# aagdev/mlimgsynth

Hardware: AMD Instinct MI355X
Metric: images/sec (20-step Euler-a, cfg 7) SDXL 1024x1024 (higher is better)
Workload: dtype f16; 1 GPU; sdxl-1024x1024-euler_a-20-cfg7-b4-vae; batch_per_gpu=4, global_batch=4, unet_evals_per_image=40, hipgraph=False, parallelism=single GPU, weights=synthetic seed 1234

## Files before the change

### include/mlblock_amd.h

```cpp
#pragma once
#include <stdbool.h>
#include <stddef.h>
#include <stdint.h>

#ifdef __cplusplus
extern "C" {
#endif

typedef struct MLCtx MLCtx;
typedef struct MLTensor MLTensor;

enum { MLT_F32 = 0, MLT_F16 = 1, MLT_Q4_0 = 2, MLT_Q4_1 = 3, MLT_Q5_0 = 6, MLT_Q5_1 = 7, MLT_Q8_0 = 8, MLT_I32 = 26, MLT_I64 = 27, MLT_F64 = 28,
       MLT_BF16 = 30 };

enum MLCtxFlags {
	MLB_F_MULTI_COMPUTE = 1,
	MLB_F_QUIET = 2,
	MLB_F_DUMP = 4,
	MLB_F_HIPGRAPH = 8,
	MLB_F_OPSHAPES = 16,
	MLB_F_SYNTH_PARAMS = 32,
	MLB_F_KEEP = 64,
};

// ... 23 lines not shown
int    mlctx_ln_fused(const MLCtx* C);
void   mlctx_set_autotune(int on);
void   mlctx_set_hoist(int on);
int    mlctx_once_ops(const MLCtx* C);
int    mlctx_plan_tune_misses(const MLCtx* C);
void   mlctx_set_nearest_tile(int on);
int    mlctx_plan_tune_nearest(const MLCtx* C);
int    mlctx_tune_misses(void);
int    mlctx_tune_inplan(MLCtx* C, int reps);
int    mlsd_tune_dump(const char* path);

void      mlctx_block_begin(MLCtx* C);
MLTensor* mlctx_tensor_add(MLCtx* C, const char* name, MLTensor* t);
MLTensor* mlctx_input_new(MLCtx* C, const char* name, int dtype, int n0, int n1, int n2, int n3);
MLTensor* mlctx_result(MLCtx* C);
MLTensor* mlctx_split_add(MLCtx* C, MLTensor* t);
void mlctx_free(MLCtx* C);
int  mlctx_build_alloc(MLCtx* C, MLTensor* result);
int  mlctx_block_graph_dump_path(const MLCtx* C, const char* path);

int mlctx_input_set(MLCtx* C, MLTensor* t, const void* host_data, size_t nbytes);
int mlctx_output_get(MLCtx* C, MLTensor* t, float* host_out, size_t nbytes);
typedef struct LocalTensor {
	float* d;
	int n[4];
	int flags;
} LocalTensor;
enum { LT_F_OWNMEM = 1, LT_F_READY = 2 };
size_t ltensor_nelements(const LocalTensor* S);
size_t ltensor_nbytes(const LocalTensor* S);
void   ltensor_resize(LocalTensor* S, int n0, int n1, int n2, int n3);
void   ltensor_free(LocalTensor* S);
int    ltensor_shape_check(const LocalTensor* S, int n0, int n1, int n2, int n3);
int    ltensor_finite_check(const LocalTensor* S);
int    ltensor_to_backend(MLCtx* C, const LocalTensor* S, MLTensor* input);
int    ltensor_from_backend(MLCtx* C, LocalTensor* S, MLTensor* t);
int mlctx_run_(MLCtx* C, LocalTensor* out, const LocalTensor** inputs);
struct MLTStore;
void mlctx_set_tstore(MLCtx* C, const struct MLTStore* S);
#define mlctx_run(C,O,...) mlctx_run_((C), (O), (const LocalTensor*[]){ __VA_ARGS__, NULL })
void* mlctx_input_device_ptr(MLTensor* t);
int mlctx_input_bind(MLTensor* t, const float* dev_src, int n_src, const float* dev_scale, float scale0, int mode);
uint16_t mlb_f32_to_f16_bits(float f);
float mlb_f16_bits_to_f32(uint16_t h);
const float* mlctx_tensor_device_f32(MLCtx* C, MLTensor* t, int64_t* ld);
void mlctx_tensor_shape(const MLTensor* t, int64_t ne[4]);

int mlctx_param_count(const MLCtx* C);
void mlctx_params_unload(MLCtx* C);
int mlctx_params_loaded(const MLCtx* C);
int mlctx_param_info(const MLCtx* C, int i, const char** key, int* type, int64_t ne[4]);
int mlctx_param_set(MLCtx* C, const char* key, int src_type, const void* host_data, int64_t n_elem);
int mlctx_param_find(const MLCtx* C, const char* key);
int mlctx_param_lora(MLCtx* C, const char* key, const float* up, const float* down, int64_t n0, int64_t n1, int r, float scale);
int mlctx_params_synth(MLCtx* C, uint64_t seed);

typedef struct MLCtxInfo {
	size_t mem_params, mem_compute, mem_total;
	double t_load, t_compute;
	unsigned n_compute, n_conv;
	unsigned n_ops;
	double flops;
} MLCtxInfo;
void mlctx_info(const MLCtx* C, MLCtxInfo* out);
int mlctx_op_info(const MLCtx* C, int i, const char** label, double* flops);
const struct mlsd_gemm_args* mlctx_op_gemm_args(const MLCtx* C, int i);
const struct mlsd_attn_args* mlctx_op_attn_args(const MLCtx* C, int i);
int mlctx_op_attn_is_ctx(const MLCtx* C, int i);
typedef struct mlb_ln_args { const float* x; int64_t ldx; int rows, d; float eps; const float *g, *b; void* y16; float* y32; } mlb_ln_args;
typedef struct mlb_n2h_args { const float* src; int n_src, C, HW; void* dst; int n_dst, Cpad; const float* scale; float scale0; int mode; } mlb_n2h_args;
typedef struct mlb_h2n_args { const float* src; int64_t ld; int n, C, HW; float* dst; float mul, add; } mlb_h2n_args;
typedef struct mlb_temb_args { const float* t; int n, dim; float maxp; void* out; } mlb_temb_args;
typedef struct mlb_act_args { const float* x; void* y; size_t n; int act; } mlb_act_args;
typedef struct mlb_cemb_args { const int32_t* tok; int n, T, d; const void* tw; const float* pw; float* out; } mlb_cemb_args;
typedef struct mlb_smax_args { const float* in; int64_t ld_in; void* out; int64_t ld_out; int rows, cols; float scale; } mlb_smax_args;
typedef struct mlb_copy_args { const void* src; void* dst; size_t nbytes; } mlb_copy_args;
typedef struct mlb_cadd_args { float* dst; int64_t ld_dst; const float* base; int64_t ld_base; const float* ctrl; int64_t ld_ctrl; int n_img, rows, C, n_ctrl; const float* gain; } mlb_cadd_args;
typedef struct mlb_freeu_args { float* dst; int64_t ld_dst; const float* src; int64_t ld_src; int n_img, H, W, C; float* ws; const float* f; } mlb_freeu_args;
typedef struct mlb_xavt_args { const void* v; int64_t ldv; int n_img, Tk, N; void* vt; } mlb_xavt_args;
typedef struct MLOpRecord {
	int kind, fused, once;
	int gn_src[2];
	const char* label;
	const void* args; size_t args_bytes;
} MLOpRecord;
int mlctx_op_record(const MLCtx* C, int i, MLOpRecord* out);
int mlctx_op_kind_info(int kind, const char** name, size_t* args_bytes);
int mlctx_op_kind_can_fuse(int kind);
int mlctx_param_device(const MLCtx* C, int i, const void** dev, size_t* elems, int* elem_bytes);
int mlctx_weight_slab(const MLCtx* C, int k, const void** dev, size_t* nbytes);
typedef struct MLInputRecord { const char* name; const void* stage; size_t stage_bytes; const void* src; int n_src; const void* scale; } MLInputRecord;
int mlctx_input_count(const MLCtx* C);
int mlctx_input_record(const MLCtx* C, int i, MLInputRecord* out);
int mlctx_zeroed_block(const MLCtx* C, int i, const void** dev, size_t* nbytes);
int mlctx_scratch_block(const MLCtx* C, int which, const void** dev, size_t* nbytes);
double mlctx_op_bytes(const MLCtx* C, int i);
int mlctx_profile_ops(MLCtx* C, float* ms_out, int n_out);

MLTensor* mlb_nn_linear(MLCtx* C, MLTensor* x, int n_out, bool bias);
MLTensor* mlb_nn_conv2d(MLCtx* C, MLTensor* x, int ch_out,
	int k0, int k1, int s0, int s1, int p0, int p1, int d0, int d1, bool bias);
MLTensor* mlb_nn_layer_norm(MLCtx* C, MLTensor* x, bool affine, bool bias, float eps);
MLTensor* mlb_nn_groupnorm(MLCtx* C, MLTensor* x, int n_grp, bool affine, float eps);
static inline MLTensor* mlb_nn_groupnorm32(MLCtx* C, MLTensor* x) { return mlb_nn_groupnorm(C, x, 32, true, 1e-6f); }
MLTensor* mlb_downsample(MLCtx* C, MLTensor* x, int ch_out, bool vae);
MLTensor* mlb_upsample(MLCtx* C, MLTensor* x, int ch_out);
// ... 17 lines not shown
```

### include/mlsd_kernels.h

```cpp
#pragma once
#include <stddef.h>
#include <stdint.h>

#ifdef __cplusplus
extern "C" {
#endif

const char* mlsd_last_error(void);
const char* mlsd_peek_runtime_error(void);
void mlsd_runtime_dry(int on);
int mlsd_runtime_is_dry(void);
int mlsd_device_count(void);
int mlsd_device_set(int dev);
int mlsd_device_info(int dev, char* name, int name_len, char* arch, int arch_len, int* n_cu,
                     size_t* mem_total, size_t* mem_free);
int mlsd_malloc(void** out, size_t nbytes);
int mlsd_free(void* p);
int mlsd_host_alloc(void** out, size_t nbytes);
int mlsd_host_free(void* p);
int mlsd_memset(void* dst, int value, size_t nbytes, void* stream);
int mlsd_memcpy(void* dst, const void* src, size_t nbytes, int kind , void* stream);
int mlsd_stream_create(void** out);
int mlsd_stream_create_masked(void** out, const uint32_t* cu_mask, int n_words);
int mlsd_cu_census(unsigned* out_dev, int n_blocks, int spin_cycles, void* stream);
// ... 42 lines not shown
	MLSD_TILE_W4_128x320 = 27,
	MLSD_TILE_PPSK_128x320 = 28,
	MLSD_TILE_SKINNY = 29,
	MLSD_TILE_TT = 30,
	MLSD_TILE_CONV_SMALLN = 31
};
#define MLSD_TILE_ARG(v) ((v) + 1)

typedef struct mlsd_gemm_args {
	const void* A;
	int64_t lda;
	int conv;
	int n_img, H, W, Cin;
	int OH, OW;
	int KH, KW, stride, pad;
	int upsample;
	const void* W_;
	int64_t ldb;
	int M, N, K;
	const float* bias;
	const float* rowbias;
	int rows_per_batch;
	int64_t ldrb;
	const float* resid;
	int64_t ldr;
	int act;
	float* C32;
	int64_t ldc32;
	void* C16;
	int64_t ldc16;
	const float* bias_m;
	int act_after_resid;
	int tile_variant;
	int ksplit;
	void* ws;
	size_t ws_bytes;
	float* colstats;
	int colstats_rows;
	unsigned* sk_flags;
	void* ln_y16; int64_t ldln;
	const float *ln_gamma, *ln_beta;
	float ln_eps;
	float* ln_ws;
	unsigned* ln_cnt;
	int ln_slot;
	void* gn_y16; int64_t gn_ldy;
	const float *gn_gamma, *gn_beta;
	float gn_eps;
	int gn_groups, gn_hw, gn_silu;
	const void* xa_k; int64_t xa_ldk;
	const void* xa_vt;
	void* xa_out; int64_t xa_ldo;
	int xa_Tq, xa_Tk;
	int colstats_shift;
	int wrap;
} mlsd_gemm_args;

int mlsd_gemm(const mlsd_gemm_args* a, void* stream);
int mlsd_gemm_colstats_rows(const mlsd_gemm_args* a);
int mlsd_gemm_ln_fused(const mlsd_gemm_args* a);
int mlsd_gemm_xattn_fused(const mlsd_gemm_args* a);
void mlsd_gemm_set_xattn(int mode);
int mlsd_xattn_pack_vt(const void* v, int64_t ldv, int n_img, int Tk, int N, void* vt, void* stream);
int mlsd_gemm_gn_fused(const mlsd_gemm_args* a);
const char* mlsd_gemm_variant(const mlsd_gemm_args* a);
typedef struct mlsd_gemm_route_info {
	int variant;
	int asked;
	int nsplit;
	int stats_rows;
	int ln;
	int gn;
	int xattn;
	int handoff;
	int stats_rows_if;
	int ln_if;
	size_t ln_ws_bytes_if;
} mlsd_gemm_route_info;
int mlsd_gemm_route(const mlsd_gemm_args* a, mlsd_gemm_route_info* out);
void mlsd_gemm_set_panel(int width);
void mlsd_gemm_set_mode(int mode);
void mlsd_gemm_force_variant(int v);
int mlsd_gemm_num_variants(void);
void mlsd_gemm_set_epilogue(int e);
void mlsd_gemm_set_debug(int d);
void mlsd_gemm_set_splitk_inline(int on);
void mlsd_gemm_set_splitk_parallel(int on);
int mlsd_gemm_splitk_parallel(const mlsd_gemm_args* a);
int mlsd_conv_smalln_eligible(const mlsd_gemm_args* a);
void mlsd_conv_smalln_set(int ring_rows, int strip_rows);
size_t mlsd_gemm_streamk_ws_bytes(void);
void mlsd_gemm_set_cus(int n);
void mlsd_gemm_set_trace(void* buf);
size_t mlsd_gemm_splitk_ws_bytes(int M, int N, int ksplit);

typedef struct mlsd_attn_args {
	const void *q, *k, *v;
	void* out;
	int64_t ldq, ldk, ldv, ldo;
	int64_t bsq, bsk, bsv, bso;
	int n_batch, n_head, d_head, Tq, Tk;
	int causal;
} mlsd_attn_args;

int mlsd_attention(const mlsd_attn_args* a, void* stream);
int mlsd_attention_ctx(const mlsd_attn_args* a, void* stream);
const char* mlsd_attention_variant(const mlsd_attn_args* a, int ctx);
int mlsd_attention_ctx_takes(const mlsd_attn_args* a);
void mlsd_attention_ctx_mode(int mode);
void mlsd_attention_force_old(int on);
void mlsd_attention_x2_min_tq(int tq);
// ... 112 lines not shown
```

### mlimgsynth_amd/csrc/hip/gemm_conv.hip

```cpp
#include <hip/hip_runtime.h>
#include <stdio.h>
#include <string.h>
#include <stddef.h>
#include <type_traits>
#include "common.hpp"
#include "mlsd_kernels.h"
#include "gemm_params.hpp"
#include "gemm_epilogue.hpp"
#include "gemm_pp.hpp"
#include "gemm_skinny.hpp"

namespace {

template <int BM, int BN, int BK, int WAVES_M, int WAVES_N, bool CONV, int NSTAGE, int DBG = 0, bool REG = false, bool PAR = false, bool ST = false, bool WRAP = false>
__global__ __launch_bounds__(WAVES_M* WAVES_N * 64) __attribute__((amdgpu_waves_per_eu((ST && WAVES_M * WAVES_N >= 8) ? 4 : 1, (ST && WAVES_M * WAVES_N >= 8) ? 4 : 10)))
void gemm_kernel(const GemmP p, const GemmP pe)
{
    constexpr int THREADS = WAVES_M * WAVES_N * 64;
    constexpr int WM = BM / WAVES_M, WN = BN / WAVES_N;
    constexpr int TM = WM / 32, TN = WN / 32;
    constexpr int CPR = BK / 8;
    constexpr int RB = BK * 2;
    constexpr int A_IT = BM * CPR / THREADS, B_IT = BN * CPR / THREADS;
    constexpr int LPT = A_IT + B_IT;
// ... 716 lines not shown
}

bool wrap_foldable(const mlsd_gemm_args* a, int wrap)
{
    const int He = a->upsample ? 2 * a->H : a->H, We = a->upsample ? 2 * a->W : a->W;
    if ((wrap & 2) && (a->pad > He || (a->OH - 1) * a->stride - a->pad + a->KH > 2 * He)) return false;
    if ((wrap & 1) && (a->pad > We || (a->OW - 1) * a->stride - a->pad + a->KW > 2 * We)) return false;
    return true;
}

int g_gemm_ncu = 256;
int g_gemm_dbg = 0;
unsigned long long* g_gemm_tbuf = nullptr;
int g_gemm_panel = 8;
int g_gemm_epi = 0;
int g_gemm_sk_inline = 0;
int g_gemm_sk_par = -1;
bool sk_par_on()
{
    if (g_gemm_sk_par < 0) { const char* e = getenv("MLSD_SPLITK_PAR"); g_gemm_sk_par = (e && *e && *e != '0') ? 1 : 0; }
    return g_gemm_sk_par != 0;
}

int device_cus();
bool splitk_par_ok(const mlsd_gemm_args* a, int BM, int nsplit, long tiles)
{
#ifndef MLSD_GEMM_EXPERIMENTS
    return false;
#endif
    if (!sk_par_on() || !a->sk_flags || nsplit < 2 || tiles > 2047 || a->wrap) return false;
    const int cus = device_cus();
    if (cus < g_gemm_ncu || g_gemm_ncu < 256) return false;
    return tiles * nsplit <= (long)cus * (BM == 64 ? 3 : 2);
}

bool wide_epilogue_ok(const mlsd_gemm_args* a)
{
    return (!a->C32 || (!(a->ldc32 & 3) && !((uintptr_t)a->C32 & 15))) && (!a->C16 || (!(a->ldc16 & 3) && !((uintptr_t)a->C16 & 7))) &&
           (!a->resid || (!(a->ldr & 3) && !((uintptr_t)a->resid & 15))) && (!a->bias || !((uintptr_t)a->bias & 15)) &&
           (!a->rowbias || (!(a->ldrb & 3) && !((uintptr_t)a->rowbias & 15)));
}

GemmP gemm_params_from(const mlsd_gemm_args* a, const GemmRoute& r)
{
    GemmP p{};
    p.A = (const _Float16*)a->A; p.B = (const _Float16*)a->W_;
    p.lda = a->lda; p.ldb = a->ldb; p.M = a->M; p.N = a->N; p.K = a->K;
    p.H = a->H; p.W = a->W; p.Cin = a->Cin; p.OH = a->OH; p.OW = a->OW; p.KH = a->KH; p.KW = a->KW;
    p.stride = a->stride; p.pad = a->pad; p.ups = a->upsample; p.wrap = r.wrap;
    p.bias = a->bias; p.biasm = a->bias_m; p.act_post = a->act_after_resid; p.rowbias = a->rowbias; p.rows_per_batch = a->rows_per_batch > 0 ? a->rows_per_batch : 1;
    p.ldrb = a->ldrb; p.resid = a->resid; p.ldr = a->ldr; p.act = a->act;
    p.C32 = a->C32; p.ldc32 = a->ldc32; p.C16 = (_Float16*)a->C16; p.ldc16 = a->ldc16;
    p.cs_shift = a->colstats_shift ? 1 : 0;
    return p;
}

GemmP split_to_workspace(GemmP& p, const mlsd_gemm_args* a)
{
    GemmP pe = p;
    p.bias = p.biasm = p.rowbias = p.resid = nullptr; p.act = 0; p.act_post = 0;
    p.C16 = nullptr; p.C32 = (float*)a->ws; p.ldc32 = a->N; p.ws_stride = (long)a->M * a->N;
    pe.ws_stride = p.ws_stride;
    return pe;
}

template <int BM, int BN, int BK, int WAVES_M, int WAVES_N, int NSTAGE, bool REG = false>
int launch(const mlsd_gemm_args* a, const GemmRoute& r, hipStream_t st)
{
    GemmP p = gemm_params_from(a, r);
    p.nbm = (a->M + BM - 1) / BM; p.nbn = (a->N + BN - 1) / BN;
    p.vec = r.vec;
    p.dbg = g_gemm_dbg;
    p.gw = g_gemm_panel;
    const int nsplit = r.nsplit;
    p.kt_per = r.kt_per;
    if (r.stats_rows > 0 && nsplit == 1) p.colstats = a->colstats;
    GemmP pe = p;
    const bool inl = r.splitk == SPLITK_INLINE;
    if (inl) { p.sk_L = nsplit; p.sk_ws = (float*)a->ws; p.sk_flag = a->sk_flags; }
    else if (nsplit > 1) {
        const size_t need = (size_t)nsplit * a->M * a->N * sizeof(float);
        if (a->ws_bytes < need || ((uintptr_t)a->ws & 15))
            return mlsd_set_error(-1, "mlsd_gemm: split-K workspace too small or misaligned (%zu < %zu)", (size_t)a->ws_bytes, need);
        pe = split_to_workspace(p, a);
        if (r.stats_rows > 0) pe.colstats = a->colstats;
    }
    constexpr int THREADS = WAVES_M * WAVES_N * 64;
    constexpr size_t RING = (size_t)NSTAGE * (BM + BN) * BK * 2;
    constexpr size_t EPI = (size_t)WAVES_M * WAVES_N * 32 * 64 * 4;
    constexpr size_t LDS = RING > EPI ? RING : EPI;
    const dim3 grid(p.nbm * p.nbn, nsplit), block(THREADS);
    auto go = [&](auto kfn, const char* what = "gemm_kernel") -> int {
        if (LDS > 65536) MLSD_HIP_TRY(hipFuncSetAttribute((const void*)kfn, hipFuncAttributeMaxDynamicSharedMemorySize, (int)LDS));
        hipLaunchKernelGGL(kfn, grid, block, LDS, st, p, pe);
        if (r.splitk == SPLITK_TWO_LAUNCH) {
            const long n = (long)a->M * (a->N >> 2);
#ifdef MLSD_GEMM_EXPERIMENTS
            if (r.gn) {
                GemmP pl = pe;
                pl.ln_g = a->gn_gamma; pl.ln_b = a->gn_beta; pl.ln_eps = a->gn_eps; pl.ln_y = (_Float16*)a->gn_y16; pl.ldln = a->gn_ldy;
                pl.gn_G = a->gn_groups; pl.gn_hw = a->gn_hw; pl.gn_silu = a->gn_silu;
                hipLaunchKernelGGL(splitk_reduce_gn, dim3((unsigned)a->gn_groups, (unsigned)(a->M / a->gn_hw)), dim3(256), 0, st, pl, (const float*)a->ws, nsplit);
            } else
#endif
            if (r.ln == 2) {
                GemmP pl = pe;
                pl.ln_g = a->ln_gamma; pl.ln_b = a->ln_beta; pl.ln_eps = a->ln_eps; pl.ln_y = (_Float16*)a->ln_y16; pl.ldln = a->ldln;
                hipLaunchKernelGGL(splitk_reduce_ln, dim3((unsigned)a->M), dim3((unsigned)(((a->N >> 2) + 63) / 64 * 64)), 0, st, pl, (const float*)a->ws, nsplit);
            } else if (pe.colstats)
                hipLaunchKernelGGL(splitk_reduce_stats, dim3((unsigned)(((a->N >> 2) + 63) / 64), (unsigned)((a->M + 31) / 32)), dim3(256), 0, st, pe, (const float*)a->ws, nsplit);
            else
            hipLaunchKernelGGL(splitk_reduce, dim3((unsigned)((n + 255) / 256)), dim3(256), 0, st, pe, (const float*)a->ws, nsplit);
        }
        return mlsd_check_launch(what);
    };
#ifdef MLSD_GEMM_EXPERIMENTS
    if constexpr ((BM == 64 || BM == 128) && BN == 128 && BK == 64 && NSTAGE == 2 && !REG) {
        if (r.splitk == SPLITK_PAR) {
            p.sk_flag = a->sk_flags;
            const char* what = "gemm_kernel(split-K, reduced in the launch)";
            return a->conv ? go(gemm_kernel<BM, BN, BK, WAVES_M, WAVES_N, true, NSTAGE, 0, false, true>, what) : go(gemm_kernel<BM, BN, BK, WAVES_M, WAVES_N, false, NSTAGE, 0, false, true>, what);
        }
    }
#endif
#ifdef MLSD_GEMM_EXPERIMENTS
    if (!a->conv && g_gemm_dbg == 1) return go(gemm_kernel<BM, BN, BK, WAVES_M, WAVES_N, false, NSTAGE, 1, REG>);
    if (!a->conv && g_gemm_dbg == 2) return go(gemm_kernel<BM, BN, BK, WAVES_M, WAVES_N, false, NSTAGE, 2, REG>);
#endif
    if (r.wrap) {
        if constexpr (((BN / WAVES_N) / 32) % 2 == 0) {
            if (p.colstats) return go(gemm_kernel<BM, BN, BK, WAVES_M, WAVES_N, true, NSTAGE, 0, false, false, true, true>);
        }
        return go(gemm_kernel<BM, BN, BK, WAVES_M, WAVES_N, true, NSTAGE, 0, false, false, false, true>);
    }
    if constexpr (((BN / WAVES_N) / 32) % 2 == 0 && !REG) {
        if (p.colstats) return a->conv ? go(gemm_kernel<BM, BN, BK, WAVES_M, WAVES_N, true, NSTAGE, 0, false, false, true>) : go(gemm_kernel<BM, BN, BK, WAVES_M, WAVES_N, false, NSTAGE, 0, false, false, true>);
    }
    return a->conv ? go(gemm_kernel<BM, BN, BK, WAVES_M, WAVES_N, true, NSTAGE, 0, REG>) : go(gemm_kernel<BM, BN, BK, WAVES_M, WAVES_N, false, NSTAGE, 0, REG>);
}

int device_cus()
{
    static thread_local int cached_dev = -1, cached = 0;
    int dev = 0;
    if (mlsd_runtime_is_dry() || hipGetDevice(&dev) != hipSuccess) { (void)hipGetLastError(); return 0; }
    if (dev != cached_dev) {
        hipDeviceProp_t pr;
        cached = hipGetDeviceProperties(&pr, dev) == hipSuccess ? pr.multiProcessorCount : 0;
        cached_dev = dev;
    }
    return cached;
}

int g_gemm_korder = 0;
int pp_epilogue_kind(const mlsd_gemm_args* a, int BN);
bool pp_eligible(const mlsd_gemm_args* a, int BM, int BN)
{
    if ((a->K & 63) || a->K < 192 || (a->M % (BM / 2)) || (a->N % (BN / 4))) return false;
    if (a->conv && ((a->Cin & 63) || a->KH * a->KW > 9)) return false;
    if (a->conv && a->upsample) {
        const int e = pp_epilogue_kind(a, BN);
        if (a->stride != 1 || a->pad > 16 || a->H > 16000 || a->W > 16000 || (e != 2  && e != 5 )) return false;
    }
    if (a->conv && a->wrap) {
        const int e = pp_epilogue_kind(a, BN);
        if (a->pad > 16 || a->H > 16000 || a->W > 16000 || (e != PP_EPI_F32 && e != PP_EPI_F32_STATS && e != PP_EPI_F32_RES && e != PP_EPI_F32_RES_STATS)) return false;
    }
    if (a->rowbias && ((a->rows_per_batch > 0 ? a->rows_per_batch : 1) % BM)) return false;
    if (a->act == MLSD_ACT_GEGLU && BN != 256) return false;
    const int nout = a->act == MLSD_ACT_GEGLU ? a->N / 2 : a->N;
    return !(nout & 3) && wide_epilogue_ok(a) && g_gemm_epi != 1;
}

bool ln_eligible(const mlsd_gemm_args* a)
{
    if (!a->ln_y16 || !a->ln_gamma || !a->ln_beta || !a->ln_ws || !a->ln_cnt || a->conv || a->colstats || a->rowbias || a->bias_m || a->act != MLSD_ACT_NONE) return false;
    if (!a->C32 || a->C16 || (a->M % 128) || (a->N % 320) || (a->ldln & 7) || ((uintptr_t)a->ln_y16 & 15) || ((uintptr_t)a->ln_gamma & 15) || ((uintptr_t)a->ln_beta & 15)) return false;
    const long nbn = a->N / 320, tiles = (long)(a->M / 128) * nbn;
    const bool one_round = tiles <= g_gemm_ncu;
    const bool whole_rounds = g_gemm_ncu == 256 && !(tiles % 256) && (nbn == 1 || nbn == 2 || nbn == 4);
    return (one_round || whole_rounds) && nbn <= 8 && a->ln_slot >= 0 && a->ln_slot < 8191 && pp_eligible(a, 128, 320) && device_cus() >= g_gemm_ncu;
}

int g_xattn_mode = -1;
int xattn_mode()
{
    if (g_xattn_mode < 0) { const char* e = getenv("MLSD_XATTN"); g_xattn_mode = (e && *e >= '0' && *e <= '2') ? *e - '0' : 1; }
    return g_xattn_mode;
}
bool xattn_eligible(const mlsd_gemm_args* a)
{
    if (!a->xa_k || !a->xa_vt || !a->xa_out || !xattn_mode() || a->conv || a->act != MLSD_ACT_NONE || a->C32 || a->resid || a->rowbias || a->bias_m || a->colstats) return false;
    if (a->ln_y16 || a->gn_y16 || (a->M % 128) || (a->N % 320) || (a->K & 63) || a->K < 192) return false;
    if (a->xa_Tq <= 0 || (a->xa_Tq % 128) || (a->M % a->xa_Tq) || a->xa_Tk < 1 || a->xa_Tk > 77) return false;
    if (xattn_mode() != 2 && (long)(a->M / 128) * (a->N / 320) <= g_gemm_ncu / 2) return false;
    if ((a->xa_ldk & 7) || (a->xa_ldo & 7) || ((uintptr_t)a->xa_k & 15) || ((uintptr_t)a->xa_vt & 15) || ((uintptr_t)a->xa_out & 15) || (a->bias && ((uintptr_t)a->bias & 15))) return false;
    return g_gemm_epi != 1 && !(g_gemm_dbg & 2);
}

int pp_epilogue_kind(const mlsd_gemm_args* a, int BN)
{
    if (a->xa_k && BN == 320 && xattn_eligible(a)) return PP_EPI_XATTN;
    if ((g_gemm_dbg & 2) || a->bias_m) return PP_EPI_GENERIC;
    const bool c16_wide = a->C16 && !(a->ldc16 & 7) && !((uintptr_t)a->C16 & 15);
    if (a->act == MLSD_ACT_NONE) {
        if (a->C16 && !a->C32 && !a->resid) return c16_wide ? PP_EPI_F16 : PP_EPI_GENERIC;
        if (a->C32 && !a->C16) {
            if (a->ln_y16 && ln_eligible(a)) return a->resid ? PP_EPI_F32_RES_LN : PP_EPI_F32_LN;
            const bool st = a->colstats != nullptr && !((uintptr_t)a->colstats & 15) && !(a->N & 3);
            return a->resid ? (st ? PP_EPI_F32_RES_STATS : PP_EPI_F32_RES) : (st ? PP_EPI_F32_STATS : PP_EPI_F32);
        }
    } else if (a->act == MLSD_ACT_GEGLU && BN == 256 && c16_wide && !a->C32 && !a->resid && !a->conv) return PP_EPI_GEGLU16;
    return PP_EPI_GENERIC;
}

int sk_share(long ntiles, int nkt, int ncu)
{
    const long even = (ntiles * nkt + ncu - 1) / ncu;
    for (int L = (int)(even < 4 ? 4 : even); L < nkt; ++L) if (nkt % L == 0) return L;
    return nkt;
}

bool sk_eligible(const mlsd_gemm_args* a, int BM, int BN, bool ignore_stats = false)
{
    if (!pp_eligible(a, BM, BN) || !a->ws || !a->sk_flags || ((uintptr_t)a->ws & 15) || device_cus() < g_gemm_ncu || (a->conv && a->upsample)) return false;
    if (a->conv && a->colstats && !ignore_stats) return false;
    if (a->conv && a->wrap && !a->colstats && pp_epilogue_kind(a, BN) != PP_EPI_F32 && pp_epilogue_kind(a, BN) != PP_EPI_F32_RES) return false;
    const long tiles = (long)((a->M + BM - 1) / BM) * ((a->N + BN - 1) / BN), nkt = a->K / 64;
    const long L = sk_share(tiles, (int)nkt, g_gemm_ncu);
    return nkt >= 3 && L >= 4 && L < nkt && a->ws_bytes >= (size_t)g_gemm_ncu * BM * BN * sizeof(float);
}

template <int BM, int BN, int CB0, int CB1, bool RESBATCH, bool SK = false, int NPH = 4, int SCH = 0>
int launch_pp(const mlsd_gemm_args* a, const GemmRoute& r, hipStream_t st)
{
    constexpr int BK = 64;
    GemmP p = gemm_params_from(a, r);
    p.korder = g_gemm_korder;
    p.nbm = (a->M + BM - 1) / BM; p.nbn = (a->N + BN - 1) / BN;
    p.vec = 1;
    p.dbg = g_gemm_dbg; p.gw = g_gemm_panel; p.tbuf = g_gemm_tbuf;
    p.kt_per = (a->K + BK - 1) / BK;
    constexpr size_t LDS = 2 * (size_t)(BM + BN) * BK * 2;
    const int ntiles = p.nbm * p.nbn;
    p.ln_g = a->ln_gamma; p.ln_b = a->ln_beta; p.ln_eps = a->ln_eps; p.ln_y = (_Float16*)a->ln_y16; p.ldln = a->ldln; p.ln_ws = a->ln_ws; p.ln_cnt = a->ln_cnt; p.ln_slot = a->ln_slot;
    if constexpr (SK) {
        p.sk_L = sk_share(ntiles, a->K / BK, g_gemm_ncu);
        p.sk_ws = (float*)a->ws; p.sk_flag = a->sk_flags;
    }
    const dim3 grid(SK ? g_gemm_ncu : (ntiles < g_gemm_ncu ? ntiles : g_gemm_ncu)), block(512);
    auto go = [&](auto kfn) -> int {
        MLSD_HIP_TRY(hipFuncSetAttribute((const void*)kfn, hipFuncAttributeMaxDynamicSharedMemorySize, (int)LDS));
        hipLaunchKernelGGL(kfn, grid, block, LDS, st, p);
        return mlsd_check_launch("gemm_pp_kernel");
    };
    auto go_ln = [&](auto kfn) -> int {
        MLSD_HIP_TRY(hipFuncSetAttribute((const void*)kfn, hipFuncAttributeMaxDynamicSharedMemorySize, (int)(LDS + 4096 + 8192)));
        hipLaunchKernelGGL(kfn, grid, block, LDS + 4096 + 8192, st, p);
        return mlsd_check_launch("gemm_pp_kernel(+LN)");
    };
    auto go_xa = [&](auto kfn) -> int {
        constexpr int XLDS = 57344 + 128 * 640;
        p.xa_k = (const _Float16*)a->xa_k; p.xa_vt = (const _Float16*)a->xa_vt; p.xa_out = (_Float16*)a->xa_out; p.xa_ldk = a->xa_ldk; p.xa_ldo = a->xa_ldo;
        p.xa_Tq = a->xa_Tq; p.xa_Tk = a->xa_Tk; p.xa_sc = 1.4426950408889634f * 0.125f;
        MLSD_HIP_TRY(hipFuncSetAttribute((const void*)kfn, hipFuncAttributeMaxDynamicSharedMemorySize, XLDS));
        hipLaunchKernelGGL(kfn, dim3(ntiles), block, XLDS, st, p);
        return mlsd_check_launch("gemm_pp_kernel(+attention)");
    };
    const int epi = r.epi;
    p.colstats = (epi == PP_EPI_F32_STATS || epi == PP_EPI_F32_RES_STATS) ? a->colstats : nullptr;
    if constexpr (SK) {
        if (r.wrap) {
            if (epi == PP_EPI_F32) return go(gemm_pp_kernel<BM, BN, CB0, CB1, RESBATCH, 5, PP_EPI_F32, true>);
            if (epi == PP_EPI_F32_RES) return go(gemm_pp_kernel<BM, BN, CB0, CB1, RESBATCH, 5, PP_EPI_F32_RES, true>);
            return mlsd_set_error(-1, "mlsd_gemm: stream-K tile: wrap convolution with epilogue %d", epi);
        }
        if (a->conv) {
            switch (epi) {
            case PP_EPI_F32: return go(gemm_pp_kernel<BM, BN, CB0, CB1, RESBATCH, true, PP_EPI_F32, true>);
            case PP_EPI_F32_RES: return go(gemm_pp_kernel<BM, BN, CB0, CB1, RESBATCH, true, PP_EPI_F32_RES, true>);
            case PP_EPI_F32_STATS: return go(gemm_pp_kernel<BM, BN, CB0, CB1, RESBATCH, true, PP_EPI_F32_STATS, true>);
            case PP_EPI_F32_RES_STATS: return go(gemm_pp_kernel<BM, BN, CB0, CB1, RESBATCH, true, PP_EPI_F32_RES_STATS, true>);
            default: return go(gemm_pp_kernel<BM, BN, CB0, CB1, RESBATCH, true, PP_EPI_GENERIC, true>);
            }
        }
        switch (epi) {
        case PP_EPI_F16: return go(gemm_pp_kernel<BM, BN, CB0, CB1, RESBATCH, false, PP_EPI_F16, true>);
        case PP_EPI_F32: return go(gemm_pp_kernel<BM, BN, CB0, CB1, RESBATCH, false, PP_EPI_F32, true>);
        case PP_EPI_F32_RES: return go(gemm_pp_kernel<BM, BN, CB0, CB1, RESBATCH, false, PP_EPI_F32_RES, true>);
        default: return go(gemm_pp_kernel<BM, BN, CB0, CB1, RESBATCH, false, PP_EPI_GENERIC, true>);
        }
    }
    if (r.wrap) {
        if (a->upsample) {
            if (epi == PP_EPI_F32_STATS) return go(gemm_pp_kernel<BM, BN, CB0, CB1, RESBATCH, 6, PP_EPI_F32_STATS, false, NPH, SCH>);
            if (epi == PP_EPI_F32) return go(gemm_pp_kernel<BM, BN, CB0, CB1, RESBATCH, 6, PP_EPI_F32, false, NPH, SCH>);
        } else {
            switch (epi) {
            case PP_EPI_F32: return go(gemm_pp_kernel<BM, BN, CB0, CB1, RESBATCH, 5, PP_EPI_F32, false, NPH, SCH>);
            case PP_EPI_F32_RES: return go(gemm_pp_kernel<BM, BN, CB0, CB1, RESBATCH, 5, PP_EPI_F32_RES, false, NPH, SCH>);
            case PP_EPI_F32_STATS: return go(gemm_pp_kernel<BM, BN, CB0, CB1, RESBATCH, 5, PP_EPI_F32_STATS, false, NPH, SCH>);
            case PP_EPI_F32_RES_STATS: return go(gemm_pp_kernel<BM, BN, CB0, CB1, RESBATCH, 5, PP_EPI_F32_RES_STATS, false, NPH, SCH>);
            default: break;
            }
        }
        return mlsd_set_error(-1, "mlsd_gemm: ping-pong tile: wrap convolution with epilogue %d", epi);
    }
    if (a->conv && a->upsample) {
        if (epi == PP_EPI_F32_STATS) return go(gemm_pp_kernel<BM, BN, CB0, CB1, RESBATCH, 2, PP_EPI_F32_STATS, false, NPH, SCH>);
        if (epi == PP_EPI_F32) return go(gemm_pp_kernel<BM, BN, CB0, CB1, RESBATCH, 2, PP_EPI_F32, false, NPH, SCH>);
        return mlsd_set_error(-1, "mlsd_gemm: ping-pong tile: upsampled convolution with epilogue %d", epi);
    }
    if (a->conv) {
        switch (epi) {
        case PP_EPI_F32: return go(gemm_pp_kernel<BM, BN, CB0, CB1, RESBATCH, true, PP_EPI_F32, false, NPH, SCH>);
        case PP_EPI_F32_RES: return go(gemm_pp_kernel<BM, BN, CB0, CB1, RESBATCH, true, PP_EPI_F32_RES, false, NPH, SCH>);
        case PP_EPI_F32_STATS: return go(gemm_pp_kernel<BM, BN, CB0, CB1, RESBATCH, true, PP_EPI_F32_STATS, false, NPH, SCH>);
        case PP_EPI_F32_RES_STATS: return go(gemm_pp_kernel<BM, BN, CB0, CB1, RESBATCH, true, PP_EPI_F32_RES_STATS, false, NPH, SCH>);
        default: return go(gemm_pp_kernel<BM, BN, CB0, CB1, RESBATCH, true, PP_EPI_GENERIC, false, NPH, SCH>);
        }
    }
    switch (epi) {
    case PP_EPI_F16: return go(gemm_pp_kernel<BM, BN, CB0, CB1, RESBATCH, false, PP_EPI_F16, false, NPH, SCH>);
    case PP_EPI_F32: return go(gemm_pp_kernel<BM, BN, CB0, CB1, RESBATCH, false, PP_EPI_F32, false, NPH, SCH>);
    case PP_EPI_F32_RES: return go(gemm_pp_kernel<BM, BN, CB0, CB1, RESBATCH, false, PP_EPI_F32_RES, false, NPH, SCH>);
    case PP_EPI_F32_STATS: return go(gemm_pp_kernel<BM, BN, CB0, CB1, RESBATCH, false, PP_EPI_F32_STATS, false, NPH, SCH>);
    case PP_EPI_F32_RES_STATS: return go(gemm_pp_kernel<BM, BN, CB0, CB1, RESBATCH, false, PP_EPI_F32_RES_STATS, false, NPH, SCH>);
    case PP_EPI_F32_LN:
        if constexpr (BM == 128 && BN == 320 && NPH == 4 && SCH == 0) return go_ln(gemm_pp_kernel<BM, BN, CB0, CB1, RESBATCH, false, PP_EPI_F32_LN, false, 4, 0>);
        break;
    case PP_EPI_F32_RES_LN:
        if constexpr (BM == 128 && BN == 320 && NPH == 4 && SCH == 0) return go_ln(gemm_pp_kernel<BM, BN, CB0, CB1, RESBATCH, false, PP_EPI_F32_RES_LN, false, 4, 0>);
        break;
    case PP_EPI_GEGLU16:
        if constexpr (BN == 256) return go(gemm_pp_kernel<BM, BN, CB0, CB1, RESBATCH, false, PP_EPI_GEGLU16, false, NPH, SCH>);
        break;
    case PP_EPI_XATTN:
        if constexpr (BM == 128 && BN == 320 && NPH == 4 && SCH == 0) return go_xa(gemm_pp_kernel<BM, BN, CB0, CB1, RESBATCH, false, PP_EPI_XATTN, false, 4, 0>);
        return mlsd_set_error(-1, "mlsd_gemm: cross attention at the end of a projection runs on the four-phase 128x320 tile only");
    default: break;
    }
    return go(gemm_pp_kernel<BM, BN, CB0, CB1, RESBATCH, false, PP_EPI_GENERIC, false, NPH, SCH>);
}

bool skinny_eligible(const mlsd_gemm_args* a)
{
    if (a->M > 128 || a->act == MLSD_ACT_GEGLU || (a->K & 63) || a->K < 128 || (a->N & 3) || !a->ws || ((uintptr_t)a->ws & 15)) return false;
    if (a->conv && (a->upsample || (a->Cin & 63) || a->KH * a->KW > 9)) return false;
    if (a->conv && a->wrap && (a->pad > 16 || a->H > 16000 || a->W > 16000)) return false;
    return wide_epilogue_ok(a);
}

int skinny_slices(const mlsd_gemm_args* a, int* kt_per_out)
{
    const int nkt = a->K / 64;
    int s = a->ksplit < 1 ? 1 : a->ksplit;
    if (s > nkt / 2) s = nkt / 2 > 0 ? nkt / 2 : 1;
    const int maxper = SKINNY_MAXG * 4;
    if ((nkt + s - 1) / s > maxper) s = (nkt + maxper - 1) / maxper;
    const int per = (nkt + s - 1) / s;
    if (kt_per_out) *kt_per_out = per;
    return (nkt + per - 1) / per;
}

int launch_skinny(const mlsd_gemm_args* a, const GemmRoute& r, hipStream_t st)
{
    GemmP p = gemm_params_from(a, r);
    p.vec = 1;
    const int nsplit = r.nsplit;
    const size_t need = (size_t)nsplit * a->M * a->N * sizeof(float);
    if (a->ws_bytes < need) return mlsd_set_error(-1, "mlsd_gemm: skinny-M workspace too small (%zu < %zu)", (size_t)a->ws_bytes, need);
    p.kt_per = r.kt_per;
    const GemmP pe = split_to_workspace(p, a);
    constexpr int PF = 3;
    const dim3 grid((a->N + 63) / 64, nsplit), block(256);
    auto go = [&](auto kfn, int rows, int pf = PF) -> int {
        const size_t lds = (size_t)(pf + 1) * rows * 128;
        static thread_local const void* attr_done[16]; static thread_local int n_done = 0;
        bool seen = false;
        for (int i = 0; i < n_done; ++i) seen |= attr_done[i] == (const void*)kfn;
        if (!seen) {
            MLSD_HIP_TRY(hipFuncSetAttribute((const void*)kfn, hipFuncAttributeMaxDynamicSharedMemorySize, (int)lds));
            if (n_done < 16) attr_done[n_done++] = (const void*)kfn;
        }
        hipLaunchKernelGGL(kfn, grid, block, lds, st, p);
        const long n = (long)a->M * (a->N >> 2);
        hipLaunchKernelGGL(splitk_reduce, dim3((unsigned)((n + 255) / 256)), dim3(256), 0, st, pe, (const float*)a->ws, nsplit);
        return mlsd_check_launch("gemm_skinny_kernel");
    };
#ifdef MLSD_GEMM_EXPERIMENTS
    if (g_gemm_dbg == 16) return a->conv ? go(gemm_skinny_kernel<true, 8, 7, 1>, 128, 7) : go(gemm_skinny_kernel<false, 8, 7, 1>, 128, 7);
    if (g_gemm_dbg == 32) return a->conv ? go(gemm_skinny_kernel<true, 8, 7>, 128, 7) : go(gemm_skinny_kernel<false, 8, 7>, 128, 7);
    if (g_gemm_dbg == 48) return a->conv ? go(gemm_skinny_kernel<true, 8, 3, 1>, 128, 3) : go(gemm_skinny_kernel<false, 8, 3, 1>, 128, 3);
#endif
    if (r.wrap) {
        if (a->M <= 16) return go(gemm_skinny_kernel<true, 1, PF, 0, true>, 32);
        if (a->M <= 64) return go(gemm_skinny_kernel<true, 4, PF, 0, true>, 64);
        return go(gemm_skinny_kernel<true, 8, PF, 0, true>, 128);
    }
    if (a->M <= 16) return a->conv ? go(gemm_skinny_kernel<true, 1, PF>, 32) : go(gemm_skinny_kernel<false, 1, PF>, 32);
// ... 42 lines not shown
    {"256x256x64pp2", 256, 256, 256, 64, 0, 0},
    {"128x320x64ppb", 128, 320, 256, 64, 0, 0},
    {"64x128x64s3", 64, 128, 512, 64, 32, 64},
    {"64x128x64r2", 64, 128, 768, 64, 32, 64, true},
    {"256x128x64pp2", 256, 128, 256, 64, 0, 0},
    {"256x256x64w4", 256, 256, 256, 64, 0, 0},
    {"128x320x64w4", 128, 320, 256, 64, 0, 0},
    {"128x320x64ppsk", 128, 320, 256, 64, 0, 0},
    {"skinny128x64", 128, 64, 512, 64, 0, 0},
    {"128x160x64tt", 128, 160, 512, 64, 0, 0},
    {"conv3x3n16", 64, 16, 512, 64, 0, 0},
};
constexpr int kNumVariants = sizeof(kVariants) / sizeof(kVariants[0]);

int pick_variant(const mlsd_gemm_args* a)
{
    if (g_gemm_variant >= 0 && g_gemm_variant < kNumVariants) return g_gemm_variant;
    if (a->xa_k && xattn_eligible(a) && pp_eligible(a, 128, 320)) return MLSD_TILE_PP_128x320;
    if (mlsd_conv_smalln_eligible(a)) return MLSD_TILE_CONV_SMALLN;
    if (a->tile_variant > 0 && a->tile_variant <= kNumVariants) return a->tile_variant - 1;
    if (a->M <= 64) return MLSD_TILE_64x128;
    auto fill = [&](int bm, int bn, int slots) {
        const long blocks = (long)((a->M + bm - 1) / bm) * ((a->N + bn - 1) / bn);
        const long rounds = (blocks + slots - 1) / slots;
        return (double)blocks / (double)(rounds * slots);
    };
    const double e0 = fill(128, 128, 512), e3 = 1.08 * fill(256, 128, 256);
    if (a->M >= 2048 && a->N >= 1920 && e3 > e0) return MLSD_TILE_256x128;
    return MLSD_TILE_128x128;
}

int general_stats_rows(const mlsd_gemm_args* a, const GemmRoute& r, const Variant& t)
{
    if (!a->colstats || ((uintptr_t)a->colstats & 15) || !a->C32 || a->act == MLSD_ACT_GEGLU || a->ln_y16 || a->gn_y16 || ((t.wave_n / 32) & 1) || (a->N & 3)) return 0;
    if (!r.vec || g_gemm_sk_inline) return 0;
    if (r.nsplit > 1) {
#ifdef MLSD_GEMM_EXPERIMENTS
        if (sk_par_on()) return 0;
#endif
        return 32;
    }
    return t.reg ? 0 : t.wave_m;
}

GemmRoute resolve(const mlsd_gemm_args* a)
{
    GemmRoute r{};
    mlsd_gemm_args aw;
    if (a->wrap) { aw = *a; aw.wrap = conv_wrap(a); a = &aw; }
    r.wrap = a->wrap;
    r.pick = pick_variant(a);
    int v = r.pick;
    GemmFamily fam = FAM_GENERAL;
    switch (v) {
    case MLSD_TILE_W4_256x256: case MLSD_TILE_W4_128x320:
        if (mlsd_gemm_w4_eligible(a, v - MLSD_TILE_W4_256x256)) fam = FAM_W4; else v = v == MLSD_TILE_W4_256x256 ? MLSD_TILE_PP_256x256 : MLSD_TILE_PP_128x320;
        break;
    case MLSD_TILE_PPSK_256x256: if (sk_eligible(a, 256, 256)) fam = FAM_PP_SK; else v = MLSD_TILE_PP_256x256; break;
    case MLSD_TILE_PPSK_128x320: if (sk_eligible(a, 128, 320)) fam = FAM_PP_SK; else v = MLSD_TILE_PP_128x320; break;
    case MLSD_TILE_SKINNY: if (skinny_eligible(a)) fam = FAM_SKINNY; else v = MLSD_TILE_64x128; break;
    case MLSD_TILE_TT: if ((r.epi = mlsd_gemm_tt_eligible(a, tt_ncu()))) fam = FAM_TT; else v = MLSD_TILE_PP_128x320; break;
    case MLSD_TILE_CONV_SMALLN: if (mlsd_conv_smalln_eligible(a)) fam = FAM_SMALLN; else v = MLSD_TILE_128x128; break;
#ifndef MLSD_GEMM_EXPERIMENTS
    case MLSD_TILE_PPB_128x320: v = MLSD_TILE_PP_128x320; break;
    case MLSD_TILE_PP2_256x128: v = MLSD_TILE_256x128; break;
    case 2: case 5: case 6: case 7: case 8: case 10: case 11: case 12: case 13: case 14: case 15: case 23: case 24: v = MLSD_TILE_128x128; break;
#else
    case MLSD_TILE_PPB_128x320: if (r.wrap) v = MLSD_TILE_PP_128x320; break;
    case MLSD_TILE_PP2_256x128: if (r.wrap) v = MLSD_TILE_256x128; break;
    case 2: case 5: case 6: case 7: case 8: case 10: case 11: case 12: case 13: case 14: case 15: case 23: case 24: if (r.wrap) v = MLSD_TILE_128x128; break;
#endif
    default: break;
    }
    if (fam == FAM_GENERAL && !kVariants[v].wave_m) {
        if (pp_eligible(a, kVariants[v].bm, kVariants[v].bn)) fam = FAM_PP;
        else v = kVariants[v].bn == 256 ? MLSD_TILE_256x256 : kVariants[v].bn == 320 ? MLSD_TILE_128x320 : MLSD_TILE_256x128;
    }
    const Variant& t = kVariants[v];
    r.v = v; r.fam = fam; r.bk = t.bk;
    r.nsplit = 1; r.kt_per = (a->K + t.bk - 1) / t.bk;
    switch (fam) {
    case FAM_GENERAL: {
        const int nout = a->act == MLSD_ACT_GEGLU ? a->N / 2 : a->N;
        r.vec = !(nout & 3) && !(a->N & 3) && wide_epilogue_ok(a) && g_gemm_epi != 1;
        int per;
        if (r.vec && (r.nsplit = splitk_slices(a, t.bk, &per)) > 1) {
            r.kt_per = per;
            const long tiles = (long)((a->M + t.bm - 1) / t.bm) * ((a->N + t.bn - 1) / t.bn);
            if (g_gemm_sk_inline && a->sk_flags && tiles <= 4095 && !((uintptr_t)a->ws & 15) &&
                a->ws_bytes >= (size_t)r.nsplit * tiles * t.bm * t.bn * sizeof(float))
                r.splitk = SPLITK_INLINE;
            else if ((v == MLSD_TILE_128x128 || v == MLSD_TILE_64x128) && splitk_par_ok(a, t.bm, r.nsplit, tiles)) r.splitk = SPLITK_PAR;
            else r.splitk = SPLITK_TWO_LAUNCH;
        }
        r.stats_rows = general_stats_rows(a, r, t);
        const bool reduce_norm = (v == MLSD_TILE_128x128 || v == MLSD_TILE_64x128) && r.splitk == SPLITK_TWO_LAUNCH && !g_gemm_sk_inline && a->C32 && !a->C16;
        if (reduce_norm && a->ln_y16 && a->ln_gamma && a->ln_beta && a->N <= 4096 && !(a->ldln & 3) && !((uintptr_t)a->ln_y16 & 7) &&
            !((uintptr_t)a->ln_gamma & 15) && !((uintptr_t)a->ln_beta & 15))
            r.ln = 2;
#ifdef MLSD_GEMM_EXPERIMENTS
        if (reduce_norm && a->gn_y16 && !a->ln_y16 && !a->colstats && a->gn_gamma && a->gn_beta && a->gn_groups > 0 && a->gn_hw > 0 && !(a->N % a->gn_groups) && !(a->M % a->gn_hw)) {
            const int cg = a->N / a->gn_groups;
            r.gn = !(cg & 3) && (long)a->gn_hw * (cg >> 2) <= 256L * GNR_MAXI && !(a->gn_ldy & 3) && !((uintptr_t)a->gn_y16 & 7) && !((uintptr_t)a->gn_gamma & 15) &&
                   !((uintptr_t)a->gn_beta & 15);
        }
#endif
        break;
    }
    case FAM_PP: case FAM_PP_SK:
        r.epi = pp_epilogue_kind(a, t.bn);
        if (r.epi == PP_EPI_F32_STATS || r.epi == PP_EPI_F32_RES_STATS) r.stats_rows = t.bm / 2;
        r.ln = fam == FAM_PP && r.pick == MLSD_TILE_PP_128x320 && (r.epi == PP_EPI_F32_LN || r.epi == PP_EPI_F32_RES_LN);
        r.xattn = fam == FAM_PP && r.pick == MLSD_TILE_PP_128x320 && r.epi == PP_EPI_XATTN && g_gemm_variant < 0;
        break;
    case FAM_SKINNY:
        r.nsplit = skinny_slices(a, &r.kt_per);
        r.splitk = SPLITK_TWO_LAUNCH;
        break;
    case FAM_TT: r.ln = r.epi >= 4 && r.epi <= 7; break;
    case FAM_W4: case FAM_SMALLN: break;
    }
    if (((r.pick == MLSD_TILE_PPSK_256x256 || r.pick == MLSD_TILE_PPSK_128x320) && a->conv && sk_eligible(a, kVariants[r.pick].bm, kVariants[r.pick].bn, true)) || r.pick == MLSD_TILE_TT) r.stats_rows = 0;
    return r;
}

mlsd_gemm_args what_if(const mlsd_gemm_args* a, bool stats, bool ln)
{
    alignas(256) static float ph[64];
    mlsd_gemm_args w = *a;
    if (stats && !w.colstats) w.colstats = ph;
    if (ln && !w.ln_y16) { w.ln_y16 = ph; w.ldln = w.N; w.ln_gamma = w.ln_beta = w.ln_ws = ph; w.ln_cnt = (unsigned*)ph; }
    return w;
}

}

extern "C" {

MLSD_API int mlsd_gemm(const mlsd_gemm_args* a, void* stream)
{
    if (!a || !a->A || !a->W_) return mlsd_set_error(-1, "mlsd_gemm: null operand");
    if (a->M <= 0 || a->N <= 0 || a->K <= 0) return mlsd_set_error(-1, "mlsd_gemm: empty problem M=%d N=%d K=%d", a->M, a->N, a->K);
    if ((a->K & 7) || (a->lda & 7) || (a->ldb & 7)) return mlsd_set_error(-1, "mlsd_gemm: K, lda, ldb must be multiples of 8 (K=%d lda=%ld ldb=%ld)", a->K, (long)a->lda, (long)a->ldb);
    if (((uintptr_t)a->A & 15) || ((uintptr_t)a->W_ & 15)) return mlsd_set_error(-1, "mlsd_gemm: operands must be 16-byte aligned");
    if (a->conv) {
        if (a->K != a->KH * a->KW * a->Cin) return mlsd_set_error(-1, "mlsd_gemm: conv K mismatch");
        if (a->Cin & 7) return mlsd_set_error(-1, "mlsd_gemm: conv Cin must be a multiple of 8");
        if (a->M != a->n_img * a->OH * a->OW) return mlsd_set_error(-1, "mlsd_gemm: conv M mismatch");
        if (a->wrap & ~3) return mlsd_set_error(-1, "mlsd_gemm: wrap %d is not a mode (bit 0: columns, bit 1: rows)", a->wrap);
        if (!wrap_foldable(a, conv_wrap(a)))
            return mlsd_set_error(-1, "mlsd_gemm: wrap: a tap lies more than one image extent outside the %dx%d source (pad %d)", a->H, a->W, a->pad);
    }
    if (a->act == MLSD_ACT_GEGLU && (a->N & 63)) return mlsd_set_error(-1, "mlsd_gemm: GEGLU needs N %% 64 == 0");
    if (!a->C32 && !a->C16 && !a->xa_k) return mlsd_set_error(-1, "mlsd_gemm: no output");
    const GemmRoute r = resolve(a);
    if (a->colstats && a->colstats_rows > 0 && r.stats_rows != a->colstats_rows)
        return mlsd_set_error(-1, "mlsd_gemm: a GroupNorm was planned on this launch's column statistics (blocks of %d rows) but the launch "
                              "would write %d-row blocks / none: tile or epilogue settings changed after planning", a->colstats_rows, r.stats_rows);
    if (a->gn_y16 && !r.gn)
        return mlsd_set_error(-1, "mlsd_gemm: the plan dropped a GroupNorm for this launch's reduce pass but the launch would not run it (tile or K-split settings changed after planning)");
    if (a->xa_k && !r.xattn)
        return mlsd_set_error(-1, "mlsd_gemm: the plan dropped a cross attention for this projection's launch but the launch would not run it (tile settings changed after planning)");
    if (a->ln_y16 && !r.ln)
        return mlsd_set_error(-1, "mlsd_gemm: the plan dropped a LayerNorm for this launch's *_LN epilogue but the launch would not run it (tile or epilogue settings changed after planning)");
    hipStream_t st = (hipStream_t)stream;
    switch (r.fam) {
    case FAM_W4: return mlsd_gemm_w4(a, r.v - MLSD_TILE_W4_256x256, st, g_gemm_ncu);
    case FAM_TT: return mlsd_gemm_tt(a, st, tt_ncu());
    case FAM_SMALLN: return mlsd_conv_smalln(a, st);
    case FAM_SKINNY: return launch_skinny(a, r, st);
    case FAM_PP_SK: return r.v == MLSD_TILE_PPSK_256x256 ? launch_pp<256, 256, 2, 2, false, true>(a, r, st) : launch_pp<128, 320, 3, 2, true, true>(a, r, st);
    case FAM_PP:
        switch (r.v) {
        case MLSD_TILE_PP_256x256: return launch_pp<256, 256, 2, 2, false>(a, r, st);
        case MLSD_TILE_PP2_128x320: return launch_pp<128, 320, 3, 2, true, false, 2>(a, r, st);
        case MLSD_TILE_PP2_256x256: return launch_pp<256, 256, 2, 2, false, false, 2>(a, r, st);
#ifdef MLSD_GEMM_EXPERIMENTS
        case MLSD_TILE_PPB_128x320: return launch_pp<128, 320, 3, 2, true, false, 4, 1>(a, r, st);
        case MLSD_TILE_PP2_256x128: return launch_pp<256, 128, 1, 1, false, false, 2>(a, r, st);
#endif
        default: return launch_pp<128, 320, 3, 2, true>(a, r, st);
        }
    case FAM_GENERAL: break;
    }
    switch (r.v) {
    case MLSD_TILE_64x128: return launch<64, 128, 64, 2, 2, 2>(a, r, st);
    case MLSD_TILE_256x128: return launch<256, 128, 64, 4, 2, 2>(a, r, st);
    case MLSD_TILE_256x128_S3: return launch<256, 128, 32, 4, 2, 3>(a, r, st);
    case MLSD_TILE_256x256: return launch<256, 256, 64, 4, 4, 2>(a, r, st);
    case MLSD_TILE_128x320:
        if (a->act == MLSD_ACT_GEGLU)
            return mlsd_set_error(-1, "%s", r.pick == MLSD_TILE_128x320 ? "mlsd_gemm: tile variant 16 (odd slab count) does not support GEGLU" : "mlsd_gemm: the 128x320 tiles do not support GEGLU");
        return launch<128, 320, 64, 4, 2, 2>(a, r, st);
#ifdef MLSD_GEMM_EXPERIMENTS
    case 2: return launch<128, 128, 32, 2, 2, 4>(a, r, st);
    case 5: return launch<128, 128, 64, 2, 2, 3>(a, r, st);
    case 14: return launch<128, 128, 64, 2, 2, 2, true>(a, r, st);
    case 23: return launch<64, 128, 64, 2, 2, 3>(a, r, st);
    case 24: return launch<64, 128, 64, 2, 2, 2, true>(a, r, st);
    case 6: return launch<256, 256, 32, 2, 4, 3>(a, r, st);
    case 7: return launch<256, 128, 32, 4, 2, 4>(a, r, st);
    case 8: return launch<256, 256, 32, 4, 4, 3>(a, r, st);
    case 10: return launch<256, 256, 32, 4, 4, 4>(a, r, st);
    case 11: return launch<256, 256, 64, 2, 4, 2>(a, r, st);
    case 12: return launch<256, 256, 32, 2, 4, 4>(a, r, st);
    case 13: return launch<256, 256, 64, 4, 4, 2, true>(a, r, st);
    case 15: return launch<256, 128, 64, 4, 2, 2, true>(a, r, st);
#endif
// ... 7 lines not shown
MLSD_API void mlsd_gemm_set_epilogue(int e) { g_gemm_epi = e; }
MLSD_API void mlsd_gemm_set_debug(int d) { g_gemm_dbg = d; }
#ifdef MLSD_GEMM_EXPERIMENTS
MLSD_API void mlsd_gemm_set_korder(int k) { g_gemm_korder = k; }
#else
MLSD_API void mlsd_gemm_set_korder(int k) { (void)k; }
#endif
#ifdef MLSD_GEMM_EXPERIMENTS
MLSD_API void mlsd_gemm_set_splitk_inline(int on) { g_gemm_sk_inline = on != 0; }
#else
MLSD_API void mlsd_gemm_set_splitk_inline(int on) { (void)on; }
#endif
MLSD_API int mlsd_has_experiments(void)
{
#ifdef MLSD_GEMM_EXPERIMENTS
    return 1;
#else
    return 0;
#endif
}
MLSD_API void mlsd_gemm_set_splitk_parallel(int on) { g_gemm_sk_par = on ? 1 : 0; }
MLSD_API int mlsd_gemm_splitk_parallel(const mlsd_gemm_args* a) { return a && a->ksplit >= 2 && a->sk_flags && resolve(a).splitk == SPLITK_PAR; }
MLSD_API void mlsd_gemm_set_cus(int n) { g_gemm_ncu = n > 0 && n <= 256 ? n : 256; }
MLSD_API void mlsd_gemm_set_trace(void* buf) { g_gemm_tbuf = (unsigned long long*)buf; }

MLSD_API int mlsd_gemm_num_variants(void) { return kNumVariants; }

MLSD_API size_t mlsd_gemm_splitk_ws_bytes(int M, int N, int ksplit)
{
    return ksplit > 1 ? (size_t)ksplit * ((M + 127) / 128 * 128) * ((N + 127) / 128 * 128) * sizeof(float) : 0;
}

MLSD_API size_t mlsd_gemm_streamk_ws_bytes(void) { return (size_t)256 * 256 * 256 * sizeof(float); }

MLSD_API int mlsd_gemm_route(const mlsd_gemm_args* a, mlsd_gemm_route_info* out)
{
    if (!a || !out) return -1;
    const mlsd_gemm_args ws = what_if(a, true, false), wl = what_if(a, false, true);
    const GemmRoute r = resolve(a), rs = resolve(&ws), rl = resolve(&wl);
    *out = {r.v, r.v == r.pick, r.nsplit, a->colstats ? r.stats_rows : 0, a->ln_y16 ? r.ln : 0, a->gn_y16 && r.gn, a->xa_k && r.xattn,
            r.fam == FAM_PP_SK || r.ln == 1 || r.splitk == SPLITK_PAR, rs.stats_rows, rl.ln,
            rl.ln == 1 ? (size_t)a->M * (a->N / kVariants[rl.v].bn) * 16 : 0};
    return 0;
}

MLSD_API int mlsd_gemm_colstats_rows(const mlsd_gemm_args* a) { mlsd_gemm_route_info r; return mlsd_gemm_route(a, &r) ? 0 : r.stats_rows; }

MLSD_API int mlsd_gemm_ln_fused(const mlsd_gemm_args* a) { mlsd_gemm_route_info r; return mlsd_gemm_route(a, &r) ? 0 : r.ln; }

MLSD_API int mlsd_gemm_gn_fused(const mlsd_gemm_args* a) { mlsd_gemm_route_info r; return mlsd_gemm_route(a, &r) ? 0 : r.gn; }

MLSD_API void mlsd_gemm_set_xattn(int mode) { g_xattn_mode = (mode >= 0 && mode <= 2) ? mode : -1; }

MLSD_API int mlsd_gemm_xattn_fused(const mlsd_gemm_args* a) { mlsd_gemm_route_info r; return mlsd_gemm_route(a, &r) ? 0 : r.xattn; }

MLSD_API const char* mlsd_gemm_variant(const mlsd_gemm_args* a)
{
    static thread_local char buf[64];
    const GemmRoute r = resolve(a);
    const char *name = kVariants[r.v].name, *op = a->conv ? "conv" : "linear";
    const int ns = r.fam == FAM_GENERAL ? splitk_slices(a, r.bk, nullptr) : 1;
    if (r.fam == FAM_SKINNY) snprintf(buf, sizeof(buf), "gemm<%s,%s,k/%d>", name, op, r.nsplit);
    else if (ns > 1) snprintf(buf, sizeof(buf), "gemm<%s,%s%s,k/%d%s>", name, op, r.ln == 2 ? "+layernorm" : (r.gn ? "+groupnorm" : ""), ns, r.splitk == SPLITK_PAR ? "p" : "");
    else if (r.xattn) snprintf(buf, sizeof(buf), "gemm<%s,linear+attention>", name);
    else if (r.ln) snprintf(buf, sizeof(buf), "gemm<%s,linear+layernorm>", name);
    else snprintf(buf, sizeof(buf), "gemm<%s,%s>", name, op);
    return buf;
}

}
```

### mlimgsynth_amd/csrc/hip/gemm_params.hpp

```cpp
#pragma once
#include <hip/hip_runtime.h>
#include <stddef.h>
#include "common.hpp"
#include "mlsd_kernels.h"

namespace {

struct GemmP {
    const _Float16* A;
    const _Float16* B;
    long lda, ldb;
    int M, N, K;
    int H, W, Cin, OH, OW, KH, KW, stride, pad, ups;
    int korder;
    const float* bias;
    const float* biasm;
    int act_post;
    int wrap;
    const float* rowbias;
    int rows_per_batch;
    long ldrb;
    const float* resid;
    long ldr;
    int act;
    float* C32;
    long ldc32;
    _Float16* C16;
    long ldc16;
    int nbm, nbn;
    int vec;
    int dbg;
    int kt_per;
    long ws_stride;
    int gw;
    unsigned long long* tbuf;
    float* colstats;
    int cs_shift;
    int sk_L;
    float* sk_ws;
    unsigned* sk_flag;
    const float *ln_g, *ln_b;
    float ln_eps;
    _Float16* ln_y;
    long ldln;
    float* ln_ws;
    unsigned* ln_cnt;
    int ln_slot;
    int gn_G, gn_hw, gn_silu;
    const _Float16 *xa_k, *xa_vt;
    _Float16* xa_out;
    long xa_ldk, xa_ldo;
    int xa_Tq, xa_Tk;
    float xa_sc;
};

static_assert(offsetof(GemmP, wrap) + sizeof(int) == offsetof(GemmP, rowbias), "GemmP::wrap must fill act_post's padding");

__device__ __forceinline__ int wrap_fold(int v, int e) { return v < 0 ? v + e : (v >= e ? v - e : v); }

template <int BK>
__device__ __forceinline__ int row_swz(int row) { return BK == 64 ? ((row >> 1) & 7) : ((row >> 2) & 3); }
template <int BK>
__device__ __forceinline__ int lds_off(int row, int chunk) { return row * (BK * 2) + ((chunk ^ row_swz<BK>(row)) << 4); }

__device__ uint4 g_zero_page[4];

template <int N>
__device__ __forceinline__ void wait_vmcnt()
{
    static_assert(N >= 0 && N < 64, "vmcnt immediate range");
    asm volatile("s_waitcnt vmcnt(%0)" ::"n"(N) : "memory");
}

}
```

### mlimgsynth_amd/csrc/hip/gemm_pp.hpp

```cpp
#pragma once
#include "gemm_params.hpp"

namespace {

struct PPTile { int m0, n0; };

template <int BM, int BN>
__device__ __forceinline__ PPTile pp_tile_coords(const GemmP& p, int v)
{
    const int nblk = p.nbm * p.nbn;
    const int q = nblk >> 3, r = nblk & 7, x = v & 7, j = v >> 3;
    int bid = (x < r ? x * (q + 1) : r * (q + 1) + (x - r) * q) + j;
    int bm, bn;
    if (p.gw > 0 && p.nbn > p.gw) {
        const int per_panel = p.gw * p.nbm;
        const int panel = bid / per_panel;
        const int first = panel * p.gw;
        const int w = min(p.gw, p.nbn - first);
        const int rr = bid - panel * per_panel;
        bm = rr / w; bn = first + (rr - bm * w);
    } else {
        bm = bid / p.nbn; bn = bid - bm * p.nbn;
    }
    return PPTile{bm * BM, bn * BN};
}

template <int BM, int BN>
__device__ __forceinline__ PPTile pp_tile_plain(const GemmP& p, int bid)
{
    int bm, bn;
    if (p.gw > 0 && p.nbn > p.gw) {
        const int per_panel = p.gw * p.nbm;
        const int panel = bid / per_panel;
        const int first = panel * p.gw;
        const int w = min(p.gw, p.nbn - first);
        const int rr = bid - panel * per_panel;
        bm = rr / w; bn = first + (rr - bm * w);
    } else {
        bm = bid / p.nbn; bn = bid - bm * p.nbn;
    }
    return PPTile{bm * BM, bn * BN};
}

enum { PP_EPI_GENERIC = 0, PP_EPI_F16 = 1, PP_EPI_F32 = 2, PP_EPI_F32_RES = 3, PP_EPI_GEGLU16 = 4, PP_EPI_F32_STATS = 5, PP_EPI_F32_RES_STATS = 6,
       PP_EPI_F32_LN = 7, PP_EPI_F32_RES_LN = 8, PP_EPI_XATTN = 9 };
template <int BM, int BN, int CB0, int CB1, bool RESBATCH, int CONV, int EPI, bool SK = false, int NPH = 4, int SCH = 0>
__global__ __launch_bounds__(512) void gemm_pp_kernel(const GemmP p)
{
    constexpr int BK = 64, RB = BK * 2;
    constexpr int WM = BM / 2, WN = BN / 4;
    constexpr int RA = WM / 32;
    constexpr int NCB = CB0 + CB1;
    static_assert(NCB * 16 == WN && RA * 32 == WM, "wave tile");
    constexpr int STAGE = (BM + BN) * RB;
    constexpr int BOFF = BM * RB;
    constexpr int NU1 = BM / 128, NU2 = CB0, NU3 = CB1;
    constexpr int W4 = NU3 + 2 * NU1, W1 = 2 * NU1 + NU2, W2 = NU1 + NU2 + NU3;
    extern __shared__ __attribute__((aligned(16))) unsigned char smem[];

    const int tid = threadIdx.x, lane = tid & 63;
    const int wave = __builtin_amdgcn_readfirstlane(tid >> 6);
    const int wr = wave >> 2, wc = wave & 3;
    const int l15 = lane & 15, lg = lane >> 4;
    const int nblk = p.nbm * p.nbn;
    const int G = gridDim.x;
    const int nkt = p.K / BK;
    int ntile = (nblk - (int)blockIdx.x + G - 1) / G;
    int S = ntile * nkt;
    int kt0 = 0, tfirst = 0, skw = 0;
    if constexpr (SK) {
        const int q = G >> 3, r = G & 7, x = (int)blockIdx.x & 7, j = (int)blockIdx.x >> 3;
        skw = (x < r ? x * (q + 1) : r * (q + 1) + (x - r) * q) + j;
        const long W = (long)nblk * nkt, u0 = (long)skw * p.sk_L;
        if (u0 >= W) return;
        const long u1 = min(u0 + p.sk_L, W);
        S = (int)(u1 - u0); tfirst = (int)(u0 / nkt); kt0 = (int)(u0 - (long)tfirst * nkt);
        ntile = (int)((u1 - 1) / nkt) - tfirst + 1;
    }
    auto tile_at = [&](int ti) __attribute__((always_inline)) {
        if constexpr (SK) return pp_tile_plain<BM, BN>(p, min(tfirst + ti, nblk - 1));
        else return pp_tile_coords<BM, BN>(p, (int)blockIdx.x + ti * G);
    };
    int kenter = kt0;

    auto a_row0 = [&](int it, int second) __attribute__((always_inline)) {
        const int g = it * 8 + wave;
        return (g / (WM / 16)) * WM + (g % (WM / 16)) * 8 + second * (WM / 2);
    };
    auto b_row0 = [&](int it, int second) __attribute__((always_inline)) {
        const int per = (second ? CB1 : CB0) * 2;
        const int g = it * 8 + wave;
        return (g / per) * WN + (g % per) * 8 + second * (CB0 * 16);
    };
    auto chunk_of = [&](int row) __attribute__((always_inline)) { return ((lane & 7) ^ ((row >> 1) & 7)) * 8; };

    constexpr bool UPS = (CONV & 3) == 2, WRAP = (CONV & 4) != 0, POS = UPS || WRAP;
    struct SeqA { int kt, par; const _Float16* ptr[NU1]; int mask[CONV ? NU1 : 1]; int pos[POS ? NU1 : 1]; int kh, kw, cin; };
    struct SeqB2 { int kt, par; const _Float16* ptr[NU2]; };
    struct SeqB3 { int kt, par; const _Float16* ptr[NU3]; };
    SeqA sa[2];
    SeqB2 sb2;
    SeqB3 sb3;
    PPTile tnext = tile_at(0);
    PPTile tcur = tnext;
    const _Float16* zsrc = reinterpret_cast<const _Float16*>(g_zero_page);

    auto enter_A = [&](SeqA& s, int second) __attribute__((always_inline)) {
        s.kt = kenter; s.kh = 0; s.kw = 0; s.cin = 0;
        if constexpr (CONV) {
            if (kenter) {
#ifdef MLSD_GEMM_EXPERIMENTS
                if (p.korder) { const int kk = p.KH * p.KW, slab = kenter / kk, tap = kenter - slab * kk; s.cin = slab * BK; s.kh = tap / p.KW; s.kw = tap - s.kh * p.KW; }
                else
#endif
                { const int k0 = kenter * BK, tap = k0 / p.Cin; s.cin = k0 - tap * p.Cin; s.kh = tap / p.KW; s.kw = tap - s.kh * p.KW; }
            }
        }
#pragma unroll
        for (int it = 0; it < NU1; ++it) {
            const int r = a_row0(it, second) + (lane >> 3);
            const int m = min(tnext.m0 + r, p.M - 1);
            if constexpr (CONV) {
                const int ohw = p.OH * p.OW;
                const int img = m / ohw, rem = m - img * ohw;
                const int oh = rem / p.OW, ow = rem - oh * p.OW;
                const int ih0 = oh * p.stride - p.pad, iw0 = ow * p.stride - p.pad;
                const int He = UPS ? 2 * p.H : p.H, We = UPS ? 2 * p.W : p.W;
                int mk = 0;
                if constexpr (WRAP) {
                    const bool wy = p.wrap & 2, wx = p.wrap & 1;
                    for (int kh = 0; kh < p.KH; ++kh)
                        for (int kw = 0; kw < p.KW; ++kw)
                            if ((wy || (unsigned)(ih0 + kh) < (unsigned)He) && (wx || (unsigned)(iw0 + kw) < (unsigned)We)) mk |= 1 << (kh * p.KW + kw);
                } else
                for (int kh = 0; kh < p.KH; ++kh)
                    for (int kw = 0; kw < p.KW; ++kw)
                        if ((unsigned)(ih0 + kh) < (unsigned)He && (unsigned)(iw0 + kw) < (unsigned)We) mk |= 1 << (kh * p.KW + kw);
                s.mask[it] = mk;
                if constexpr (POS) {
                    s.pos[it] = ((ih0 + 16) << 16) | (iw0 + 16);
                    s.ptr[it] = p.A + (long)img * p.H * p.W * p.lda + chunk_of(r);
                } else
                s.ptr[it] = p.A + ((long)img * p.H * p.W + (long)ih0 * p.W + iw0) * p.lda + chunk_of(r);
            } else {
                s.ptr[it] = p.A + (long)m * p.lda + chunk_of(r) + kenter * BK;
            }
        }
    };
    auto enter_B2 = [&](SeqB2& s) __attribute__((always_inline)) {
        s.kt = kenter;
#pragma unroll
        for (int it = 0; it < NU2; ++it) {
            const int r = b_row0(it, 0) + (lane >> 3);
            s.ptr[it] = p.B + (long)min(tnext.n0 + r, p.N - 1) * p.ldb + chunk_of(r) + kenter * BK;
        }
    };
    auto enter_B3 = [&](SeqB3& s) __attribute__((always_inline)) {
        s.kt = kenter;
#pragma unroll
        for (int it = 0; it < NU3; ++it) {
            const int r = b_row0(it, 1) + (lane >> 3);
            s.ptr[it] = p.B + (long)min(tnext.n0 + r, p.N - 1) * p.ldb + chunk_of(r) + kenter * BK;
        }
    };
    auto issue_A = [&](SeqA& s, int second) __attribute__((always_inline)) {
        unsigned char* stage = smem + s.par * STAGE;
        const long toff = CONV ? ((long)s.kh * p.W + s.kw) * p.lda + s.cin : 0;
        const int tbit = CONV ? 1 << (s.kh * p.KW + s.kw) : 0;
#pragma unroll
        for (int it = 0; it < NU1; ++it) {
            unsigned char* dst = stage + a_row0(it, second) * RB;
            const _Float16* src = s.ptr[it];
            if constexpr (WRAP) {
                const int He = UPS ? 2 * p.H : p.H, We = UPS ? 2 * p.W : p.W;
                int ih = wrap_fold((s.pos[it] >> 16) - 16 + s.kh, He), iw = wrap_fold((s.pos[it] & 0xffff) - 16 + s.kw, We);
                if constexpr (UPS) { ih >>= 1; iw >>= 1; }
                src = (s.mask[it] & tbit) ? s.ptr[it] + ((long)ih * p.W + iw) * p.lda + s.cin : zsrc;
            } else
            if constexpr (UPS) {
// ... 86 lines not shown
        } else {
#pragma unroll
            for (int e = 0; e < 4; ++e) v[e] = fmaxf(v[e], act_lo);
        }
        return v;
    };
    f32x4 cb[NCB];
    f32x4 rpre[RESBATCH ? 2 * RA * NCB : 1];
    auto epi_rows = [&](auto QA, auto I, int wrow0, int wcol0) __attribute__((always_inline)) {
        constexpr int qa = decltype(QA)::value, i = decltype(I)::value;
        const int m = wrow0 + qa * (WM / 2) + i * 16 + l15;
        const float bm = p.biasm ? p.biasm[m] : 0.f;
        if (!geglu) {
            const long col = wcol0 + 4 * lg;
            const float* rrow = p.resid ? p.resid + (long)m * p.ldr + col : nullptr;
            float* c32 = p.C32 ? p.C32 + (long)m * p.ldc32 + col : nullptr;
            _Float16* c16 = p.C16 ? p.C16 + (long)m * p.ldc16 + col : nullptr;
#pragma unroll
            for (int c = 0; c < NCB; ++c) {
                f32x4 v = acc[qa][i][c] + cb[c];
                v += bm;
                f32x4 rs = {0.f, 0.f, 0.f, 0.f};
                if constexpr (RESBATCH) { if (p.resid) rs = rpre[(qa * RA + i) * NCB + c]; }
                else { if (rrow) rs = *reinterpret_cast<const f32x4*>(rrow + c * 16); }
                if (p.act_post) v += rs;
                v = act4(v);
                if (!p.act_post) v += rs;
                if (c32) *reinterpret_cast<f32x4*>(c32 + c * 16) = v;
                if (c16) {
                    f16x4 h = {(_Float16)v[0], (_Float16)v[1], (_Float16)v[2], (_Float16)v[3]};
                    *reinterpret_cast<f16x4*>(c16 + c * 16) = h;
                }
            }
        } else if constexpr (CB0 == 2 && CB1 == 2) {
            const long col = (wcol0 >> 6) * 32 + 4 * lg;
            const float* rrow = p.resid ? p.resid + (long)m * p.ldr + col : nullptr;
            float* c32 = p.C32 ? p.C32 + (long)m * p.ldc32 + col : nullptr;
            _Float16* c16 = p.C16 ? p.C16 + (long)m * p.ldc16 + col : nullptr;
#pragma unroll
            for (int j = 0; j < 2; ++j) {
                const f32x4 a4 = acc[qa][i][j] + cb[j], g4 = acc[qa][i][2 + j] + cb[2 + j];
                f32x4 v;
                v[0] = a4[0] * gelu_tanh_f(g4[0]); v[1] = a4[1] * gelu_tanh_f(g4[1]);
                v[2] = a4[2] * gelu_tanh_f(g4[2]); v[3] = a4[3] * gelu_tanh_f(g4[3]);
                if (rrow) v += *reinterpret_cast<const f32x4*>(rrow + j * 16);
                if (c32) *reinterpret_cast<f32x4*>(c32 + j * 16) = v;
                if (c16) {
                    f16x4 h = {(_Float16)v[0], (_Float16)v[1], (_Float16)v[2], (_Float16)v[3]};
                    *reinterpret_cast<f16x4*>(c16 + j * 16) = h;
                }
            }
        }
    };
    auto epi_fast = [&](auto S32_, auto S16_, auto RES_, auto ST_, int wrow0, int wcol0) __attribute__((always_inline)) {
        constexpr bool S32 = decltype(S32_)::value, S16 = decltype(S16_)::value, RES = decltype(RES_)::value, ST = decltype(ST_)::value;
        constexpr int NR = 2 * RA;
        constexpr int PF = !ST ? (BM == 128 ? NR : 2) : (BM == 128 ? NR : 1);
        f32x4 cs[ST ? NCB : 1], cq[ST ? NCB : 1], ck[ST ? NCB : 1];
        if constexpr (ST) {
#pragma unroll
            for (int c = 0; c < NCB; ++c) { cs[c] = f32x4{0.f, 0.f, 0.f, 0.f}; cq[c] = f32x4{0.f, 0.f, 0.f, 0.f}; }
        }
        f32x4 rr[RES ? NR : 1][RES ? NCB : 1];
        const float* rbase = RES ? p.resid + (long)(wrow0 + l15) * p.ldr + wcol0 + 4 * lg : nullptr;
        auto row_of = [&](int r) __attribute__((always_inline)) { return (r / RA) * (WM / 2) + (r % RA) * 16; };
        auto fetch = [&](int r) __attribute__((always_inline)) {
            if constexpr (RES) {
                const float* rp = rbase + (long)row_of(r) * p.ldr;
#pragma unroll
                for (int c = 0; c < NCB; ++c) rr[r][c] = *reinterpret_cast<const f32x4*>(rp + c * 16);
            }
        };
#pragma unroll
        for (int r = 0; r < PF && r < NR; ++r) fetch(r);
        float* c32b = S32 ? p.C32 + (long)(wrow0 + l15) * p.ldc32 + wcol0 + 4 * lg : nullptr;
        _Float16* c16b = S16 ? p.C16 + (long)(wrow0 + l15) * p.ldc16 + wcol0 + 4 * lg : nullptr;
#pragma unroll
        for (int r = 0; r < NR; ++r) {
            if (r + PF < NR) fetch(r + PF);
            const int qa = r / RA, i = r % RA;
            if constexpr (S16 && !S32 && !RES && !ST) {
                _Float16* rowp = p.C16 + (long)(wrow0 + l15 + row_of(r)) * p.ldc16 + wcol0 + 8 * (lg >> 1) + 16 * (lg & 1);
#pragma unroll
                for (int c = 0; c + 1 < NCB; c += 2) {
                    const f32x4 v0 = acc[qa][i][c] + cb[c], v1 = acc[qa][i][c + 1] + cb[c + 1];
                    const f16x4 h0 = {(_Float16)v0[0], (_Float16)v0[1], (_Float16)v0[2], (_Float16)v0[3]};
                    const f16x4 h1 = {(_Float16)v1[0], (_Float16)v1[1], (_Float16)v1[2], (_Float16)v1[3]};
                    u32x2 a = __builtin_bit_cast(u32x2, h0), b = __builtin_bit_cast(u32x2, h1);
                    const auto r0 = __builtin_amdgcn_permlane16_swap(a[0], b[0], false, false);
                    const auto r1 = __builtin_amdgcn_permlane16_swap(a[1], b[1], false, false);
                    *reinterpret_cast<u32x4*>(rowp + c * 16) = u32x4{r0[0], r1[0], r0[1], r1[1]};
                }
                if constexpr (NCB & 1) {
                    const f32x4 v = acc[qa][i][NCB - 1] + cb[NCB - 1];
                    f16x4 h = {(_Float16)v[0], (_Float16)v[1], (_Float16)v[2], (_Float16)v[3]};
                    *reinterpret_cast<f16x4*>(c16b + (long)row_of(r) * p.ldc16 + (NCB - 1) * 16) = h;
                }
            } else {
#pragma unroll
            for (int c = 0; c < NCB; ++c) {
                f32x4 v = acc[qa][i][c] + cb[c];
                if constexpr (RES) v += rr[r][c];
                if constexpr (ST) {
                    if (r == 0) {
#pragma unroll
                        for (int e = 0; e < 4; ++e) { const float k = __shfl(v[e], lane & 48, 64); ck[c][e] = p.cs_shift ? k : 0.f; }
                    }
                    const f32x4 d = v - ck[c];
                    cs[c] += d; cq[c] += d * d;
                }
                if constexpr (S32) *reinterpret_cast<f32x4*>(c32b + (long)row_of(r) * p.ldc32 + c * 16) = v;
                if constexpr (S16) {
                    f16x4 h = {(_Float16)v[0], (_Float16)v[1], (_Float16)v[2], (_Float16)v[3]};
                    *reinterpret_cast<f16x4*>(c16b + (long)row_of(r) * p.ldc16 + c * 16) = h;
                }
            }
            }
        }
        if constexpr (ST) {
            auto row16_sum = [&](float v) __attribute__((always_inline)) {
                v += __builtin_bit_cast(float, __builtin_amdgcn_update_dpp(0, __builtin_bit_cast(int, v), 0xB1, 0xF, 0xF, false));
                v += __builtin_bit_cast(float, __builtin_amdgcn_update_dpp(0, __builtin_bit_cast(int, v), 0x4E, 0xF, 0xF, false));
                v += __builtin_bit_cast(float, __builtin_amdgcn_update_dpp(0, __builtin_bit_cast(int, v), 0x141, 0xF, 0xF, false));
                v += __builtin_bit_cast(float, __builtin_amdgcn_update_dpp(0, __builtin_bit_cast(int, v), 0x140, 0xF, 0xF, false));
                return v;
            };
            const long rb = (long)(tcur.m0 / BM) * 2 + wr;
            float* st = p.colstats + rb * 2 * p.N + wcol0 + 4 * lg;
#pragma unroll
            for (int c = 0; c < NCB; ++c) {
#pragma unroll
                for (int e = 0; e < 4; ++e) { cs[c][e] = row16_sum(cs[c][e]); cq[c][e] = row16_sum(cq[c][e]); }
                if (l15 == 0) {
// ... 333 lines not shown
            wait_vmcnt<0>();
            __builtin_amdgcn_s_barrier();
            xstamp(6);
            _Float16* orow = p.xa_out + (long)(tcur.m0 + wave * 16 + l15) * p.xa_ldo + tcur.n0 + 8 * (lg >> 1) + 16 * (lg & 1);
#pragma unroll
            for (int h = 0; h < 5; ++h) {
                union VF { f16x4 h4[2]; f16x8 f; };
                VF vf[4][3];
#pragma unroll
                for (int dt = 0; dt < 4; ++dt) {
                    const unsigned char* vr = smem + QOFF + (h * 64 + dt * 16 + l15) * VP + lg * 8;
#pragma unroll
                    for (int ks = 0; ks < 3; ++ks) {
                        vf[dt][ks].h4[0] = *reinterpret_cast<const f16x4*>(vr + ks * 64);
                        vf[dt][ks].h4[1] = *reinterpret_cast<const f16x4*>(vr + ks * 64 + 32);
                    }
                }
                f32x4 oa[4];
#pragma unroll
                for (int dt = 0; dt < 4; ++dt) oa[dt] = f32x4{0.f, 0.f, 0.f, 0.f};
#pragma unroll
                for (int ks = 0; ks < 3; ++ks)
#pragma unroll
                    for (int dt = 0; dt < 4; ++dt) oa[dt] = __builtin_amdgcn_mfma_f32_16x16x32_f16(vf[dt][ks].f, pf[h][ks], oa[dt], 0, 0, 0);
#pragma unroll
                for (int dt = 0; dt < 4; dt += 2) {
                    const f32x4 o0 = oa[dt] * linv[h], o1 = oa[dt + 1] * linv[h];
                    const f16x4 h0 = {(_Float16)o0[0], (_Float16)o0[1], (_Float16)o0[2], (_Float16)o0[3]};
                    const f16x4 h1 = {(_Float16)o1[0], (_Float16)o1[1], (_Float16)o1[2], (_Float16)o1[3]};
                    const u32x2 a = __builtin_bit_cast(u32x2, h0), b = __builtin_bit_cast(u32x2, h1);
                    const auto r0 = __builtin_amdgcn_permlane16_swap(a[0], b[0], false, false);
                    const auto r1 = __builtin_amdgcn_permlane16_swap(a[1], b[1], false, false);
                    *reinterpret_cast<u32x4*>(orow + h * 64 + dt * 16) = u32x4{r0[0], r1[0], r0[1], r1[1]};
                }
            }
            xstamp(7);
        }
    };
    auto epilogue = [&]() __attribute__((always_inline)) {
        const int wrow0 = tcur.m0 + wr * WM, wcol0 = tcur.n0 + wc * WN;
        if (wrow0 >= p.M || wcol0 >= p.N) return;
        const float* rbias = p.rowbias ? p.rowbias + (long)(tcur.m0 / p.rows_per_batch) * p.ldrb : nullptr;
#pragma unroll
        for (int c = 0; c < NCB; ++c) {
            const int n = wcol0 + c * 16 + 4 * lg;
            f32x4 v = {0.f, 0.f, 0.f, 0.f};
            if (p.bias) v = *reinterpret_cast<const f32x4*>(p.bias + n);
            if (rbias) v += *reinterpret_cast<const f32x4*>(rbias + n);
            cb[c] = v;
        }
        using std::integral_constant;
        using T = std::true_type;
        using F = std::false_type;
        if constexpr (EPI == PP_EPI_F16) { epi_fast(F{}, T{}, F{}, F{}, wrow0, wcol0); return; }
        if constexpr (EPI == PP_EPI_F32) { epi_fast(T{}, F{}, F{}, F{}, wrow0, wcol0); return; }
        if constexpr (EPI == PP_EPI_F32_RES) { epi_fast(T{}, F{}, T{}, F{}, wrow0, wcol0); return; }
        if constexpr (EPI == PP_EPI_F32_STATS) { epi_fast(T{}, F{}, F{}, T{}, wrow0, wcol0); return; }
        if constexpr (EPI == PP_EPI_F32_RES_STATS) { epi_fast(T{}, F{}, T{}, T{}, wrow0, wcol0); return; }
        if constexpr (EPI == PP_EPI_GEGLU16) { epi_fast_geglu(wrow0, wcol0); return; }
        if constexpr (EPI == PP_EPI_F32_LN) { epi_ln(F{}, wrow0, wcol0); return; }
        if constexpr (EPI == PP_EPI_F32_RES_LN) { epi_ln(T{}, wrow0, wcol0); return; }
        if constexpr (EPI == PP_EPI_XATTN) { epi_xattn(wrow0, wcol0); return; }
        if constexpr (EPI == PP_EPI_GENERIC) {
        if constexpr (RESBATCH) {
            if (p.resid) {
#pragma unroll
                for (int qa = 0; qa < 2; ++qa)
#pragma unroll
                    for (int i = 0; i < RA; ++i)
#pragma unroll
                        for (int c = 0; c < NCB; ++c)
                            rpre[(qa * RA + i) * NCB + c] = *reinterpret_cast<const f32x4*>(
                                p.resid + (long)(wrow0 + qa * (WM / 2) + i * 16 + l15) * p.ldr + wcol0 + c * 16 + 4 * lg);
            }
        }
        epi_rows(integral_constant<int, 0>{}, integral_constant<int, 0>{}, wrow0, wcol0);
        epi_rows(integral_constant<int, 0>{}, integral_constant<int, 1>{}, wrow0, wcol0);
        if constexpr (RA > 2) {
            epi_rows(integral_constant<int, 0>{}, integral_constant<int, 2>{}, wrow0, wcol0);
            epi_rows(integral_constant<int, 0>{}, integral_constant<int, 3>{}, wrow0, wcol0);
        }
        epi_rows(integral_constant<int, 1>{}, integral_constant<int, 0>{}, wrow0, wcol0);
        epi_rows(integral_constant<int, 1>{}, integral_constant<int, 1>{}, wrow0, wcol0);
        if constexpr (RA > 2) {
            epi_rows(integral_constant<int, 1>{}, integral_constant<int, 2>{}, wrow0, wcol0);
            epi_rows(integral_constant<int, 1>{}, integral_constant<int, 3>{}, wrow0, wcol0);
        }
        }
    };

    auto stamp = [&](int slot) __attribute__((always_inline)) {
        if (p.tbuf && tid == 0) p.tbuf[(long)blockIdx.x * 8 + slot] = __builtin_readcyclecounter();
    };
    stamp(0);
    sa[0].par = sa[1].par = sb2.par = sb3.par = 0;
    enter_A(sa[0], 0); enter_A(sa[1], 1); enter_B2(sb2); enter_B3(sb3);
    kenter = 0;
    tcur = tnext;
    tnext = tile_at(ntile > 1 ? 1 : 0);
    if constexpr (NPH == 4 && SCH == 1) {
        issue_A(sa[0], 0); issue_B2(); issue_A(sa[1], 1); issue_B3(); issue_A(sa[0], 0); issue_B2();
        wait_vmcnt<NU1 + NU2 + NU3 + NU1>();
    } else {
        issue_A(sa[0], 0); issue_B2(); issue_B3(); issue_A(sa[1], 1);
        if constexpr (NPH == 4) { issue_A(sa[0], 0); wait_vmcnt<W4>(); }
        else wait_vmcnt<NU1>();
    }
    __builtin_amdgcn_s_barrier();
    stamp(1);
    if (wr == 1) __builtin_amdgcn_s_barrier();

// ... 185 lines not shown
```

### mlimgsynth_amd/csrc/host/mlblock.c

```c
#include "mlblock_int.h"
#include <math.h>
#include <stdarg.h>
#include <time.h>

#define CHUNK_BYTES   ((size_t)64 << 20)
#define BIG_BYTES     ((size_t)8 << 20)
#define ALIGN_UP(x,a) (((x) + (a) - 1) / (a) * (a))

#define SK_FLAG_WORDS 4096
#define LN_CNT_WORDS 8192

static mlsd_gemm_route_info route_of(const mlsd_gemm_args* g) { mlsd_gemm_route_info r; mlsd_gemm_route(g, &r); return r; }

#define VEC_PUSH(C, arr, n, cap, T) \
	(((n) == (cap) ? ((cap) = (cap) ? (cap)*2 : 64, (arr) = (T*)realloc((arr), sizeof(T)*(cap))) : 0), &(arr)[(n)++])

static double now_s(void)
{
	struct timespec ts; clock_gettime(CLOCK_MONOTONIC, &ts);
	return ts.tv_sec + ts.tv_nsec*1e-9;
}

int mlctx_fail(MLCtx* C, const char* fmt, ...)
{
	char buf[400];
	va_list ap; va_start(ap, fmt); vsnprintf(buf, sizeof(buf), fmt, ap); va_end(ap);
	if (C && !C->err) C->err = -1;
	return mlsd_set_error(-1, "%s%s%s", C ? C->name : "", C ? ": " : "", buf);
}

MLB_API MLCtx* mlctx_new(void* stream)
{
	MLCtx *C = (MLCtx*)calloc(1, sizeof(MLCtx));
	C->stream = stream;
	C->wtype = MLT_F16;
	C->dry = mlsd_runtime_is_dry();
	return C;
}

static void ctx_reset_(MLCtx* C);
static void wstream_free(MLCtx* C);
static void ctx_reset(MLCtx* C)
{
	const int was = mlsd_runtime_is_dry();
	if (C->dry != was) mlsd_runtime_dry(C->dry);
	ctx_reset_(C);
	if (C->dry != was) mlsd_runtime_dry(was);
	C->dry = was;
}

static void ctx_reset_(MLCtx* C)
{
	if (C->graph_exec) { mlsd_graph_destroy(C->graph_exec); C->graph_exec = NULL; }
	for (int i=0;i<C->n_tensors;++i) free(C->tensors[i]);
	C->n_tensors = 0; C->n_inputs = 0; C->result = NULL;
	for (int i=0;i<C->n_names;++i) free(C->names[i].name);
	C->n_names = 0;
	for (int i=0;i<C->n_params;++i) free(C->params[i].key);
	C->n_params = 0;
	C->n_ops = 0;
	for (int i=0;i<C->n_chunks;++i) mlsd_free(C->chunks[i]);
	if (C->splitk_ws) { mlsd_free(C->splitk_ws); C->splitk_ws = NULL; C->splitk_ws_bytes = 0; }
	if (C->sk_flags) { mlsd_free(C->sk_flags); C->sk_flags = NULL; }
	if (C->ln_cnt) { mlsd_free(C->ln_cnt); C->ln_cnt = NULL; }
	if (C->ln_ws) { mlsd_free(C->ln_ws); C->ln_ws = NULL; C->ln_ws_bytes = 0; }
	if (C->lora_buf) { mlsd_free(C->lora_buf); C->lora_buf = NULL; C->lora_buf_bytes = 0; }
	wstream_free(C);
	C->n_chunks = 0; C->cur = NULL; C->cur_left = 0; C->n_free = 0; C->n_zeroed = 0;
	C->mem_compute = C->mem_params = C->mem_live = C->mem_peak_live = 0;
	C->err = 0; C->prepared = 0; C->tuned = 0; C->n_tune_miss = 0; C->n_tune_near = 0; C->static_valid = 0; C->n_once = 0;
	C->n_ln_fused = 0; C->n_ln_alias = 0; C->n_gn_fused = 0;
	memset(&C->kvb, 0, sizeof(C->kvb));
	memset(&C->epb, 0, sizeof(C->epb));
	memset(&C->info, 0, sizeof(C->info));
}

MLB_API void mlctx_destroy(MLCtx* C)
{
	if (!C) return;
	mlsd_stream_sync(C->stream);
	ctx_reset(C);
	free(C->ops); free(C->tensors); free(C->inputs); free(C->names); free(C->params); free(C->chunks); free(C->freel); free(C->zeroed);
	free(C);
}

MLB_API void mlctx_free(MLCtx* C) { mlctx_destroy(C); }
MLB_API MLTensor* mlctx_split_add(MLCtx* C, MLTensor* t) { (void)C; return t; }

MLB_API void mlctx_begin(MLCtx* C, const char* name)
{
	mlsd_stream_sync(C->stream);
	ctx_reset(C);
	snprintf(C->name, sizeof(C->name), "%s", name ? name : "");
}

MLB_API void mlctx_end(MLCtx* C) { mlsd_stream_sync(C->stream); ctx_reset(C); }
MLB_API void mlctx_set_tprefix(MLCtx* C, const char* p) { snprintf(C->tprefix, sizeof(C->tprefix), "%s", p ? p : ""); }
MLB_API void mlctx_set_flags(MLCtx* C, int f) { C->flags = f; }
MLB_API void mlctx_set_wtype(MLCtx* C, int t) { C->wtype = t; }
MLB_API void mlctx_set_conv_wrap(MLCtx* C, int mode) { C->conv_wrap = mode & 3; }
MLB_API MLTensor* mlctx_result(MLCtx* C) { return C->result; }
MLB_API int mlctx_sync(MLCtx* C) { return mlsd_stream_sync(C->stream) ? -1 : 1; }

MLB_API int mlctx_ln_fused(const MLCtx* C) { return C ? C->n_ln_fused : 0; }
MLB_API int mlctx_ln_alias_refused(const MLCtx* C) { return C ? C->n_ln_alias : 0; }
MLB_API void mlctx_set_cus(MLCtx* C, int n) { if (C) C->cu_budget = n; }

MLB_API int mlctx_handoff_check(MLCtx* C)
{
	if (!C) return 0;
	unsigned w = 0, w2 = 0;
	if (C->sk_flags && (mlsd_memcpy(&w, C->sk_flags + 4095, 4, 1, C->stream) || mlsd_stream_sync(C->stream))) return -1;
	if (C->ln_cnt && (mlsd_memcpy(&w2, C->ln_cnt + 8191, 4, 1, C->stream) || mlsd_stream_sync(C->stream))) return -1;
	if (!w && !w2) return 0;
	mlsd_stream_sync(C->stream);
	if (C->sk_flags) mlsd_memset(C->sk_flags, 0, SK_FLAG_WORDS * 4, C->stream);
	if (C->ln_cnt) mlsd_memset(C->ln_cnt, 0, LN_CNT_WORDS * 4, C->stream);
	if (C->ln_ws) mlsd_memset(C->ln_ws, 0, C->ln_ws_bytes, C->stream);
	mlsd_stream_sync(C->stream);
	return mlsd_set_error(-8, "an in-launch hand-off (%s) timed out (block not resident: is the GPU shared with another process?); results of this plan are invalid",
	                      w ? "stream-K" : "LayerNorm statistics");
}

MLB_API int mlctx_handoff_ops(const MLCtx* C)
{
	int n = 0;
	if (!C || !C->prepared) return 0;
	for (int i=0;i<C->n_ops;++i) {
		const MLOp *o = &C->ops[i];
		if (o->kind == OP_GEMM && route_of(&o->u.gemm).handoff) ++n;
	}
	return n;
}

static int g_handoff_retries = 0;
// ... 75 lines not shown
void* mlctx_dalloc(MLCtx* C, size_t nbytes, int is_param) { return dalloc_ex(C, nbytes, is_param, 0x7fffffff); }

static int is_virtual(const MLCtx* C, const void* p) { return C->pstream && (const char*)p >= MLW_VBASE && (const char*)p < MLW_VBASE + C->pv_size; }

void* mlctx_walloc(MLCtx* C, size_t nbytes)
{
	if (!C->pstream) return dalloc_ex(C, nbytes, 1, 0x7fffffff);
	nbytes = ALIGN_UP(nbytes ? nbytes : 256, 256);
	MLWAlloc *a = VEC_PUSH(C, C->pv_allocs, C->n_pv, C->cap_pv, MLWAlloc);
	a->voff = C->pv_size; a->bytes = nbytes; a->moff = a->voff;
	C->pv_size += nbytes;
	return MLW_VBASE + a->voff;
}

void mlctx_drelease(MLCtx* C, void* p, size_t nbytes)
{
	if (!p || !nbytes) return;
	nbytes = ALIGN_UP(nbytes, 256);
	if (C->flags & MLB_F_KEEP) return;
	MLFreeBlk *b = VEC_PUSH(C, C->freel, C->n_free, C->cap_free, MLFreeBlk);
	b->ptr = p; b->size = nbytes; b->rel_op = C->n_ops;
	C->mem_live -= nbytes;
}

MLTensor* mlt_new(MLCtx* C, int n, int h, int w, int c)
{
	MLTensor *t = (MLTensor*)calloc(1, sizeof(MLTensor));
	t->n = n; t->h = h; t->w = w; t->c = c; t->prod = -1; t->def_op = C->n_ops;
	if (h > 1 || 0) { t->ne[0]=w; t->ne[1]=h; t->ne[2]=c; t->ne[3]=n; }
	else { t->ne[0]=c; t->ne[1]=w; t->ne[2]=n; t->ne[3]=1; }
	*VEC_PUSH(C, C->tensors, C->n_tensors, C->cap_tensors, MLTensor*) = t;
	return t;
}

MLB_API void mlctx_tensor_shape(const MLTensor* t, int64_t ne[4]) { memcpy(ne, t->ne, sizeof(t->ne)); }

MLOp* mlctx_op_new(MLCtx* C, MLOpKind kind, const char* label)
{
	MLOp *op = VEC_PUSH(C, C->ops, C->n_ops, C->cap_ops, MLOp);
	memset(op, 0, sizeof(*op));
	op->kind = kind;
	snprintf(op->label, sizeof(op->label), "%s", label ? label : "");
	return op;
}

float* mlt_need32(MLCtx* C, MLTensor* t)
{
	if (!t) return NULL;
	if (t->d32) return t->d32;
	if (t->released) { mlctx_fail(C, "use of released tensor %s", t->name); return NULL; }
	const int64_t rows = (int64_t)t->n * t->h * t->w;
	if (t->prod >= 0) {
		MLOp *op = &C->ops[t->prod];
		t->sz32 = (size_t)rows * t->c * sizeof(float);
		t->d32 = (float*)dalloc_ex(C, t->sz32, 0, t->prod); t->ld32 = t->c;
		op->u.gemm.C32 = t->d32; op->u.gemm.ldc32 = t->c;
		return t->d32;
	}
	mlctx_fail(C, "tensor %s has no fp32 form", t->name);
	return NULL;
}

void* mlt_need16(MLCtx* C, MLTensor* t)
{
	if (!t) return NULL;
	if (t->d16) return t->d16;
	if (t->released) { mlctx_fail(C, "use of released tensor %s", t->name); return NULL; }
	const int64_t rows = (int64_t)t->n * t->h * t->w;
	if (t->prod >= 0) {
		MLOp *op = &C->ops[t->prod];
		if (t->c % 8) {
			const int cpad = (t->c + 7) / 8 * 8;
			const size_t sz = (size_t)rows * cpad * 2;
			t->d16 = dalloc_ex(C, sz, 2, 0); t->ld16 = cpad;
			if (t->d16) mlsd_memset(t->d16, 0, sz, C->stream);
			if (t->d16) { MLFreeBlk *z = VEC_PUSH(C, C->zeroed, C->n_zeroed, C->cap_zeroed, MLFreeBlk); z->ptr = t->d16; z->size = sz; z->rel_op = t->prod; }
		} else {
			t->sz16 = (size_t)rows * t->c * 2;
			t->d16 = dalloc_ex(C, t->sz16, 0, t->prod); t->ld16 = t->c;
		}
		op = &C->ops[t->prod];
		op->u.gemm.C16 = t->d16; op->u.gemm.ldc16 = t->ld16;
		return t->d16;
	}
	if (t->is_input && t->in_type == MLT_F32 && t->h > 1) {
		const int cpad = (t->c + 7) / 8 * 8;
		t->sz16 = (size_t)rows * cpad * 2;
		t->d16 = mlctx_dalloc(C, t->sz16, 0); t->ld16 = cpad;
		MLOp *op = mlctx_op_new(C, OP_NCHW2NHWC, "nchw_to_nhwc_f16");
		op->u.n2h.src = t->in_src ? t->in_src : (const float*)t->in_stage;
		op->u.n2h.n_src = t->in_src ? t->in_src_n : t->n; op->u.n2h.C = t->c; op->u.n2h.HW = t->h*t->w;
		op->u.n2h.dst = t->d16; op->u.n2h.n_dst = t->n; op->u.n2h.Cpad = cpad;
		op->u.n2h.scale = t->in_scale; op->u.n2h.scale0 = t->in_scale0; op->u.n2h.mode = t->in_mode;
		return t->d16;
	}
	if (t->d32 && t->ld32 == t->c) {
		t->sz16 = (size_t)rows * t->c * 2;
		t->d16 = mlctx_dalloc(C, t->sz16, 0); t->ld16 = t->c;
		MLOp *op = mlctx_op_new(C, OP_ACT, "f32_to_f16");
		op->u.act.x = t->d32; op->u.act.y = t->d16; op->u.act.n = (size_t)rows * t->c; op->u.act.act = MLSD_ACT_NONE;
		return t->d16;
	}
	mlctx_fail(C, "tensor %s has no fp16 form", t->name);
	return NULL;
}

MLB_API void mlb_release(MLCtx* C, MLTensor* t)
{
	if (!t || t->released || t->is_input) return;
	t->released = 1;
	if (t->sz32) mlctx_drelease(C, t->d32, t->sz32);
	if (t->sz16) mlctx_drelease(C, t->d16, t->sz16);
	if (t->sz_silu) mlctx_drelease(C, t->silu16, t->sz_silu);
	t->d32 = NULL; t->d16 = NULL; t->silu16 = NULL; t->sz32 = t->sz16 = t->sz_silu = 0;
}

MLB_API void mlctx_block_begin(MLCtx* C)
{
	MLNameRec *r = VEC_PUSH(C, C->names, C->n_names, C->cap_names, MLNameRec);
	memset(r, 0, sizeof(*r)); r->param = -1;
}
// ... 936 lines not shown
		for (int g=0; g<ns; ++g) {
			float a = 0, b = 0, c = 0, d = 0;
			mlsd_event_elapsed_ms(TC[par][0], T0[par][g], &a); mlsd_event_elapsed_ms(TC[par][0], T1[par][g], &b);
			mlsd_event_elapsed_ms(TC[par][0], TC[par][g], &c); mlsd_event_elapsed_ms(TC[par][0], C->ev_done[g], &d);
			fprintf(stderr, "[wstream] %2d (%4zu MiB, ops %d..%d): %7.2f .. %7.2f | %7.2f .. %7.2f\n", g, C->segs[g].bytes >> 20, C->segs[g].op0, C->segs[g].op1, a, b, c, d);
		}
	}
	return 1;
}

static void wire_gn_fold(MLCtx* C)
{
	const char *e = getenv("MLSD_NO_GN_FOLD");
	if (e && *e && *e != '0') return;
	const char *eh = getenv("MLSD_GN_FOLD_MAX_HW");
	const int max_hw = eh && *eh ? atoi(eh) : 1024;
	for (int i=1;i<C->n_ops;++i) {
		MLOp *l = &C->ops[i];
		if (l->kind != OP_GN || l->fused) continue;
		mlsd_gn_args *n = &l->u.gn;
		if (n->C2 || n->raw16 || n->cs1 || !n->y16 || l->gn_src[0] != i - 1) continue;
		MLOp *o = &C->ops[i-1];
		mlsd_gemm_args *g = &o->u.gemm;
		if (o->kind != OP_GEMM || o->once || g->C32 != n->x1 || g->ldc32 != n->ld1 || g->N != n->C1 || g->M != n->n_img * n->HW || g->ln_y16 || g->gn_y16 || g->colstats || g->ksplit < 2) continue;
		if (!mlsd_groupnorm_single_pass(n->n_img, n->HW, n->C1, n->n_grp)) continue;
		if (n->HW > max_hw) continue;
		{
			const char *y0 = (const char*)n->y16, *y1 = y0 + (size_t)g->M * g->N * 2;
			const struct { const void* p; size_t nb; } rd[4] = {
				{ g->resid, g->resid ? (size_t)g->M * (size_t)g->ldr * 4 : 0 }, { g->bias, g->bias ? (size_t)g->N * 4 : 0 },
				{ g->rowbias, g->rowbias ? (size_t)(g->M / (g->rows_per_batch > 0 ? g->rows_per_batch : 1)) * (size_t)g->ldrb * 4 : 0 }, { g->ws, g->ws_bytes } };
			int clash = 0;
			for (int q=0;q<4;++q) if (rd[q].p && rd[q].nb && (const char*)rd[q].p < y1 && y0 < (const char*)rd[q].p + rd[q].nb) clash = 1;
			if (clash) continue;
		}
		g->gn_y16 = n->y16; g->gn_ldy = n->C1; g->gn_gamma = n->gamma; g->gn_beta = n->beta; g->gn_eps = n->eps; g->gn_groups = n->n_grp; g->gn_hw = n->HW; g->gn_silu = n->silu;
		if (mlsd_gemm_gn_fused(g) == 1) { l->fused = 1; C->n_gn_fused++; }
		else { g->gn_y16 = NULL; g->gn_gamma = g->gn_beta = NULL; g->gn_groups = g->gn_hw = g->gn_silu = 0; }
	}
}
MLB_API int mlctx_gn_fused(const MLCtx* C) { return C ? C->n_gn_fused : 0; }

MLB_API int mlctx_prep(MLCtx* C)
{
	if (C->err) return C->err;
	if (!C->n_names || !C->result) return mlctx_fail(C, "mlctx_prep: empty graph");
	if (!mlt_need32(C, C->result)) return -1;
	if (resolve_names(C) < 0) return -1;
	double fl = 0; unsigned nconv = 0;
	for (int i=0;i<C->n_ops;++i) {
		MLOp *op = &C->ops[i];
		if (op->kind == OP_GEMM) {
			if (!op->u.gemm.C32 && !op->u.gemm.C16 && !op->u.gemm.xa_k) return mlctx_fail(C, "op %d (%s): output never consumed", i, op->label);
			if (op->u.gemm.conv) nconv++;
			if (!autotune_on()) { int r = select_gemm(C, op); if (r < 0) return -1; if (r != 1) { C->n_tune_miss++; g_tune_miss++; } }
		}
		fl += op->flops;
	}
	if (C->flags & MLB_F_DUMP) {
		char path[96]; snprintf(path, sizeof(path), "dump-graph-%s.txt", C->name[0] ? C->name : "ctx");
		if (mlctx_block_graph_dump_path(C, path) < 0) return -1;
	}
	if (!autotune_on()) { wire_gn_stats(C); wire_ln_fold(C); wire_gn_fold(C); }
	C->info.flops = fl; C->info.n_conv = nconv; C->info.n_ops = C->n_ops;
	C->info.mem_params = C->mem_params; C->info.mem_compute = C->mem_compute; C->info.mem_total = C->mem_params + C->mem_compute;
	if (C->err) return C->err;
	if (wstream_setup(C) < 0) return -1;
	C->info.mem_params = C->mem_params; C->info.mem_total = C->mem_params + C->mem_compute;
	C->prepared = 1;
	return 1;
}

static int g_hoist = -1;
static int hoist_on(void)
{
	if (g_hoist < 0) { const char *e = getenv("MLSD_NO_HOIST"); g_hoist = (e && *e && *e != '0') ? 0 : 1; }
	return g_hoist;
}
MLB_API void mlctx_set_hoist(int on) { g_hoist = on ? 1 : 0; }
MLB_API int mlctx_once_ops(const MLCtx* C) { return C->n_once; }

MLB_API int mlctx_compute(MLCtx* C)
{
	if (!C->prepared) return mlctx_fail(C, "mlctx_compute before mlctx_prep");
	for (int i=0;i<C->n_params;++i) if (!C->params[i].loaded)
		return mlctx_fail(C, "parameter '%s' was never loaded", C->params[i].key);
	double t0 = now_s();
	if (!C->tuned && autotune_on() && !mlsd_runtime_is_dry()) {
		if (C->pstream && C->n_segs) return mlctx_fail(C, "tile timing mode (MLSD_AUTOTUNE / mlctx_set_autotune) on a weight-streaming context: tune the resident plan, the shapes are the same");
		for (int i=0;i<C->n_ops;++i) {
			if (C->ops[i].kind == OP_GEMM && !C->ops[i].u.gemm.tile_variant && tune_gemm(C, &C->ops[i]) < 0) return -1;
			if (run_op(C, &C->ops[i])) {
				char why[300]; snprintf(why, sizeof(why), "%s", mlsd_last_error());
				mlsd_set_error(-1, "%s: op %d (%s) failed: %s", C->name, i, C->ops[i].label, why);
				return -1;
			}
		}
		C->tuned = 1;
		C->info.n_compute++;
		return 1;
	}
	if (C->pstream && C->n_segs) {
		if (compute_streamed(C) < 0) return -1;
		C->static_valid = 1;
		C->info.t_compute = now_s() - t0;
		C->info.n_compute++;
		return 1;
	}
	int hoist = C->n_once > 0 && hoist_on();
	if (C->flags & MLB_F_HIPGRAPH) {
// ... 16 lines not shown
			int rc = run_op(C, &C->ops[i]);
			if (rc) {
				char why[300]; snprintf(why, sizeof(why), "%s", mlsd_last_error());
				mlsd_set_error(-1, "%s: op %d (%s) failed: %s", C->name, i, C->ops[i].label, why);
				return -1;
			}
		}
	}
	C->static_valid = 1;
	C->info.t_compute = now_s() - t0;
	C->info.n_compute++;
	return 1;
}

MLB_API void mlctx_info(const MLCtx* C, MLCtxInfo* out)
{
	*out = C->info;
	out->mem_params = C->mem_params; out->mem_compute = C->mem_compute; out->mem_total = C->mem_params + C->mem_compute;
}

MLB_API const mlsd_gemm_args* mlctx_op_gemm_args(const MLCtx* C, int i)
{
	if (!C || i < 0 || i >= C->n_ops || C->ops[i].kind != OP_GEMM) return NULL;
	return &C->ops[i].u.gemm;
}

MLB_API const mlsd_attn_args* mlctx_op_attn_args(const MLCtx* C, int i)
{
	if (!C || i < 0 || i >= C->n_ops || (C->ops[i].kind != OP_ATTN && C->ops[i].kind != OP_ATTN_CTX)) return NULL;
	return &C->ops[i].u.attn;
}

MLB_API int mlctx_op_record(const MLCtx* C, int i, MLOpRecord* out)
{
	if (!C || !out || i < 0 || i >= C->n_ops) return -1;
	const MLOp *o = &C->ops[i];
	out->kind = (int)o->kind; out->fused = o->fused; out->once = o->once;
	out->gn_src[0] = o->gn_src[0]; out->gn_src[1] = o->gn_src[1];
	out->label = o->label; out->args = &o->u; out->args_bytes = k_op_class[o->kind].args_bytes;
	return 1;
}

MLB_API int mlctx_param_device(const MLCtx* C, int i, const void** dev, size_t* elems, int* elem_bytes)
{
	if (!C || i < 0 || i >= C->n_params) return -1;
	if (dev) *dev = C->params[i].dev;
	if (elems) *elems = C->params[i].dev_elems;
	if (elem_bytes) *elem_bytes = C->params[i].type == MLT_F16 ? 2 : 4;
	return 1;
}

MLB_API int mlctx_weight_slab(const MLCtx* C, int k, const void** dev, size_t* nbytes)
{
	if (!C || !C->pstream || k < 0 || k >= C->n_slab || !C->slab[k]) return 0;
	if (dev) *dev = C->slab[k];
	if (nbytes) *nbytes = C->slab_bytes;
	return 1;
}

MLB_API int mlctx_input_count(const MLCtx* C) { return C ? C->n_inputs : 0; }
MLB_API int mlctx_input_record(const MLCtx* C, int i, MLInputRecord* out)
{
	if (!C || !out || i < 0 || i >= C->n_inputs) return -1;
	const MLTensor *t = C->inputs[i];
	out->name = t->name; out->stage = t->in_stage; out->stage_bytes = t->in_bytes;
	out->src = t->in_src; out->n_src = t->in_src_n; out->scale = t->in_scale;
	return 1;
}

MLB_API int mlctx_zeroed_block(const MLCtx* C, int i, const void** dev, size_t* nbytes)
{
	if (!C || i < 0 || i >= C->n_zeroed) return 0;
	if (dev) *dev = C->zeroed[i].ptr;
	if (nbytes) *nbytes = C->zeroed[i].size;
	return 1;
}

MLB_API int mlctx_scratch_block(const MLCtx* C, int which, const void** dev, size_t* nbytes)
{
	const void *p = NULL; size_t n = 0;
	if (!C) return 0;
	switch (which) {
	case 0: p = C->splitk_ws; n = C->splitk_ws_bytes; break;
	case 1: p = C->sk_flags; n = (size_t)SK_FLAG_WORDS * 4; break;
	case 2: p = C->ln_cnt; n = (size_t)LN_CNT_WORDS * 4; break;
	case 3: p = C->ln_ws; n = C->ln_ws_bytes; break;
	}
	if (!p) return 0;
	if (dev) *dev = p;
	if (nbytes) *nbytes = n;
	return 1;
}

MLB_API int mlctx_op_attn_is_ctx(const MLCtx* C, int i) { return C && i >= 0 && i < C->n_ops && C->ops[i].kind == OP_ATTN_CTX; }

MLB_API int mlctx_op_info(const MLCtx* C, int i, const char** label, double* flops)
{
	if (i < 0 || i >= C->n_ops) return -1;
	if (label) {
		const MLOp *op = &C->ops[i];
		const MLOpClass *k = &k_op_class[op->kind];
		static _Thread_local char buf[96];
		*label = (!op->label[0] && k->unnamed) ? k->unnamed(op) : op->label;
		if (k->shape && (C->flags & MLB_F_OPSHAPES)) {
			snprintf(buf, sizeof(buf), "%s ", *label);
			const size_t l = strlen(buf);
// ... 100 lines not shown
	}
	case 2: {
		const int64_t k = i % p->lp[0], row = i / p->lp[0], d = p->lp[1];
		const int64_t j = row < d ? row : row - d;
		return ((j >> 5) * 64 + (row < d ? 0 : 32) + (j & 31)) * p->lp[0] + k;
	}
	case 3: {
		const int64_t d = p->lp[1], j = i < d ? i : i - d;
		return (j >> 5) * 64 + (i < d ? 0 : 32) + (j & 31);
	}
	default: return i;
	}
}

MLB_API int mlctx_param_set(MLCtx* C, const char* key, int src_type, const void* host, int64_t n_elem)
{
	if (!C->prepared) return mlctx_fail(C, "mlctx_param_set before mlctx_prep (names are resolved at prep)");
	MLParam *p = NULL;
	for (int i=0;i<C->n_params;++i) if (C->params[i].key && !strcmp(C->params[i].key, key)) { p = &C->params[i]; break; }
	if (!p) return mlctx_fail(C, "unknown parameter '%s'", key);
	const int64_t n = p->ne[0]*p->ne[1]*p->ne[2]*p->ne[3];
	if (n != n_elem) return mlctx_fail(C, "parameter '%s': %lld elements given, %lld expected", key, (long long)n_elem, (long long)n);
	const size_t esz = p->type == MLT_F16 ? 2 : 4;
	void *buf = calloc(p->dev_elems, esz);
	if (src_type != MLT_F32 && src_type != MLT_F16 && src_type != MLT_BF16 && src_type != MLT_F64) {
		free(buf);
		return mlctx_fail(C, "parameter '%s': unsupported source type %d", key, src_type);
	}
	for (int64_t i=0;i<n;++i) {
		float v;
		switch (src_type) {
		case MLT_F16: v = f16_to_f32(((const uint16_t*)host)[i]); break;
		case MLT_BF16: { uint32_t u = (uint32_t)((const uint16_t*)host)[i] << 16; memcpy(&v, &u, 4); } break;
		case MLT_F64: { double d; memcpy(&d, (const char*)host + i*8, 8); v = (float)d; } break;
		default: memcpy(&v, (const char*)host + i*4, 4); break;
		}
		const int64_t o = param_dst_index(p, i);
		if (p->type == MLT_F16) ((uint16_t*)buf)[o] = f32_to_f16_rne(v); else ((float*)buf)[o] = v;
	}
	int rc = 0;
	char *pm = param_master(C, p);
	if (pm) {
		if (C->copy_stream) { mlsd_stream_sync(C->stream); mlsd_stream_sync(C->copy_stream); }
		C->pf_valid = 0;
		memcpy(pm, buf, p->dev_elems * esz);
	} else {
		rc = mlsd_memcpy(p->dev, buf, p->dev_elems * esz, 0, C->stream);
		if (!rc) rc = mlsd_stream_sync(C->stream);
	}
	free(buf);
	if (rc) return -1;
	p->loaded = 1;
	C->static_valid = 0;
	return 1;
}

MLB_API int mlctx_param_find(const MLCtx* C, const char* key)
{
	for (int i=0; C && key && i<C->n_params; ++i) if (C->params[i].key && !strcmp(C->params[i].key, key)) return i;
	return -1;
}

static int scratch_need(MLCtx* C, void** buf, size_t* have, size_t nbytes)
{
	if (*have >= nbytes) return 0;
	if (mlsd_stream_sync(C->stream)) return -1;
	if (*buf) mlsd_free(*buf);
	*buf = NULL; *have = 0;
	if (mlsd_malloc(buf, ALIGN_UP(nbytes, (size_t)1 << 20))) return -1;
	*have = ALIGN_UP(nbytes, (size_t)1 << 20);
	return 0;
}

MLB_API int mlctx_param_lora(MLCtx* C, const char* key, const float* up, const float* down, int64_t n0, int64_t n1, int r, float scale)
{
	if (!C) return -1;
	if (!C->prepared) return mlctx_fail(C, "mlctx_param_lora before mlctx_prep (names are resolved at prep)");
	const int ip = mlctx_param_find(C, key);
	if (ip < 0) return 0;
	MLParam *p = &C->params[ip];
	const int64_t n = p->ne[0]*p->ne[1]*p->ne[2]*p->ne[3];
	if (!up || !down || r < 1 || n0 < 1 || n1 < 1 || n0 > n || n % n0 || n / n0 != n1)
		return mlctx_fail(C, "parameter '%s': LoRA of %lld x %lld, rank %d, for %lld elements", key, (long long)n1, (long long)n0, r, (long long)n);
	if (!p->loaded) return mlctx_fail(C, "parameter '%s': LoRA before the weight is loaded", key);
	if (p->type != MLT_F16 && p->type != MLT_F32) return mlctx_fail(C, "parameter '%s': unsupported type %d", key, p->type);
	const size_t nu = (size_t)n1 * (size_t)r, nd = (size_t)r * (size_t)n0, pbytes = p->dev_elems * (p->type == MLT_F16 ? 2 : 4);
	if (scratch_need(C, &C->lora_buf, &C->lora_buf_bytes, 256 + (nu + nd) * 4)) return -1;
	int *d_flag = (int*)C->lora_buf;
	float *d_up = (float*)((char*)C->lora_buf + 256), *d_down = d_up + nu;
	void *W = p->dev;
	char *pm = param_master(C, p);
	if (pm) {
		if (C->copy_stream) { mlsd_stream_sync(C->stream); mlsd_stream_sync(C->copy_stream); }
		C->pf_valid = 0;
		if (scratch_need(C, &C->pscratch, &C->pscratch_bytes, pbytes)) return -1;
		W = C->pscratch;
		if (mlsd_memcpy(W, pm, pbytes, 0, C->stream)) return -1;
	}
	int bad = 0;
	if (mlsd_memset(d_flag, 0, 4, C->stream) || mlsd_memcpy(d_up, up, nu * 4, 0, C->stream) || mlsd_memcpy(d_down, down, nd * 4, 0, C->stream)) return -1;
	if (mlsd_lora_apply(W, p->type == MLT_F16 ? 1 : 0, n0, n1, d_up, d_down, r, scale, p->layout, p->lp[0], p->lp[1], p->lp[2], p->lp[3], p->lp[4], d_flag, C->stream)) return -1;
	if (mlsd_memcpy(&bad, d_flag, 4, 1, C->stream) || mlsd_stream_sync(C->stream)) return -1;
	C->static_valid = 0;
	if (bad) return mlsd_set_error(-1, "NaN in LoRA result");
	if (pm && (mlsd_memcpy(pm, W, pbytes, 1, C->stream) || mlsd_stream_sync(C->stream))) return -1;
	return 1;
}

static uint64_t mix64(uint64_t z)
{
	z ^= z >> 30; z *= 0xBF58476D1CE4E5B9ULL;
	z ^= z >> 27; z *= 0x94D049BB133111EBULL;
	z ^= z >> 31; return z;
}

MLB_API int mlctx_params_synth(MLCtx* C, uint64_t seed)
{
	if (!C->prepared) return mlctx_fail(C, "mlctx_params_synth before mlctx_prep");
	double t0 = now_s();
	for (int i=0;i<C->n_params;++i) {
		MLParam *p = &C->params[i];
		int nd = 4; while (nd > 1 && p->ne[nd-1] == 1) nd--;
		float offset = 0, scale;
		const size_t lk = strlen(p->key);
		if (nd == 1) {
			if (lk >= 5 && !strcmp(p->key + lk - 5, ".bias")) { offset = 0; scale = 0.05f; }
			else { offset = 1; scale = 0.1f; }
		} else {
			const double fan_in = nd >= 3 ? (double)p->ne[0]*p->ne[1]*p->ne[2] : (double)p->ne[0];
			scale = (float)(1.0 / sqrt(fan_in));
		}
		uint64_t h = 0xCBF29CE484222325ULL;
		for (const char *s = p->key; *s; ++s) { h ^= (unsigned char)*s; h *= 0x100000001B3ULL; }
		const uint64_t key = mix64(h ^ (seed * 0x9E3779B97F4A7C15ULL));
		const float kf = (float)((double)scale * 1.7320508075688772 / 65536.0);
		const int64_t n = p->ne[0]*p->ne[1]*p->ne[2]*p->ne[3];
		void *dst = p->dev;
		char *pm = param_master(C, p);
		const size_t pbytes = p->dev_elems * (p->type == MLT_F16 ? 2 : 4);
		if (pm) {
			if (C->pf_valid) { if (C->copy_stream) mlsd_stream_sync(C->copy_stream); C->pf_valid = 0; }
			if (C->pscratch_bytes < pbytes) {
				if (mlsd_stream_sync(C->stream)) return -1;
				if (C->pscratch) mlsd_free(C->pscratch);
				C->pscratch = NULL; C->pscratch_bytes = 0;
				if (mlsd_malloc(&C->pscratch, ALIGN_UP(pbytes, (size_t)1 << 20))) return -1;
				C->pscratch_bytes = ALIGN_UP(pbytes, (size_t)1 << 20);
			}
			dst = C->pscratch;
			if (p->layout == 1 && p->lp[4] != p->lp[2] && mlsd_memset(dst, 0, pbytes, C->stream)) return -1;
		}
		if (mlsd_synth_fill(dst, p->type == MLT_F16 ? 1 : 0, n, key, offset, kf, p->layout,
				p->lp[0], p->lp[1], p->lp[2], p->lp[3], p->lp[4], C->stream)) return -1;
		if (pm && mlsd_memcpy(pm, dst, pbytes, 1, C->stream)) return -1;
		p->loaded = 1;
	}
	if (mlsd_stream_sync(C->stream)) return -1;
	C->info.t_load = now_s() - t0;
	return 1;
}
```

### mlimgsynth_amd/csrc/host/mlblock_int.h

```cpp
#pragma once
#include "mlblock_amd.h"
#include "mlsd_kernels.h"
#include <stdio.h>
#include <stdlib.h>
#include <string.h>

#define MLB_API __attribute__((visibility("default")))

int mlsd_set_error(int code, const char* fmt, ...);

typedef enum {
	OP_GEMM, OP_ATTN, OP_GN, OP_LN, OP_NCHW2NHWC, OP_NHWC2NCHW, OP_TEMB, OP_ACT, OP_CLIP_EMBED, OP_SOFTMAX,
	OP_COPY_F32, OP_XA_VT, OP_ATTN_CTX, OP_CTRL_ADD, OP_FREEU_BACKBONE, OP_FREEU_SKIP,
	OP_KIND_COUNT
} MLOpKind;

typedef struct MLOp {
	MLOpKind kind;
	double flops;
	char label[56];
	int gn_src[2];
	int fused;
	int folded_from;
	int once;
	union {
		mlsd_gemm_args gemm;
		mlsd_attn_args attn;
		mlsd_gn_args gn;
		mlb_ln_args ln;
		mlb_n2h_args n2h;
		mlb_h2n_args h2n;
		mlb_temb_args temb;
		mlb_act_args act;
		mlb_cemb_args cemb;
		mlb_smax_args smax;
		mlb_copy_args copy;
		mlb_cadd_args cadd;
		mlb_freeu_args freeu;
		mlb_xavt_args xavt;
	} u;
} MLOp;

#define MLOP_MAX_OUTPUTS 5
#define MLOP_MAX_PARAMS  7
typedef struct MLOpClass {
	const char* name;
	size_t args_bytes;
	int (*run)(const MLOp* op, void* stream);
	struct { int n; size_t off[MLOP_MAX_OUTPUTS]; } out;
	int (*outputs)(const MLOp* op, const void* out[MLOP_MAX_OUTPUTS]);
	struct { int n; size_t off[MLOP_MAX_PARAMS]; } params;
	double (*bytes)(const MLOp* op);
	void (*shape)(const MLOp* op, char* buf, size_t n);
	const char* (*unnamed)(const MLOp* op);
	int fused_is_no_launch;
} MLOpClass;
extern const MLOpClass k_op_class[OP_KIND_COUNT];
int mlop_outputs(const MLOp* op, const void* out[MLOP_MAX_OUTPUTS]);

struct MLTensor {
	int64_t ne[4];
	int n, h, w, c;
	float* d32;  int64_t ld32;
	void*  d16;  int64_t ld16;
	size_t sz32, sz16;
	int prod;
	int def_op;
	MLTensor *cat_a, *cat_b;
	void* silu16;
	size_t sz_silu;
	int is_input, in_type;
	void* in_stage;
	size_t in_bytes;
	const float* in_src; int in_src_n; const float* in_scale; float in_scale0; int in_mode;
	int released;
	int* dirty;
// ... 9 lines not shown
	void* dev;
	size_t dev_elems;
	int loaded;
} MLParam;

typedef struct { int kind; char* name; int param; int64_t ne[4]; } MLNameRec;

typedef struct { void* ptr; size_t size; int rel_op; } MLFreeBlk;

#define MLW_NSLAB_MAX 5
struct MLCtx {
	void* stream;
	char name[64];
	char tprefix[32];
	int flags, wtype;
	int conv_wrap;
	int err;
	MLOp* ops; int n_ops, cap_ops;
	MLTensor** tensors; int n_tensors, cap_tensors;
	MLTensor** inputs; int n_inputs, cap_inputs;
	MLTensor* result;
	MLNameRec* names; int n_names, cap_names;
	MLParam* params; int n_params, cap_params;
	void** chunks; int n_chunks, cap_chunks;
	char* cur; size_t cur_left;
	MLFreeBlk* freel; int n_free, cap_free;
	MLFreeBlk* zeroed; int n_zeroed, cap_zeroed;
	size_t mem_compute, mem_params, mem_peak_live, mem_live;
	void* gn_ws; size_t gn_ws_bytes;
	void* graph_exec;
	struct { MLTensor* ctx; char* wbase; char* out16; int n_in, n_total, n_used; } kvb;
	struct { MLTensor* emb; char* wbase; float* bbase; float* out32; int n_in, n_total, n_used; } epb;
	const struct MLTStore* tstore;
	int prepared, tuned, n_tune_miss, n_tune_near;
	int static_valid;
	int n_once, graph_hoisted;
	int dry;
	void* splitk_ws; size_t splitk_ws_bytes;
	unsigned* sk_flags;
	unsigned* ln_cnt; float* ln_ws; size_t ln_ws_bytes; int n_ln_fused;
	int n_gn_fused;
	int n_ln_alias, cu_budget;
	int pstream;
	size_t pv_size;
	struct MLWAlloc* pv_allocs; int n_pv, cap_pv;
	char* pmaster;
	size_t slab_bytes; char* slab[MLW_NSLAB_MAX]; int n_slab;
	int pf_valid;
	struct MLWSeg* segs; int n_segs;
	void* copy_stream; void **ev_up, **ev_done;
	void* pscratch; size_t pscratch_bytes;
	void* lora_buf; size_t lora_buf_bytes;
	size_t stream_bytes_per_eval; int stream_copies_per_eval;
	MLCtxInfo info;
};

#define MLW_VBASE ((char*)0xFFFF600000000000ULL)
typedef struct MLWAlloc { size_t voff, bytes, moff; } MLWAlloc;
typedef struct MLWSeg { int op0, op1; int n; struct { size_t voff, bytes, soff, moff; } *r; size_t bytes; } MLWSeg;
void* mlctx_walloc(MLCtx* C, size_t nbytes);

MLTensor* mlt_new(MLCtx* C, int n, int h, int w, int c);
void*     mlctx_dalloc(MLCtx* C, size_t nbytes, int is_param);
void      mlctx_drelease(MLCtx* C, void* p, size_t nbytes);
MLOp*     mlctx_op_new(MLCtx* C, MLOpKind kind, const char* label);
int       mlctx_fail(MLCtx* C, const char* fmt, ...);
MLParam*  mlctx_param_new(MLCtx* C, const char* name, int type, int64_t n0, int64_t n1, int64_t n2, int64_t n3,
	int layout, int64_t lp0, int64_t lp1);
MLParam*  mlctx_param_new_at(MLCtx* C, const char* name, int type, int64_t n0, int64_t n1, int64_t n2, int64_t n3,
	int layout, void* dev);
void      mlctx_named_op(MLCtx* C, const char* name);
float*    mlt_need32(MLCtx* C, MLTensor* t);
void*     mlt_need16(MLCtx* C, MLTensor* t);

MLTensor* mlctx_input_new_seq(MLCtx* C, const char* name, int dtype, int d, int T, int N);
MLTensor* mlctx_input_new_img(MLCtx* C, const char* name, int w, int h, int c, int n);

typedef struct {
	int act;
	MLTensor* resid;
	MLTensor* rowbias;
	int act_post;
} MLEpilogue;
MLTensor* mlb_linear_ex(MLCtx* C, MLTensor* x, int n_out, bool bias, const MLEpilogue* ep, int geglu);
MLTensor* mlb_conv2d_ex(MLCtx* C, MLTensor* x, int ch_out, int k, int s, int p, int upsample, bool bias, const MLEpilogue* ep);
MLTensor* mlb_conv2d_ex2(MLCtx* C, MLTensor* x, int ch_out, int k, int s, int p, int p_end, int upsample, bool bias, const MLEpilogue* ep);
MLTensor* mlb_groupnorm_ex(MLCtx* C, MLTensor* x, int n_grp, float eps, int silu, int want_raw16, MLTensor** raw_out);
MLTensor* mlb_layer_norm_ex(MLCtx* C, MLTensor* x, float eps, int out32);
MLTensor* mlb_attn_mhead_ex(MLCtx* C, MLTensor* q, MLTensor* k, MLTensor* v, int d_out, int d_embed, int n_head,
	bool mask, bool bias, bool bias_out, MLTensor* resid);
MLTensor* mlb_resnet_ex(MLCtx* C, MLTensor* x, MLTensor* emb, int ch_out);
int mlb_cross_kv_batch(MLCtx* C, MLTensor* ctx, int n_total);
int mlb_emb_proj_batch(MLCtx* C, MLTensor* emb, int n_total);
```

### mlimgsynth_amd/csrc/host/mlblock_nn.c

```c
#include "mlblock_int.h"
#include <math.h>

#define T true
#define MLN(NAME,X)  mlctx_tensor_add(C, (NAME), (X))

static int64_t rows_of(const MLTensor* t) { return (int64_t)t->n * t->h * t->w; }

MLTensor* mlb_linear_ex(MLCtx* C, MLTensor* x, int n_out, bool bias, const MLEpilogue* ep, int geglu)
{
	if (!x || C->err) return NULL;
	mlctx_block_begin(C);
	const int n_in = x->c;
	if (C->wtype != MLT_F16 && C->wtype != MLT_F32 && C->wtype != MLT_BF16) { mlctx_fail(C, "unsupported linear weight type %d", C->wtype); return NULL; }
	if (n_in % 8) { mlctx_fail(C, "linear: n_in=%d must be a multiple of 8", n_in); return NULL; }
	const void *xd = mlt_need16(C, x);
	if (!xd) return NULL;
	MLParam *w = mlctx_param_new(C, "weight", MLT_F16, n_in, n_out, 1, 1, geglu ? 2 : 0, 0, 0);
	const void *wd = w->dev;
	const float *bd = NULL;
	if (bias) { MLParam *b = mlctx_param_new(C, "bias", MLT_F32, n_out, 1, 1, 1, geglu ? 3 : 0, 0, 0); bd = (const float*)b->dev; }
	const int n_res = geglu ? n_out/2 : n_out;
	MLTensor *y = mlt_new(C, x->n, x->h, x->w, n_res);
	const float *rd = NULL; int64_t ldr = 0;
	if (ep && ep->resid) {
// ... 92 lines not shown
	void *ws = mlctx_dalloc(C, mlsd_groupnorm_ws_bytes(x->n, HW, n_grp), 0);
	MLOp *op = mlctx_op_new(C, OP_GN, silu ? "groupnorm_silu" : "groupnorm");
	mlsd_gn_args *g = &op->u.gn;
	g->x1 = x1; g->ld1 = a->ld32; g->C1 = a->c;
	g->x2 = x2; g->ld2 = bb ? bb->ld32 : 0; g->C2 = bb ? bb->c : 0;
	g->n_img = x->n; g->HW = HW; g->n_grp = n_grp; g->eps = eps; g->gamma = wd; g->beta = bd; g->silu = silu;
	g->y16 = y->d16; g->raw16 = raw ? raw->d16 : NULL; g->ws = ws;
	op->gn_src[0] = a->prod; op->gn_src[1] = bb ? bb->prod : -1;
	return y;
}

MLB_API MLTensor* mlb_nn_groupnorm(MLCtx* C, MLTensor* x, int n_grp, bool affine, float eps)
{
	if (!affine) { mlctx_fail(C, "groupnorm without affine is not implemented"); return NULL; }
	return mlb_groupnorm_ex(C, x, n_grp, eps, 0, 0, NULL);
}

MLTensor* mlb_layer_norm_ex(MLCtx* C, MLTensor* x, float eps, int out32)
{
	if (!x || C->err) return NULL;
	mlctx_block_begin(C);
	if (!(eps > 0)) eps = 1e-5f;
	const int d = x->c;
	MLParam *w = mlctx_param_new(C, "weight", MLT_F32, d, 1, 1, 1, 0, 0, 0);
	const float *wd = (const float*)w->dev;
	MLParam *b = mlctx_param_new(C, "bias", MLT_F32, d, 1, 1, 1, 0, 0, 0);
	const float *bd = (const float*)b->dev;
	const float *xd = mlt_need32(C, x);
	if (!xd) return NULL;
	MLTensor *y = mlt_new(C, x->n, x->h, x->w, d);
	const int64_t rows = rows_of(x);
	y->sz16 = (size_t)rows * d * 2; y->d16 = mlctx_dalloc(C, y->sz16, 0); y->ld16 = d;
	if (out32) { y->sz32 = (size_t)rows * d * 4; y->d32 = (float*)mlctx_dalloc(C, y->sz32, 0); y->ld32 = d; }
	MLOp *op = mlctx_op_new(C, OP_LN, "layernorm");
	op->u.ln.x = xd; op->u.ln.ldx = x->ld32; op->u.ln.rows = (int)rows; op->u.ln.d = d; op->u.ln.eps = eps;
	op->u.ln.g = wd; op->u.ln.b = bd; op->u.ln.y16 = y->d16; op->u.ln.y32 = y->d32;
	op->gn_src[0] = x->prod; op->gn_src[1] = -1;
	return y;
}

MLB_API MLTensor* mlb_nn_layer_norm(MLCtx* C, MLTensor* x, bool affine, bool bias, float eps)
{
	if (!affine || !bias) { mlctx_fail(C, "layer_norm without affine+bias is not implemented"); return NULL; }
	return mlb_layer_norm_ex(C, x, eps, 1);
}

MLB_API MLTensor* mlb_downsample(MLCtx* C, MLTensor* x, int ch_out, bool vae)
{
	mlctx_block_begin(C);
	if (vae) return MLN("conv", mlb_conv2d_ex2(C, x, ch_out, 3, 2, 0, 1, 0, T, NULL));
	return MLN("conv", mlb_conv2d_ex(C, x, ch_out, 3, 2, 1, 0, T, NULL));
}

MLB_API MLTensor* mlb_upsample(MLCtx* C, MLTensor* x, int ch_out)
{
	mlctx_block_begin(C);
	return MLN("conv", mlb_conv2d_ex(C, x, ch_out, 3, 1, 1, 1, T, NULL));
}

static void* silu16_of(MLCtx* C, MLTensor* emb)
{
	if (emb->silu16) return emb->silu16;
	const float *e = mlt_need32(C, emb);
	if (!e) return NULL;
	const size_t n = (size_t)rows_of(emb) * emb->c;
	emb->sz_silu = n * 2;
	emb->silu16 = mlctx_dalloc(C, emb->sz_silu, 0);
	MLOp *op = mlctx_op_new(C, OP_ACT, "silu_f16");
	op->u.act.x = e; op->u.act.y = emb->silu16; op->u.act.n = n; op->u.act.act = MLSD_ACT_SILU;
	return emb->silu16;
}

int mlb_emb_proj_batch(MLCtx* C, MLTensor* emb, int n_total)
{
	if (!emb || n_total <= 0 || C->err) return -1;
	void *e16 = silu16_of(C, emb);
	if (!e16) return -1;
	const int n_in = emb->c;
	const int64_t rows = rows_of(emb);
	C->epb.emb = emb; C->epb.n_in = n_in; C->epb.n_total = n_total; C->epb.n_used = 0;
	C->epb.wbase = (char*)mlctx_walloc(C, (size_t)n_total * n_in * 2);
	C->epb.bbase = (float*)mlctx_walloc(C, (size_t)n_total * 4);
	C->epb.out32 = (float*)mlctx_dalloc(C, (size_t)rows * n_total * 4, 0);
	MLOp *op = mlctx_op_new(C, OP_GEMM, "");
	mlsd_gemm_args *g = &op->u.gemm;
	g->A = e16; g->lda = n_in; g->W_ = C->epb.wbase; g->ldb = n_in; g->M = (int)rows; g->N = n_total; g->K = n_in;
	g->bias = C->epb.bbase; g->C32 = C->epb.out32; g->ldc32 = n_total;
	op->flops = 2.0 * rows * (double)n_total * n_in;
	return 1;
}

MLTensor* mlb_resnet_ex(MLCtx* C, MLTensor* x, MLTensor* emb, int ch_out)
{
	if (!x || C->err) return NULL;
	MLTensor *x0 = x;
	const int ch_in = x->c;
	mlctx_block_begin(C);
	const int need_skip = ch_in != ch_out;
	MLTensor *raw = NULL;
	MLTensor *h = MLN("norm1", mlb_groupnorm_ex(C, x, 32, 1e-6f, 1, need_skip && x->cat_a != NULL, &raw));
	MLEpilogue ep1 = {0};
	MLTensor *ep_t = NULL;
	if (emb) {
		if (C->epb.emb == emb && emb->c == C->epb.n_in && C->epb.n_used + ch_out <= C->epb.n_total) {
			const int off = C->epb.n_used;
			mlctx_block_begin(C);
			mlctx_param_new_at(C, "weight", MLT_F16, emb->c, ch_out, 1, 1, 0, C->epb.wbase + (size_t)off * emb->c * 2);
			mlctx_param_new_at(C, "bias", MLT_F32, ch_out, 1, 1, 1, 0, C->epb.bbase + off);
			mlctx_named_op(C, "emb_proj");
// ... 269 lines not shown
```

### mlimgsynth_amd/csrc/host/tune_table.inc

```
	{ 0, 616, 166400, 2048, 0, 0, 0, 0, 2, 0, 0, 0, 10, 1 },
	{ 0, 8, 1280, 320, 1, 0, 0, 0, 2, 0, 0, 0, 30, 2 },
	{ 0, 8, 1280, 1280, 0, 0, 0, 0, 1, 0, 0, 0, 30, 10 },
	{ 0, 8, 1280, 2816, 1, 0, 0, 0, 2, 0, 0, 0, 30, 13 },
	{ 0, 8, 1280, 1280, 0, 0, 0, 0, 5, 0, 0, 0, 30, 10 },
	{ 1, 131072, 320, 72, 0, 128, 1, 0, 1, 8, 3, 0, 5, 1 },
	{ 0, 8, 320, 1280, 0, 0, 0, 0, 1, 0, 0, 0, 2, 10 },
	{ 1, 131072, 320, 2880, 0, 128, 1, 0, 1, 320, 3, 1, 21, 1 },
	{ 1, 131072, 320, 2880, 0, 128, 1, 0, 5, 320, 3, 0, 19, 1 },
	{ 1, 131072, 320, 2880, 0, 128, 1, 0, 7, 320, 3, 0, 19, 1 },
	{ 1, 32768, 320, 2880, 0, 64, 2, 0, 3, 320, 3, 0, 19, 1 },
	{ 0, 8, 640, 1280, 0, 0, 0, 0, 1, 0, 0, 0, 2, 10 },
	{ 1, 32768, 640, 2880, 0, 64, 1, 0, 1, 320, 3, 1, 21, 1 },
	{ 1, 32768, 640, 320, 0, 64, 1, 0, 1, 320, 1, 0, 19, 1 },
	{ 1, 32768, 640, 5760, 0, 64, 1, 0, 5, 640, 3, 0, 21, 1 },
	{ 1, 32768, 640, 640, 0, 64, 1, 0, 1, 640, 1, 0, 31, 1 },
	{ 0, 32768, 1920, 640, 0, 0, 0, 0, 2, 0, 0, 0, 18, 1 },
	{ 0, 32768, 640, 640, 0, 0, 0, 0, 5, 0, 0, 0, 19, 1 },
	{ 0, 32768, 640, 640, 0, 0, 0, 0, 2, 0, 0, 0, 31, 1 },
	{ 0, 32768, 5120, 640, 5, 0, 0, 0, 2, 0, 0, 0, 18, 1 },
	{ 0, 32768, 640, 2560, 0, 0, 0, 0, 5, 0, 0, 0, 19, 1 },
	{ 0, 32768, 640, 2560, 0, 0, 0, 0, 7, 0, 0, 0, 19, 1 },
	{ 1, 32768, 640, 640, 0, 64, 1, 0, 5, 640, 1, 0, 19, 1 },
	{ 1, 32768, 640, 5760, 0, 64, 1, 0, 1, 640, 3, 1, 21, 1 },
	{ 1, 32768, 640, 640, 0, 64, 1, 0, 7, 640, 1, 0, 19, 1 },
// ... 853 lines not shown
	{ 1, 4608, 640, 17280, 0, 48, 1, 0, 1, 1920, 3, 1, 29, 1 },
	{ 1, 4608, 640, 1920, 0, 48, 1, 0, 1, 1920, 1, 0, 31, 1 },
	{ 1, 18432, 640, 5760, 0, 96, 1, 1, 1, 640, 3, 0, 22, 1 },
	{ 1, 18432, 320, 960, 0, 96, 1, 0, 1, 960, 1, 0, 31, 1 },
	{ 1, 18432, 320, 640, 0, 96, 1, 0, 1, 640, 1, 0, 31, 1 },
	{ 1, 18432, 4, 2880, 0, 96, 1, 0, 1, 320, 3, 0, 1, 2 },
	{ 1, 6144, 640, 5760, 0, 48, 1, 0, 5, 640, 3, 0, 20, 1 },
	{ 1, 6144, 640, 5760, 0, 48, 1, 0, 1, 640, 3, 1, 20, 1 },
	{ 1, 1536, 1280, 11520, 0, 24, 1, 0, 5, 1280, 3, 0, 1, 4 },
	{ 0, 1536, 3840, 1280, 0, 0, 0, 0, 2, 0, 0, 0, 31, 1 },
	{ 0, 1536, 1280, 5120, 0, 0, 0, 0, 7, 0, 0, 0, 1, 4 },
	{ 1, 1536, 1280, 11520, 0, 24, 1, 0, 1, 1280, 3, 1, 1, 4 },
	{ 1, 1536, 1280, 2560, 0, 24, 1, 0, 1, 2560, 1, 0, 1, 4 },
	{ 1, 1536, 1280, 17280, 0, 24, 1, 0, 1, 1920, 3, 1, 1, 4 },
	{ 1, 1536, 1280, 1920, 0, 24, 1, 0, 1, 1920, 1, 0, 1, 4 },
	{ 1, 6144, 1280, 11520, 0, 48, 1, 1, 1, 1280, 3, 0, 1, 1 },
	{ 1, 6144, 640, 17280, 0, 48, 1, 0, 1, 1920, 3, 1, 20, 1 },
	{ 1, 6144, 640, 11520, 0, 48, 1, 0, 1, 1280, 3, 1, 20, 1 },
	{ 1, 24576, 640, 5760, 0, 96, 1, 1, 1, 640, 3, 0, 5, 1 },
	{ 1, 73728, 320, 2880, 0, 96, 1, 0, 7, 320, 3, 0, 21, 1 },
	{ 1, 18432, 640, 320, 0, 48, 1, 0, 1, 320, 1, 0, 31, 1 },
	{ 1, 18432, 640, 640, 0, 48, 1, 0, 1, 640, 1, 0, 10, 1 },
	{ 0, 18432, 640, 640, 0, 0, 0, 0, 5, 0, 0, 0, 18, 1 },
	{ 0, 18432, 640, 640, 0, 0, 0, 0, 2, 0, 0, 0, 18, 1 },
	{ 0, 18432, 640, 2560, 0, 0, 0, 0, 5, 0, 0, 0, 20, 1 },
	{ 0, 18432, 640, 2560, 0, 0, 0, 0, 7, 0, 0, 0, 20, 1 },
	{ 1, 18432, 640, 640, 0, 48, 1, 0, 7, 640, 1, 0, 10, 1 },
	{ 1, 4608, 1280, 5760, 0, 24, 1, 0, 1, 640, 3, 1, 2, 1 },
	{ 0, 4608, 3840, 1280, 0, 0, 0, 0, 2, 0, 0, 0, 31, 1 },
	{ 1, 4608, 1280, 11520, 0, 24, 1, 0, 1, 1280, 3, 1, 2, 1 },
	{ 1, 4608, 1280, 23040, 0, 24, 1, 0, 1, 2560, 3, 1, 2, 1 },
	{ 1, 4608, 1280, 2560, 0, 24, 1, 0, 1, 2560, 1, 0, 31, 1 },
	{ 1, 4608, 1280, 17280, 0, 24, 1, 0, 1, 1920, 3, 1, 2, 1 },
	{ 1, 18432, 1280, 11520, 0, 48, 1, 1, 1, 1280, 3, 0, 22, 1 },
	{ 1, 18432, 640, 1920, 0, 48, 1, 0, 1, 1920, 1, 0, 18, 1 },
	{ 1, 18432, 640, 1280, 0, 48, 1, 0, 1, 1280, 1, 0, 10, 1 },
	{ 1, 18432, 640, 960, 0, 48, 1, 0, 1, 960, 1, 0, 31, 1 },
	{ 1, 73728, 640, 5760, 0, 96, 1, 1, 1, 640, 3, 0, 5, 1 },
	{ 1, 73728, 4, 2880, 0, 96, 1, 0, 1, 320, 3, 0, 5, 1 },
	{ 0, 4608, 640, 2560, 0, 0, 0, 0, 7, 0, 0, 0, 2, 1 },
	{ 1, 6144, 640, 320, 0, 48, 1, 0, 1, 320, 1, 0, 31, 1 },
	{ 0, 6144, 640, 640, 0, 0, 0, 0, 2, 0, 0, 0, 31, 1 },
	{ 1, 1536, 1280, 640, 0, 24, 1, 0, 1, 640, 1, 0, 31, 1 },
	{ 1, 1536, 1280, 1280, 0, 24, 1, 0, 1, 1280, 1, 0, 31, 1 },
	{ 1, 1536, 1280, 23040, 0, 24, 1, 0, 1, 2560, 3, 1, 29, 1 },
	{ 1, 6144, 640, 1920, 0, 48, 1, 0, 1, 1920, 1, 0, 31, 1 },
	{ 1, 6144, 640, 1280, 0, 48, 1, 0, 1, 1280, 1, 0, 31, 1 },
	{ 1, 6144, 640, 960, 0, 48, 1, 0, 1, 960, 1, 0, 31, 1 },
	{ 1, 24576, 320, 960, 0, 96, 1, 0, 1, 960, 1, 0, 31, 1 },
	{ 1, 24576, 320, 640, 0, 96, 1, 0, 1, 640, 1, 0, 31, 1 },
	{ 0, 18432, 1920, 640, 0, 0, 0, 0, 2, 0, 0, 0, 31, 1 },
	{ 0, 4608, 1280, 5120, 0, 0, 0, 0, 5, 0, 0, 0, 31, 1 },
	{ 1, 73728, 320, 640, 0, 96, 1, 0, 1, 640, 1, 0, 31, 1 },
```

### mlimgsynth_amd/kernels.py

```python
import ctypes

from . import _lib
from ._lib import check, lib, vp

c_i64, c_int, c_f = ctypes.c_int64, ctypes.c_int, ctypes.c_float

ACT_NONE, ACT_SILU, ACT_GELU, ACT_GELU_QUICK, ACT_RELU, ACT_GEGLU = range(6)
RESAMPLE_NEAREST, RESAMPLE_BILINEAR, RESAMPLE_BICUBIC = range(3)

TILE_128x128, TILE_64x128, TILE_256x128, TILE_256x128_S3, TILE_256x256, TILE_128x320 = 0, 1, 3, 4, 9, 16
TILE_PP_256x256, TILE_PP_128x320, TILE_PPSK_256x256, TILE_PP2_128x320, TILE_PP2_256x256, TILE_PPB_128x320 = 17, 18, 19, 20, 21, 22
TILE_PP2_256x128, TILE_W4_256x256, TILE_W4_128x320, TILE_PPSK_128x320, TILE_SKINNY, TILE_TT, TILE_CONV_SMALLN = 25, 26, 27, 28, 29, 30, 31
TILE_LABELS = {TILE_128x128: "128x128x64s2", TILE_64x128: "64x128x64s2", TILE_256x128: "256x128x64s2", TILE_256x128_S3: "256x128x32s3",
               TILE_256x256: "256x256x64s2w16", TILE_128x320: "128x320x64s2", TILE_PP_256x256: "256x256x64pp", TILE_PP_128x320: "128x320x64pp",
               TILE_PPSK_256x256: "256x256x64ppsk", TILE_PP2_128x320: "128x320x64pp2", TILE_PP2_256x256: "256x256x64pp2",
               TILE_PPB_128x320: "128x320x64ppb", TILE_PP2_256x128: "256x128x64pp2", TILE_W4_256x256: "256x256x64w4",
               TILE_W4_128x320: "128x320x64w4", TILE_PPSK_128x320: "128x320x64ppsk", TILE_SKINNY: "skinny128x64", TILE_TT: "128x160x64tt",
               TILE_CONV_SMALLN: "conv3x3n16"}


def tile_arg(v):
    return v + 1


class GemmArgs(ctypes.Structure):
    _fields_ = [("A", vp), ("lda", c_i64), ("conv", c_int), ("n_img", c_int), ("H", c_int), ("W", c_int),
                ("Cin", c_int), ("OH", c_int), ("OW", c_int), ("KH", c_int), ("KW", c_int), ("stride", c_int),
                ("pad", c_int), ("upsample", c_int), ("W_", vp), ("ldb", c_i64), ("M", c_int), ("N", c_int),
                ("K", c_int), ("bias", vp), ("rowbias", vp), ("rows_per_batch", c_int), ("ldrb", c_i64),
                ("resid", vp), ("ldr", c_i64), ("act", c_int), ("C32", vp), ("ldc32", c_i64), ("C16", vp),
                ("ldc16", c_i64), ("bias_m", vp), ("act_after_resid", c_int), ("tile_variant", c_int),
                ("ksplit", c_int), ("ws", vp), ("ws_bytes", ctypes.c_size_t), ("colstats", vp), ("colstats_rows", c_int), ("sk_flags", vp),
                ("ln_y16", vp), ("ldln", ctypes.c_int64), ("ln_gamma", vp), ("ln_beta", vp), ("ln_eps", ctypes.c_float), ("ln_ws", vp), ("ln_cnt", vp), ("ln_slot", c_int),
                ("gn_y16", vp), ("gn_ldy", ctypes.c_int64), ("gn_gamma", vp), ("gn_beta", vp), ("gn_eps", ctypes.c_float), ("gn_groups", c_int), ("gn_hw", c_int),
                ("gn_silu", c_int),
                ("xa_k", vp), ("xa_ldk", c_i64), ("xa_vt", vp), ("xa_out", vp), ("xa_ldo", c_i64), ("xa_Tq", c_int), ("xa_Tk", c_int),
                ("colstats_shift", c_int), ("wrap", c_int)]


class GemmRouteInfo(ctypes.Structure):
    _fields_ = [("variant", c_int), ("asked", c_int), ("nsplit", c_int), ("stats_rows", c_int), ("ln", c_int), ("gn", c_int), ("xattn", c_int),
                ("handoff", c_int), ("stats_rows_if", c_int), ("ln_if", c_int), ("ln_ws_bytes_if", ctypes.c_size_t)]


class AttnArgs(ctypes.Structure):
    _fields_ = [("q", vp), ("k", vp), ("v", vp), ("out", vp), ("ldq", c_i64), ("ldk", c_i64), ("ldv", c_i64),
                ("ldo", c_i64), ("bsq", c_i64), ("bsk", c_i64), ("bsv", c_i64), ("bso", c_i64), ("n_batch", c_int),
                ("n_head", c_int), ("d_head", c_int), ("Tq", c_int), ("Tk", c_int), ("causal", c_int)]


class GnArgs(ctypes.Structure):
    _fields_ = [("x1", vp), ("x2", vp), ("ld1", c_i64), ("ld2", c_i64), ("C1", c_int), ("C2", c_int),
                ("n_img", c_int), ("HW", c_int), ("n_grp", c_int), ("eps", c_f), ("gamma", vp), ("beta", vp),
                ("silu", c_int), ("y16", vp), ("raw16", vp), ("ws", vp), ("cs1", vp), ("cs2", vp), ("rb_rows1", c_int), ("rb_rows2", c_int),
                ("cs_shifted", c_int)]


class LnArgs(ctypes.Structure):
    _fields_ = [("x", vp), ("ldx", c_i64), ("rows", c_int), ("d", c_int), ("eps", c_f), ("g", vp), ("b", vp), ("y16", vp), ("y32", vp)]


class N2hArgs(ctypes.Structure):
    _fields_ = [("src", vp), ("n_src", c_int), ("C", c_int), ("HW", c_int), ("dst", vp), ("n_dst", c_int), ("Cpad", c_int), ("scale", vp),
                ("scale0", c_f), ("mode", c_int)]


class H2nArgs(ctypes.Structure):
    _fields_ = [("src", vp), ("ld", c_i64), ("n", c_int), ("C", c_int), ("HW", c_int), ("dst", vp), ("mul", c_f), ("add", c_f)]


class TembArgs(ctypes.Structure):
    _fields_ = [("t", vp), ("n", c_int), ("dim", c_int), ("maxp", c_f), ("out", vp)]


class ActArgs(ctypes.Structure):
    _fields_ = [("x", vp), ("y", vp), ("n", ctypes.c_size_t), ("act", c_int)]


class CembArgs(ctypes.Structure):
    _fields_ = [("tok", vp), ("n", c_int), ("T", c_int), ("d", c_int), ("tw", vp), ("pw", vp), ("out", vp)]


class SmaxArgs(ctypes.Structure):
    _fields_ = [("in_", vp), ("ld_in", c_i64), ("out", vp), ("ld_out", c_i64), ("rows", c_int), ("cols", c_int), ("scale", c_f)]


class CopyArgs(ctypes.Structure):
    _fields_ = [("src", vp), ("dst", vp), ("nbytes", ctypes.c_size_t)]

# ... 160 lines not shown
```

Baseline: 3.007 images/s.

## Decompose nearest-upsample 3x3 conv into four 2x2 phase convolutions

Replaces the nearest-neighbour upsample followed by a 3x3 convolution with four sub-pixel phase GEMMs. Each phase runs a 2x2 kernel on the low-resolution input using pre-summed derived weights, and a new epilogue scatters results into the interleaved full-resolution output. This cuts the upsample convolution FLOPs from 9 taps to 4 per output and avoids reading the upsampled input. In exchange it adds derived weight buffers, four launches per upsample, and extra weight-derivation steps whenever weights are loaded or LoRA is applied. It only activates for large launches without conv wrap.

```diff
diff --git a/include/mlblock_amd.h b/include/mlblock_amd.h
--- a/include/mlblock_amd.h
+++ b/include/mlblock_amd.h
@@ -99,6 +99,7 @@
 int mlctx_param_info(const MLCtx* C, int i, const char** key, int* type, int64_t ne[4]);
 int mlctx_param_set(MLCtx* C, const char* key, int src_type, const void* host_data, int64_t n_elem);
 int mlctx_param_find(const MLCtx* C, const char* key);
+int mlctx_ups_weights(const MLCtx* C, int i, int* param, const void** dev, int* cout, int* cin);
 int mlctx_param_lora(MLCtx* C, const char* key, const float* up, const float* down, int64_t n0, int64_t n1, int r, float scale);
 int mlctx_params_synth(MLCtx* C, uint64_t seed);
 
diff --git a/include/mlsd_kernels.h b/include/mlsd_kernels.h
--- a/include/mlsd_kernels.h
+++ b/include/mlsd_kernels.h
@@ -118,11 +118,20 @@
 	const void* xa_vt;
 	void* xa_out; int64_t xa_ldo;
 	int xa_Tq, xa_Tk;
+	int tap_oy, tap_ox;
+	int out_phase;
 	int colstats_shift;
 	int wrap;
 } mlsd_gemm_args;
 
 int mlsd_gemm(const mlsd_gemm_args* a, void* stream);
+int mlsd_ups_phase_weights(const void* src, void* dst, int cout, int cin, void* stream);
+int mlsd_ups_phase_weights_host(const void* src, void* dst, int cout, int cin);
+long mlsd_conv_tap_source(const mlsd_gemm_args* a, int m, int kh, int kw);
+long mlsd_conv_out_pixel(const mlsd_gemm_args* a, int m);
+int mlsd_gemm_phase_form(const mlsd_gemm_args* a);
+void mlsd_gemm_set_ups_phases(int mode);
+int mlsd_gemm_ups_phases(void);
 int mlsd_gemm_colstats_rows(const mlsd_gemm_args* a);
 int mlsd_gemm_ln_fused(const mlsd_gemm_args* a);
 int mlsd_gemm_xattn_fused(const mlsd_gemm_args* a);
diff --git a/mlimgsynth_amd/csrc/hip/gemm_conv.hip b/mlimgsynth_amd/csrc/hip/gemm_conv.hip
--- a/mlimgsynth_amd/csrc/hip/gemm_conv.hip
+++ b/mlimgsynth_amd/csrc/hip/gemm_conv.hip
@@ -792,6 +792,7 @@
     p.ldrb = a->ldrb; p.resid = a->resid; p.ldr = a->ldr; p.act = a->act;
     p.C32 = a->C32; p.ldc32 = a->ldc32; p.C16 = (_Float16*)a->C16; p.ldc16 = a->ldc16;
     p.cs_shift = a->colstats_shift ? 1 : 0;
+    p.tap_oy = a->tap_oy; p.tap_ox = a->tap_ox; p.opix = a->out_phase;
     return p;
 }
 
@@ -894,9 +895,17 @@
 
 int g_gemm_korder = 0;
 int pp_epilogue_kind(const mlsd_gemm_args* a, int BN);
+bool phase_fields(const mlsd_gemm_args* a) { return a->tap_oy || a->tap_ox || a->out_phase; }
+bool phase_ok(const mlsd_gemm_args* a, int BN)
+{
+    if (!a->conv || a->upsample || a->stride != 1 || a->tap_oy < 0 || a->tap_oy > 1 || a->tap_ox < 0 || a->tap_ox > 1 || a->out_phase < 0 || a->out_phase > 4) return false;
+    if (!a->out_phase) return true;
+    return !(a->OW & 15) && a->OH > 0 && a->M == a->n_img * a->OH * a->OW && pp_epilogue_kind(a, BN) == PP_EPI_F32_PIX;
+}
 bool pp_eligible(const mlsd_gemm_args* a, int BM, int BN)
 {
-    if ((a->K & 63) || a->K < 192 || (a->M % (BM / 2)) || (a->N % (BN / 4))) return false;
+    if (phase_fields(a) && !phase_ok(a, BN)) return false;
+    if ((a->K & 63) || a->K < 192 || (a->out_phase ? (a->M & 15) : (a->M % (BM / 2))) || (a->N % (BN / 4))) return false;
     if (a->conv && ((a->Cin & 63) || a->KH * a->KW > 9)) return false;
     if (a->conv && a->upsample) {
         const int e = pp_epilogue_kind(a, BN);
@@ -904,7 +913,7 @@
     }
     if (a->conv && a->wrap) {
         const int e = pp_epilogue_kind(a, BN);
-        if (a->pad > 16 || a->H > 16000 || a->W > 16000 || (e != PP_EPI_F32 && e != PP_EPI_F32_STATS && e != PP_EPI_F32_RES && e != PP_EPI_F32_RES_STATS)) return false;
+        if (a->pad > 16 || a->H > 16000 || a->W > 16000 || (e != PP_EPI_F32 && e != PP_EPI_F32_STATS && e != PP_EPI_F32_RES && e != PP_EPI_F32_RES_STATS && e != PP_EPI_F32_PIX)) return false;
     }
     if (a->rowbias && ((a->rows_per_batch > 0 ? a->rows_per_batch : 1) % BM)) return false;
     if (a->act == MLSD_ACT_GEGLU && BN != 256) return false;
@@ -942,6 +951,8 @@
 {
     if (a->xa_k && BN == 320 && xattn_eligible(a)) return PP_EPI_XATTN;
     if ((g_gemm_dbg & 2) || a->bias_m) return PP_EPI_GENERIC;
+    if (a->out_phase)
+        return (a->act == MLSD_ACT_NONE && a->C32 && !a->C16 && !a->resid && !a->rowbias && !a->colstats && !a->ln_y16 && !a->gn_y16 && !a->xa_k) ? PP_EPI_F32_PIX : PP_EPI_GENERIC;
     const bool c16_wide = a->C16 && !(a->ldc16 & 7) && !((uintptr_t)a->C16 & 15);
     if (a->act == MLSD_ACT_NONE) {
         if (a->C16 && !a->C32 && !a->resid) return c16_wide ? PP_EPI_F16 : PP_EPI_GENERIC;
@@ -963,7 +974,7 @@
 
 bool sk_eligible(const mlsd_gemm_args* a, int BM, int BN, bool ignore_stats = false)
 {
-    if (!pp_eligible(a, BM, BN) || !a->ws || !a->sk_flags || ((uintptr_t)a->ws & 15) || device_cus() < g_gemm_ncu || (a->conv && a->upsample)) return false;
+    if (!pp_eligible(a, BM, BN) || !a->ws || !a->sk_flags || ((uintptr_t)a->ws & 15) || device_cus() < g_gemm_ncu || (a->conv && a->upsample) || phase_fields(a)) return false;
     if (a->conv && a->colstats && !ignore_stats) return false;
     if (a->conv && a->wrap && !a->colstats && pp_epilogue_kind(a, BN) != PP_EPI_F32 && pp_epilogue_kind(a, BN) != PP_EPI_F32_RES) return false;
     const long tiles = (long)((a->M + BM - 1) / BM) * ((a->N + BN - 1) / BN), nkt = a->K / 64;
@@ -1031,6 +1042,8 @@
         default: return go(gemm_pp_kernel<BM, BN, CB0, CB1, RESBATCH, false, PP_EPI_GENERIC, true>);
         }
     }
+    if (epi == PP_EPI_F32_PIX)
+        return r.wrap ? go(gemm_pp_kernel<BM, BN, CB0, CB1, RESBATCH, 5, PP_EPI_F32_PIX, false, NPH, SCH>) : go(gemm_pp_kernel<BM, BN, CB0, CB1, RESBATCH, true, PP_EPI_F32_PIX, false, NPH, SCH>);
     if (r.wrap) {
         if (a->upsample) {
             if (epi == PP_EPI_F32_STATS) return go(gemm_pp_kernel<BM, BN, CB0, CB1, RESBATCH, 6, PP_EPI_F32_STATS, false, NPH, SCH>);
@@ -1085,7 +1098,7 @@
 
 bool skinny_eligible(const mlsd_gemm_args* a)
 {
-    if (a->M > 128 || a->act == MLSD_ACT_GEGLU || (a->K & 63) || a->K < 128 || (a->N & 3) || !a->ws || ((uintptr_t)a->ws & 15)) return false;
+    if (a->M > 128 || a->act == MLSD_ACT_GEGLU || (a->K & 63) || a->K < 128 || (a->N & 3) || !a->ws || ((uintptr_t)a->ws & 15) || phase_fields(a)) return false;
     if (a->conv && (a->upsample || (a->Cin & 63) || a->KH * a->KW > 9)) return false;
     if (a->conv && a->wrap && (a->pad > 16 || a->H > 16000 || a->W > 16000)) return false;
     return wide_epilogue_ok(a);
@@ -1234,6 +1247,10 @@
     r.pick = pick_variant(a);
     int v = r.pick;
     GemmFamily fam = FAM_GENERAL;
+    if (phase_fields(a)) {
+        const bool is_pp = v == MLSD_TILE_PP_256x256 || v == MLSD_TILE_PP_128x320 || v == MLSD_TILE_PP2_256x256 || v == MLSD_TILE_PP2_128x320;
+        if (!is_pp || !pp_eligible(a, kVariants[v].bm, kVariants[v].bn)) v = pp_eligible(a, 256, 256) ? MLSD_TILE_PP_256x256 : MLSD_TILE_PP_128x320;
+    }
     switch (v) {
     case MLSD_TILE_W4_256x256: case MLSD_TILE_W4_128x320:
         if (mlsd_gemm_w4_eligible(a, v - MLSD_TILE_W4_256x256)) fam = FAM_W4; else v = v == MLSD_TILE_W4_256x256 ? MLSD_TILE_PP_256x256 : MLSD_TILE_PP_128x320;
@@ -1336,6 +1353,10 @@
     if (a->act == MLSD_ACT_GEGLU && (a->N & 63)) return mlsd_set_error(-1, "mlsd_gemm: GEGLU needs N %% 64 == 0");
     if (!a->C32 && !a->C16 && !a->xa_k) return mlsd_set_error(-1, "mlsd_gemm: no output");
     const GemmRoute r = resolve(a);
+    if (phase_fields(a) && r.fam != FAM_PP)
+        return mlsd_set_error(-1, "mlsd_gemm: tap_oy / tap_ox / out_phase = %d / %d / %d: only the ping-pong convolution tiles take the phase form of an upsampling convolution "
+                              "(conv, no upsample, stride 1, K %% 64 == 0 and >= 192, Cin %% 64 == 0, N in whole wave columns; out_phase: OW %% 16 == 0, fp32 output, bias only)",
+                              a->tap_oy, a->tap_ox, a->out_phase);
     if (a->colstats && a->colstats_rows > 0 && r.stats_rows != a->colstats_rows)
         return mlsd_set_error(-1, "mlsd_gemm: a GroupNorm was planned on this launch's column statistics (blocks of %d rows) but the launch "
                               "would write %d-row blocks / none: tile or epilogue settings changed after planning", a->colstats_rows, r.stats_rows);
@@ -1449,6 +1470,16 @@
 
 MLSD_API void mlsd_gemm_set_xattn(int mode) { g_xattn_mode = (mode >= 0 && mode <= 2) ? mode : -1; }
 
+MLSD_API int mlsd_gemm_phase_form(const mlsd_gemm_args* a) { return a && phase_fields(a) && resolve(a).fam == FAM_PP; }
+
+static int g_ups_phases = -2;
+MLSD_API void mlsd_gemm_set_ups_phases(int mode) { g_ups_phases = (mode == 0 || mode == 2) ? mode : -1; }
+MLSD_API int mlsd_gemm_ups_phases(void)
+{
+    if (g_ups_phases == -2) { const char* e = getenv("MLSD_UPS_PHASES"); g_ups_phases = (e && (*e == '0' || *e == '2') && !e[1]) ? *e - '0' : -1; }
+    return g_ups_phases;
+}
+
 MLSD_API int mlsd_gemm_xattn_fused(const mlsd_gemm_args* a) { mlsd_gemm_route_info r; return mlsd_gemm_route(a, &r) ? 0 : r.xattn; }
 
 MLSD_API const char* mlsd_gemm_variant(const mlsd_gemm_args* a)
diff --git a/mlimgsynth_amd/csrc/hip/gemm_params.hpp b/mlimgsynth_amd/csrc/hip/gemm_params.hpp
--- a/mlimgsynth_amd/csrc/hip/gemm_params.hpp
+++ b/mlimgsynth_amd/csrc/hip/gemm_params.hpp
@@ -52,11 +52,20 @@
     long xa_ldk, xa_ldo;
     int xa_Tq, xa_Tk;
     float xa_sc;
+    int tap_oy, tap_ox, opix;
 };
 
 static_assert(offsetof(GemmP, wrap) + sizeof(int) == offsetof(GemmP, rowbias), "GemmP::wrap must fill act_post's padding");
 
-__device__ __forceinline__ int wrap_fold(int v, int e) { return v < 0 ? v + e : (v >= e ? v - e : v); }
+__host__ __device__ __forceinline__ int wrap_fold(int v, int e) { return v < 0 ? v + e : (v >= e ? v - e : v); }
+
+__host__ __device__ __forceinline__ long ups_out_pixel(int m, int OH, int OW, int opix)
+{
+    const int hw = OH * OW, ph = opix - 1;
+    const int img = m / hw, rem = m - img * hw;
+    const int y = rem / OW, x = rem - y * OW;
+    return (long)img * 4 * hw + (long)(2 * y + (ph >> 1)) * (2 * OW) + 2 * x + (ph & 1);
+}
 
 template <int BK>
 __device__ __forceinline__ int row_swz(int row) { return BK == 64 ? ((row >> 1) & 7) : ((row >> 2) & 3); }
diff --git a/mlimgsynth_amd/csrc/hip/gemm_pp.hpp b/mlimgsynth_amd/csrc/hip/gemm_pp.hpp
--- a/mlimgsynth_amd/csrc/hip/gemm_pp.hpp
+++ b/mlimgsynth_amd/csrc/hip/gemm_pp.hpp
@@ -43,7 +43,7 @@
 }
 
 enum { PP_EPI_GENERIC = 0, PP_EPI_F16 = 1, PP_EPI_F32 = 2, PP_EPI_F32_RES = 3, PP_EPI_GEGLU16 = 4, PP_EPI_F32_STATS = 5, PP_EPI_F32_RES_STATS = 6,
-       PP_EPI_F32_LN = 7, PP_EPI_F32_RES_LN = 8, PP_EPI_XATTN = 9 };
+       PP_EPI_F32_LN = 7, PP_EPI_F32_RES_LN = 8, PP_EPI_XATTN = 9, PP_EPI_F32_PIX = 10 };
 template <int BM, int BN, int CB0, int CB1, bool RESBATCH, int CONV, int EPI, bool SK = false, int NPH = 4, int SCH = 0>
 __global__ __launch_bounds__(512) void gemm_pp_kernel(const GemmP p)
 {
@@ -124,7 +124,7 @@
                 const int ohw = p.OH * p.OW;
                 const int img = m / ohw, rem = m - img * ohw;
                 const int oh = rem / p.OW, ow = rem - oh * p.OW;
-                const int ih0 = oh * p.stride - p.pad, iw0 = ow * p.stride - p.pad;
+                const int ih0 = oh * p.stride - p.pad + p.tap_oy, iw0 = ow * p.stride - p.pad + p.tap_ox;
                 const int He = UPS ? 2 * p.H : p.H, We = UPS ? 2 * p.W : p.W;
                 int mk = 0;
                 if constexpr (WRAP) {
@@ -317,8 +317,9 @@
             }
         }
     };
-    auto epi_fast = [&](auto S32_, auto S16_, auto RES_, auto ST_, int wrow0, int wcol0) __attribute__((always_inline)) {
-        constexpr bool S32 = decltype(S32_)::value, S16 = decltype(S16_)::value, RES = decltype(RES_)::value, ST = decltype(ST_)::value;
+    auto epi_fast = [&](auto S32_, auto S16_, auto RES_, auto ST_, auto PIX_, int wrow0, int wcol0) __attribute__((always_inline)) {
+        constexpr bool S32 = decltype(S32_)::value, S16 = decltype(S16_)::value, RES = decltype(RES_)::value, ST = decltype(ST_)::value, PIX = decltype(PIX_)::value;
+        static_assert(!PIX || (S32 && !S16 && !RES && !ST), "the pixel map is built for the plain fp32 epilogue");
         constexpr int NR = 2 * RA;
         constexpr int PF = !ST ? (BM == 128 ? NR : 2) : (BM == 128 ? NR : 1);
         f32x4 cs[ST ? NCB : 1], cq[ST ? NCB : 1], ck[ST ? NCB : 1];
@@ -338,12 +339,21 @@
         };
 #pragma unroll
         for (int r = 0; r < PF && r < NR; ++r) fetch(r);
-        float* c32b = S32 ? p.C32 + (long)(wrow0 + l15) * p.ldc32 + wcol0 + 4 * lg : nullptr;
+        float* c32b = S32 && !PIX ? p.C32 + (long)(wrow0 + l15) * p.ldc32 + wcol0 + 4 * lg : nullptr;
         _Float16* c16b = S16 ? p.C16 + (long)(wrow0 + l15) * p.ldc16 + wcol0 + 4 * lg : nullptr;
 #pragma unroll
         for (int r = 0; r < NR; ++r) {
             if (r + PF < NR) fetch(r + PF);
             const int qa = r / RA, i = r % RA;
+            if constexpr (PIX) {
+                const int mb = wrow0 + row_of(r);
+                if (mb < p.M) {
+                    const long opx = ups_out_pixel(mb, p.OH, p.OW, p.opix) + 2 * l15;
+                    float* orow = p.C32 + opx * p.ldc32 + wcol0 + 4 * lg;
+#pragma unroll
+                    for (int c = 0; c < NCB; ++c) *reinterpret_cast<f32x4*>(orow + c * 16) = acc[qa][i][c] + cb[c];
+                }
+            } else
             if constexpr (S16 && !S32 && !RES && !ST) {
                 _Float16* rowp = p.C16 + (long)(wrow0 + l15 + row_of(r)) * p.ldc16 + wcol0 + 8 * (lg >> 1) + 16 * (lg & 1);
 #pragma unroll
@@ -783,11 +793,12 @@
         using std::integral_constant;
         using T = std::true_type;
         using F = std::false_type;
-        if constexpr (EPI == PP_EPI_F16) { epi_fast(F{}, T{}, F{}, F{}, wrow0, wcol0); return; }
-        if constexpr (EPI == PP_EPI_F32) { epi_fast(T{}, F{}, F{}, F{}, wrow0, wcol0); return; }
-        if constexpr (EPI == PP_EPI_F32_RES) { epi_fast(T{}, F{}, T{}, F{}, wrow0, wcol0); return; }
-        if constexpr (EPI == PP_EPI_F32_STATS) { epi_fast(T{}, F{}, F{}, T{}, wrow0, wcol0); return; }
-        if constexpr (EPI == PP_EPI_F32_RES_STATS) { epi_fast(T{}, F{}, T{}, T{}, wrow0, wcol0); return; }
+        if constexpr (EPI == PP_EPI_F16) { epi_fast(F{}, T{}, F{}, F{}, F{}, wrow0, wcol0); return; }
+        if constexpr (EPI == PP_EPI_F32) { epi_fast(T{}, F{}, F{}, F{}, F{}, wrow0, wcol0); return; }
+        if constexpr (EPI == PP_EPI_F32_RES) { epi_fast(T{}, F{}, T{}, F{}, F{}, wrow0, wcol0); return; }
+        if constexpr (EPI == PP_EPI_F32_STATS) { epi_fast(T{}, F{}, F{}, T{}, F{}, wrow0, wcol0); return; }
+        if constexpr (EPI == PP_EPI_F32_RES_STATS) { epi_fast(T{}, F{}, T{}, T{}, F{}, wrow0, wcol0); return; }
+        if constexpr (EPI == PP_EPI_F32_PIX) { epi_fast(T{}, F{}, F{}, F{}, T{}, wrow0, wcol0); return; }
         if constexpr (EPI == PP_EPI_GEGLU16) { epi_fast_geglu(wrow0, wcol0); return; }
         if constexpr (EPI == PP_EPI_F32_LN) { epi_ln(F{}, wrow0, wcol0); return; }
         if constexpr (EPI == PP_EPI_F32_RES_LN) { epi_ln(T{}, wrow0, wcol0); return; }
diff --git a/mlimgsynth_amd/csrc/hip/ups_phase.hip b/mlimgsynth_amd/csrc/hip/ups_phase.hip
--- /dev/null
+++ b/mlimgsynth_amd/csrc/hip/ups_phase.hip
@@ -0,0 +1,75 @@
+#include <hip/hip_runtime.h>
+#include "common.hpp"
+#include "gemm_params.hpp"
+
+namespace {
+
+__host__ __device__ __forceinline__ void ups_tap_set(int par, int a, int& k0, int& k1)
+{
+    if (par == 0) { k0 = a ? 1 : 0; k1 = a ? 2 : 0; }
+    else { k0 = a ? 2 : 0; k1 = a ? 2 : 1; }
+}
+
+__host__ __device__ __forceinline__ _Float16 ups_phase_weight(const _Float16* src, long e, int cout, int cin)
+{
+    const int c = (int)(e % cin); long t = e / cin;
+    const int b = (int)(t & 1), a = (int)((t >> 1) & 1); t >>= 2;
+    const int o = (int)(t % cout), phase = (int)(t / cout);
+    int kh0, kh1, kw0, kw1;
+    ups_tap_set(phase >> 1, a, kh0, kh1);
+    ups_tap_set(phase & 1, b, kw0, kw1);
+    float s = 0.f;
+    bool first = true;
+    for (int kh = kh0; kh <= kh1; ++kh)
+        for (int kw = kw0; kw <= kw1; ++kw) {
+            const float w = (float)src[((long)(o * 3 + kh) * 3 + kw) * cin + c];
+            s = first ? w : s + w;
+            first = false;
+        }
+    return (_Float16)s;
+}
+
+__global__ void ups_phase_weights_kernel(const _Float16* __restrict__ src, _Float16* __restrict__ dst, int cout, int cin, long n)
+{
+    GRID_LOOP(e, n) dst[e] = ups_phase_weight(src, e, cout, cin);
+}
+
+}
+
+extern "C" {
+
+MLSD_API int mlsd_ups_phase_weights(const void* src, void* dst, int cout, int cin, void* stream)
+{
+    if (!src || !dst || cout < 1 || cin < 1) return mlsd_set_error(-1, "mlsd_ups_phase_weights: null pointer or empty weight (%d x %d)", cout, cin);
+    const long n = 16L * cout * cin;
+    if (mlsd_runtime_is_dry()) return mlsd_ups_phase_weights_host(src, dst, cout, cin);
+    hipLaunchKernelGGL(ups_phase_weights_kernel, dim3(nblk(n)), dim3(256), 0, (hipStream_t)stream, (const _Float16*)src, (_Float16*)dst, cout, cin, n);
+    return mlsd_check_launch("ups_phase_weights");
+}
+
+MLSD_API int mlsd_ups_phase_weights_host(const void* src, void* dst, int cout, int cin)
+{
+    if (!src || !dst || cout < 1 || cin < 1) return mlsd_set_error(-1, "mlsd_ups_phase_weights_host: null pointer or empty weight (%d x %d)", cout, cin);
+    const long n = 16L * cout * cin;
+    for (long e = 0; e < n; ++e) ((_Float16*)dst)[e] = ups_phase_weight((const _Float16*)src, e, cout, cin);
+    return 0;
+}
+
+MLSD_API long mlsd_conv_tap_source(const mlsd_gemm_args* a, int m, int kh, int kw)
+{
+    if (!a || !a->conv || a->upsample || m < 0 || m >= a->M) return -2;
+    const int ohw = a->OH * a->OW, img = m / ohw, rem = m - img * ohw, oh = rem / a->OW, ow = rem - oh * a->OW;
+    int ih = oh * a->stride - a->pad + a->tap_oy + kh, iw = ow * a->stride - a->pad + a->tap_ox + kw;
+    if (a->wrap & 2) ih = wrap_fold(ih, a->H);
+    if (a->wrap & 1) iw = wrap_fold(iw, a->W);
+    if ((unsigned)ih >= (unsigned)a->H || (unsigned)iw >= (unsigned)a->W) return -1;
+    return ((long)img * a->H + ih) * a->W + iw;
+}
+
+MLSD_API long mlsd_conv_out_pixel(const mlsd_gemm_args* a, int m)
+{
+    if (!a || m < 0 || m >= a->M) return -2;
+    return a->out_phase ? ups_out_pixel(m, a->OH, a->OW, a->out_phase) : m;
+}
+
+}
diff --git a/mlimgsynth_amd/csrc/host/mlblock.c b/mlimgsynth_amd/csrc/host/mlblock.c
--- a/mlimgsynth_amd/csrc/host/mlblock.c
+++ b/mlimgsynth_amd/csrc/host/mlblock.c
@@ -69,7 +69,7 @@
 	C->n_chunks = 0; C->cur = NULL; C->cur_left = 0; C->n_free = 0; C->n_zeroed = 0;
 	C->mem_compute = C->mem_params = C->mem_live = C->mem_peak_live = 0;
 	C->err = 0; C->prepared = 0; C->tuned = 0; C->n_tune_miss = 0; C->n_tune_near = 0; C->static_valid = 0; C->n_once = 0;
-	C->n_ln_fused = 0; C->n_ln_alias = 0; C->n_gn_fused = 0;
+	C->n_ln_fused = 0; C->n_ln_alias = 0; C->n_gn_fused = 0; C->n_ups = 0;
 	memset(&C->kvb, 0, sizeof(C->kvb));
 	memset(&C->epb, 0, sizeof(C->epb));
 	memset(&C->info, 0, sizeof(C->info));
@@ -80,7 +80,7 @@
 	if (!C) return;
 	mlsd_stream_sync(C->stream);
 	ctx_reset(C);
-	free(C->ops); free(C->tensors); free(C->inputs); free(C->names); free(C->params); free(C->chunks); free(C->freel); free(C->zeroed);
+	free(C->ops); free(C->tensors); free(C->inputs); free(C->names); free(C->params); free(C->chunks); free(C->freel); free(C->zeroed); free(C->ups);
 	free(C);
 }
 
@@ -262,9 +262,10 @@
 	const int64_t rows = (int64_t)t->n * t->h * t->w;
 	if (t->prod >= 0) {
 		MLOp *op = &C->ops[t->prod];
+		const int nph = op->phases > 0 ? op->phases : 1;
 		t->sz32 = (size_t)rows * t->c * sizeof(float);
-		t->d32 = (float*)dalloc_ex(C, t->sz32, 0, t->prod); t->ld32 = t->c;
-		op->u.gemm.C32 = t->d32; op->u.gemm.ldc32 = t->c;
+		t->d32 = (float*)dalloc_ex(C, t->sz32, 0, t->prod - (nph - 1)); t->ld32 = t->c;
+		for (int k=0;k<nph;++k) { op[-k].u.gemm.C32 = t->d32; op[-k].u.gemm.ldc32 = t->c; }
 		return t->d32;
 	}
 	mlctx_fail(C, "tensor %s has no fp32 form", t->name);
@@ -277,6 +278,9 @@
 	if (t->d16) return t->d16;
 	if (t->released) { mlctx_fail(C, "use of released tensor %s", t->name); return NULL; }
 	const int64_t rows = (int64_t)t->n * t->h * t->w;
+	if (t->prod >= 0 && C->ops[t->prod].phases > 0) {
+		if (!mlt_need32(C, t)) return NULL;
+	} else
 	if (t->prod >= 0) {
 		MLOp *op = &C->ops[t->prod];
 		if (t->c % 8) {
@@ -1319,10 +1323,10 @@
 		MLOp *op = &C->ops[i];
 		if (op->kind == OP_GEMM) {
 			if (!op->u.gemm.C32 && !op->u.gemm.C16 && !op->u.gemm.xa_k) return mlctx_fail(C, "op %d (%s): output never consumed", i, op->label);
-			if (op->u.gemm.conv) nconv++;
+			if (op->u.gemm.conv && (!op->u.gemm.out_phase || op->phases)) nconv++;
 			if (!autotune_on()) { int r = select_gemm(C, op); if (r < 0) return -1; if (r != 1) { C->n_tune_miss++; g_tune_miss++; } }
 		}
-		fl += op->flops;
+		fl += op->flops + op->flops_saved;
 	}
 	if (C->flags & MLB_F_DUMP) {
 		char path[96]; snprintf(path, sizeof(path), "dump-graph-%s.txt", C->name[0] ? C->name : "ctx");
@@ -1445,6 +1449,11 @@
 
 MLB_API int mlctx_weight_slab(const MLCtx* C, int k, const void** dev, size_t* nbytes)
 {
+	if (C && !C->pstream && k >= 0 && k < C->n_ups) {
+		if (dev) *dev = C->ups[k].dev;
+		if (nbytes) *nbytes = (size_t)16 * C->ups[k].cout * C->ups[k].cin * 2;
+		return 1;
+	}
 	if (!C || !C->pstream || k < 0 || k >= C->n_slab || !C->slab[k]) return 0;
 	if (dev) *dev = C->slab[k];
 	if (nbytes) *nbytes = C->slab_bytes;
@@ -1651,7 +1660,48 @@
 	if (rc) return -1;
 	p->loaded = 1;
 	C->static_valid = 0;
-	return 1;
+	if (mlctx_ups_derive(C, (int)(p - C->params)) < 0) return -1;
+	return 1;
+}
+
+void* mlctx_ups_weights_new(MLCtx* C, int param, int cout, int cin)
+{
+	void *dev = mlctx_walloc(C, (size_t)16 * cout * cin * 2);
+	if (!dev) return NULL;
+	struct MLUpsW *u = VEC_PUSH(C, C->ups, C->n_ups, C->cap_ups, struct MLUpsW);
+	u->param = param; u->dev = dev; u->cout = cout; u->cin = cin;
+	return dev;
+}
+
+int mlctx_ups_derive(MLCtx* C, int param)
+{
+	int n = 0;
+	for (int i=0;i<C->n_ups;++i) {
+		const struct MLUpsW *u = &C->ups[i];
+		if (param >= 0 && u->param != param) continue;
+		if (is_virtual(C, u->dev)) {
+			if (mlsd_stream_sync(C->stream) || (C->copy_stream && mlsd_stream_sync(C->copy_stream))) return -1;
+			C->pf_valid = 0;
+			const size_t vo = (size_t)((const char*)u->dev - MLW_VBASE);
+			const MLWAlloc *a = &C->pv_allocs[pv_find(C, vo)];
+			if (mlsd_ups_phase_weights_host(param_master(C, &C->params[u->param]), C->pmaster + a->moff + (vo - a->voff), u->cout, u->cin)) return -1;
+		} else
+		if (mlsd_ups_phase_weights(C->params[u->param].dev, u->dev, u->cout, u->cin, C->stream)) return -1;
+		++n;
+	}
+	return n;
+}
+
+MLB_API int mlctx_ups_weights(const MLCtx* C, int i, int* param, const void** dev, int* cout, int* cin)
+{
+	if (!C) return 0;
+	if (i >= 0 && i < C->n_ups) {
+		if (param) *param = C->ups[i].param;
+		if (dev) *dev = C->ups[i].dev;
+		if (cout) *cout = C->ups[i].cout;
+		if (cin) *cin = C->ups[i].cin;
+	}
+	return C->n_ups;
 }
 
 MLB_API int mlctx_param_find(const MLCtx* C, const char* key)
@@ -1703,6 +1753,7 @@
 	C->static_valid = 0;
 	if (bad) return mlsd_set_error(-1, "NaN in LoRA result");
 	if (pm && (mlsd_memcpy(pm, W, pbytes, 1, C->stream) || mlsd_stream_sync(C->stream))) return -1;
+	if (mlctx_ups_derive(C, ip) < 0) return -1;
 	return 1;
 }
 
@@ -1754,6 +1805,7 @@
 		if (pm && mlsd_memcpy(pm, dst, pbytes, 1, C->stream)) return -1;
 		p->loaded = 1;
 	}
+	if (mlctx_ups_derive(C, -1) < 0) return -1;
 	if (mlsd_stream_sync(C->stream)) return -1;
 	C->info.t_load = now_s() - t0;
 	return 1;
diff --git a/mlimgsynth_amd/csrc/host/mlblock_int.h b/mlimgsynth_amd/csrc/host/mlblock_int.h
--- a/mlimgsynth_amd/csrc/host/mlblock_int.h
+++ b/mlimgsynth_amd/csrc/host/mlblock_int.h
@@ -22,6 +22,8 @@
 	int gn_src[2];
 	int fused;
 	int folded_from;
+	double flops_saved;
+	int phases;
 	int once;
 	union {
 		mlsd_gemm_args gemm;
@@ -137,6 +139,7 @@
 	void* pscratch; size_t pscratch_bytes;
 	void* lora_buf; size_t lora_buf_bytes;
 	size_t stream_bytes_per_eval; int stream_copies_per_eval;
+	struct MLUpsW { int param; void* dev; int cout, cin; } *ups; int n_ups, cap_ups;
 	MLCtxInfo info;
 };
 
@@ -144,6 +147,8 @@
 typedef struct MLWAlloc { size_t voff, bytes, moff; } MLWAlloc;
 typedef struct MLWSeg { int op0, op1; int n; struct { size_t voff, bytes, soff, moff; } *r; size_t bytes; } MLWSeg;
 void* mlctx_walloc(MLCtx* C, size_t nbytes);
+void* mlctx_ups_weights_new(MLCtx* C, int param, int cout, int cin);
+int   mlctx_ups_derive(MLCtx* C, int param);
 
 MLTensor* mlt_new(MLCtx* C, int n, int h, int w, int c);
 void*     mlctx_dalloc(MLCtx* C, size_t nbytes, int is_param);
diff --git a/mlimgsynth_amd/csrc/host/mlblock_nn.c b/mlimgsynth_amd/csrc/host/mlblock_nn.c
--- a/mlimgsynth_amd/csrc/host/mlblock_nn.c
+++ b/mlimgsynth_amd/csrc/host/mlblock_nn.c
@@ -168,9 +168,51 @@
 	return MLN("conv", mlb_conv2d_ex(C, x, ch_out, 3, 2, 1, 0, T, NULL));
 }
 
+static MLTensor* conv_ups_phases(MLCtx* C, MLTensor* x, int ch_out, const mlsd_gemm_args* proto)
+{
+	mlctx_block_begin(C);
+	const void *xd = mlt_need16(C, x);
+	if (!xd) return NULL;
+	if (x->ld16 != x->c) { mlctx_fail(C, "upsample: padded input rows in the phase form"); return NULL; }
+	const int ch_in = x->c, cpad = proto->Cin;
+	MLParam *w = mlctx_param_new(C, "weight", MLT_F16, 3, 3, ch_in, ch_out, 1, 0, 0);
+	const int wi = (int)(w - C->params);
+	MLParam *b = mlctx_param_new(C, "bias", MLT_F32, ch_out, 1, 1, 1, 0, 0, 0);
+	const float *bd = (const float*)b->dev;
+	const char *wd = (const char*)mlctx_ups_weights_new(C, wi, ch_out, cpad);
+	if (!wd) return NULL;
+	MLTensor *y = mlt_new(C, x->n, 2*x->h, 2*x->w, ch_out);
+	for (int ph=0; ph<4; ++ph) {
+		MLOp *op = mlctx_op_new(C, OP_GEMM, "");
+		mlsd_gemm_args *g = &op->u.gemm;
+		*g = *proto;
+		g->A = xd; g->W_ = wd + (size_t)ph * ch_out * 4 * cpad * 2; g->bias = bd;
+		g->tap_oy = ph >> 1; g->tap_ox = ph & 1; g->out_phase = 1 + ph;
+		op->flops = 2.0 * g->M * (double)ch_out * 4 * ch_in;
+		if (ph == 3) { op->phases = 4; op->flops_saved = 2.0 * 4 * g->M * (double)ch_out * 5 * ch_in; }
+	}
+	y->prod = C->n_ops - 1;
+	return y;
+}
+
 MLB_API MLTensor* mlb_upsample(MLCtx* C, MLTensor* x, int ch_out)
 {
 	mlctx_block_begin(C);
+	const int mode = mlsd_gemm_ups_phases();
+	if (x && !C->err && mode != 0 && !C->dry && x->h > 1 && !(x->c % 8)) {
+		mlsd_gemm_args g; memset(&g, 0, sizeof g);
+		g.lda = x->c; g.conv = 1; g.n_img = x->n; g.H = x->h; g.W = x->w; g.Cin = x->c; g.OH = x->h; g.OW = x->w;
+		g.KH = 2; g.KW = 2; g.stride = 1; g.pad = 1; g.wrap = C->conv_wrap;
+		g.ldb = 4 * (int64_t)x->c; g.M = x->n * x->h * x->w; g.N = ch_out; g.K = 4 * x->c;
+		g.rows_per_batch = x->h * x->w; g.ldrb = ch_out;
+		static _Alignas(256) float ph[64];
+		g.A = ph; g.W_ = ph; g.bias = ph; g.C32 = ph; g.ldc32 = ch_out; g.tap_oy = 1; g.tap_ox = 1; g.out_phase = 4;
+		const long tiles = (ch_out % 320 && ch_out % 256) ? 0 : (long)(g.M / 128) * ((ch_out + 319) / 320);
+		if (mlsd_gemm_phase_form(&g) && (mode == 2 || (tiles >= 256 && !C->conv_wrap))) {
+			g.A = g.W_ = NULL; g.bias = NULL; g.C32 = NULL; g.ldc32 = 0;
+			return MLN("conv", conv_ups_phases(C, x, ch_out, &g));
+		}
+	}
 	return MLN("conv", mlb_conv2d_ex(C, x, ch_out, 3, 1, 1, 1, T, NULL));
 }
 
diff --git a/mlimgsynth_amd/csrc/host/tune_table.inc b/mlimgsynth_amd/csrc/host/tune_table.inc
--- a/mlimgsynth_amd/csrc/host/tune_table.inc
+++ b/mlimgsynth_amd/csrc/host/tune_table.inc
@@ -929,3 +929,11 @@
 	{ 0, 18432, 1920, 640, 0, 0, 0, 0, 2, 0, 0, 0, 31, 1 },
 	{ 0, 4608, 1280, 5120, 0, 0, 0, 0, 5, 0, 0, 0, 31, 1 },
 	{ 1, 73728, 320, 640, 0, 96, 1, 0, 1, 640, 1, 0, 31, 1 },
+	{ 1, 8192, 1280, 5120, 0, 32, 1, 0, 1, 1280, 2, 0, 19, 1 },
+	{ 1, 32768, 640, 2560, 0, 64, 1, 0, 1, 640, 2, 0, 19, 1 },
+	{ 1, 16384, 1280, 5120, 0, 32, 1, 0, 1, 1280, 2, 0, 19, 1 },
+	{ 1, 65536, 640, 2560, 0, 64, 1, 0, 1, 640, 2, 0, 19, 1 },
+	{ 1, 16384, 640, 2560, 0, 64, 1, 0, 1, 640, 2, 0, 19, 1 },
+	{ 1, 65536, 512, 2048, 0, 128, 1, 0, 1, 512, 2, 0, 18, 1 },
+	{ 1, 262144, 512, 2048, 0, 256, 1, 0, 1, 512, 2, 0, 18, 1 },
+	{ 1, 1048576, 256, 1024, 0, 512, 1, 0, 1, 256, 2, 0, 18, 1 },
diff --git a/mlimgsynth_amd/kernels.py b/mlimgsynth_amd/kernels.py
--- a/mlimgsynth_amd/kernels.py
+++ b/mlimgsynth_amd/kernels.py
@@ -35,6 +35,7 @@
                 ("gn_y16", vp), ("gn_ldy", ctypes.c_int64), ("gn_gamma", vp), ("gn_beta", vp), ("gn_eps", ctypes.c_float), ("gn_groups", c_int), ("gn_hw", c_int),
                 ("gn_silu", c_int),
                 ("xa_k", vp), ("xa_ldk", c_i64), ("xa_vt", vp), ("xa_out", vp), ("xa_ldo", c_i64), ("xa_Tq", c_int), ("xa_Tk", c_int),
+                ("tap_oy", c_int), ("tap_ox", c_int), ("out_phase", c_int),
                 ("colstats_shift", c_int), ("wrap", c_int)]
 
 
```

Measured after the change: 3.060 images/s (median of 6 runs). +1.7%, better.
